# babybirdprd/dia-tts-prune

Hardware: AMD Instinct MI355X
Metric: audio-codec frames/sec (Dia-1.6B decode, whole job) (higher is better)
Workload: dtype bf16; 1 GPU; Dia-1.6B bf16 weights, bf16 K/V, batch 1, 1890 decode steps, text bytes [98], cfg 3.0 / T 1.3 / top-p 0.95 / top-k 35, hipGraph=True; batch_per_gpu=1, parallelism=single

## Files before the change

### dia-tts-prune_amd/csrc/engine.hip

```cpp
#include "common.hpp"
#include "../../include/dia_hip.h"
#include "errors.hpp"
#include "launch.hpp"
#include "tuning.hpp"
#include <cstdlib>
#include <vector>
#include <algorithm>
#include <utility>

struct dia_engine {
  dia_engine_desc d;
  std::vector<dia_dec_layer> layers;
  hipStream_t stream = nullptr;
  hipGraph_t graph = nullptr;
  hipGraphExec_t exec = nullptr;
  int launches = 0;
  bool seg = false;
  std::vector<const void*> seg_w;
  int mlp_fused = -1;
  std::vector<hipEvent_t> prof;
  int pf_lookahead = 0;
  bool pf_capturing = false;
  hipStream_t side = nullptr;
  std::vector<hipEvent_t> pf_ev;
  std::vector<std::pair<const void*, long>> pf_w;
};

int dia_prefetch_launch(const void* ptr, long nbytes, int nblocks, hipStream_t st);
static int ensure_sink();

static inline void mark(dia_engine* e, int i) {
  if (!e->prof.empty() && i + 1 < (int)e->prof.size()) (void)hipEventRecord(e->prof[i + 1], e->stream);
  if (e->pf_capturing) {
    const int j = i + e->pf_lookahead;
    if (j < (int)e->pf_w.size() && e->pf_w[j].first != nullptr) {
      (void)hipEventRecord(e->pf_ev[i], e->stream);
      (void)hipStreamWaitEvent(e->side, e->pf_ev[i], 0);
      const long bytes = e->pf_w[j].second;
      const int nb = (int)std::min<long>(512, std::max<long>(32, bytes / (256 * 16 * 8)));
      (void)dia_prefetch_launch(e->pf_w[j].first, bytes, nb, e->side);
    }
  }
}

constexpr int MXFP8_DEFAULT = (1 << DIA_MAT_WI | 1 << DIA_MAT_WO | 1 << DIA_MAT_LOGITS) | (1 << DIA_MAT_WI | 1 << DIA_MAT_LOGITS) << 8;
static_assert(MXFP8_DEFAULT == 0x5070 && DIA_MAT_COUNT <= 8, "the knob mxfp8 holds one byte of class bits per row range");
extern "C" int dia_mxfp8_classes(int rows) {
  if (rows <= 0 || rows > 16) return 0;
  const int knob = dia_tune(DIA_TUNE_MXFP8);
  const int mask = knob >= 0 ? knob : MXFP8_DEFAULT;
  return (rows <= 4 ? mask : mask >> 8) & ((1 << DIA_MAT_COUNT) - 1);
}

enum { PL_NONE = -1, PL_X, PL_A, PL_H };
enum { OUT_NONE, OUT_QKV, OUT_QC, OUT_LOGITS, OUT_X };
struct step_mat_row {
  int mat;
  const void* dia_dec_layer::*w; int32_t dia_dec_layer::*kt; int32_t dia_dec_layer::*ns;
  const void* dia_dec_layer::*w24; const void* dia_dec_layer::*wf8;
  int epi, in, out, emit;
  const int32_t* dia_dec_layer::*cmap;
  const float* dia_dec_layer::*gnext;
};
#define MAT(M, m) DIA_MAT_##M, &dia_dec_layer::w_##m, &dia_dec_layer::kt_##m, &dia_dec_layer::ns_##m, &dia_dec_layer::w_##m##_24, &dia_dec_layer::w_##m##_f8
constexpr step_mat_row STEP_MATS[DIA_MAT_COUNT] = {
  {MAT(QKV, qkv), DIA_EPI_SCALE_STORE, PL_X, OUT_QKV, PL_NONE, nullptr, nullptr},
  {MAT(O, o), DIA_EPI_RESID_EMIT, PL_A, OUT_X, PL_X, &dia_dec_layer::cmap_ca, &dia_dec_layer::g_ca},
  {MAT(CQ, cq), DIA_EPI_SCALE_STORE, PL_X, OUT_QC, PL_NONE, nullptr, nullptr},
  {MAT(CO, co), DIA_EPI_RESID_EMIT, PL_A, OUT_X, PL_X, &dia_dec_layer::cmap_mlp, &dia_dec_layer::g_mlp},
  {MAT(WI, wi), DIA_EPI_SWIGLU_EMIT, PL_X, OUT_NONE, PL_H, nullptr, nullptr},
  {MAT(WO, wo), DIA_EPI_RESID_EMIT, PL_H, OUT_X, PL_X, &dia_dec_layer::cmap_next, nullptr},
  {DIA_MAT_LOGITS, nullptr, nullptr, nullptr, nullptr, nullptr, DIA_EPI_SCALE_STORE, PL_X, OUT_LOGITS, PL_NONE, nullptr, nullptr},
};
#undef MAT
constexpr bool rows_in_order(int m = 0) { return m == DIA_MAT_COUNT || (STEP_MATS[m].mat == m && rows_in_order(m + 1)); }
static_assert(rows_in_order(), "row m of STEP_MATS describes matrix m of dia_step_mat");

struct mat_w { const void* w; int kt, ns; const void *w24, *wf8; };
static mat_w mat_weights(const dia_engine* e, int l, int m) {
  const dia_engine_desc& d = e->d;
  if (m == DIA_MAT_LOGITS) return {d.w_logits, d.kt_logits, d.ns_logits, d.w_logits_24, d.w_logits_f8};
  const dia_dec_layer& L = e->layers[l];
  const step_mat_row& r = STEP_MATS[m];
  return {L.*r.w, L.*r.kt, L.*r.ns, L.*r.w24, L.*r.wf8};
}

enum { ATTN_SELF = DIA_MAT_COUNT, ATTN_CROSS, SEG_MLP, SAMPLER };
template <class Launch>
static int step_sequence(const dia_engine* e, bool with_sampler, Launch&& launch) {
  int rc = DIA_OK;
  auto run = [&](int l, std::initializer_list<int> seq) { for (int what : seq) if (!rc) rc = launch(l, what); };
  for (int l = 0; l < e->d.n_layer; ++l) {
    if (!e->seg || l == 0) run(l, {DIA_MAT_QKV});
    run(l, {ATTN_SELF, DIA_MAT_O, DIA_MAT_CQ, ATTN_CROSS});
    if (e->seg) run(l, {SEG_MLP});
    else run(l, {DIA_MAT_CO, DIA_MAT_WI, DIA_MAT_WO});
  }
  run(e->d.n_layer, {DIA_MAT_LOGITS});
  if (with_sampler) run(e->d.n_layer, {SAMPLER});
  return rc;
}

static bool wo_split_k(const dia_engine_desc& d, const dia_dec_layer& L, int R, dia_gemm_args& g) {
  int wo_sk = (R <= 4 && L.kt_wo % 2 == 0) ? 2 : ((R <= 16 && L.kt_wo % 4 == 0) ? 4 : 1);
  int wo_spw = 0;
  if (R > 4 && R <= 16) {
    if (L.kt_wo % 64 == 0 && L.kt_wo / 64 >= 2 && L.kt_wo / 64 <= 8) wo_sk = L.kt_wo / 64;
    if (wo_sk > 1 && L.ns_wo * wo_sk >= 512 && L.ns_wo % 2 == 0) wo_spw = 2;
  }
  const int w2_sk = (d.w_planes == 2 && L.kt_wo % 128 == 0 && L.kt_wo / 128 <= 8) ? L.kt_wo / 128 : 1;
  if (d.w_planes == 2) { wo_sk = w2_sk; wo_spw = 0; }
  if (dia_tune(DIA_TUNE_WO_SK) >= 1 && dia_tune(DIA_TUNE_WO_SK) <= 8 && L.kt_wo % dia_tune(DIA_TUNE_WO_SK) == 0) wo_sk = dia_tune(DIA_TUNE_WO_SK);
  g.sk = wo_sk; g.sk_scratch = wo_sk > 1 ? d.sk_scratch : nullptr; g.sk_tickets = wo_sk > 1 ? d.sk_tickets : nullptr;
  bool wo_pair = false;
  if (R > 16 && R <= 128) {
    g.sk_scratch = d.sk_scratch; g.sk_tickets = d.sk_tickets;
    g.sk_scratch_floats = d.sk_scratch_floats > 0 ? d.sk_scratch_floats : (int64_t)(d.D / 16) * 4 * 512;
    wo_pair = L.kt_wo % 4 == 0 && g.sk_scratch_floats >= (int64_t)((R + 15) / 16) * L.ns_wo * 4 * 256 &&
              dia_tune(DIA_TUNE_WO_PAIR) != 0;
    g.sk = wo_pair ? 4 : 1;
    if (d.w_planes == 2) {
      wo_pair = w2_sk > 1 && g.sk_scratch_floats >= (int64_t)((R + 15) / 16) * L.ns_wo * w2_sk * 256;
      g.sk = wo_pair ? w2_sk : 1;
    }
  }
  if (dia_tune(DIA_TUNE_WO_NW) > 0) g.nw = dia_tune(DIA_TUNE_WO_NW);
  g.spw = wo_spw;
  if (dia_tune(DIA_TUNE_WO_SPW) > 0) g.spw = dia_tune(DIA_TUNE_WO_SPW);
  return wo_pair;
}

static int enqueue_step(dia_engine* e, bool with_sampler) {
  const dia_engine_desc& d = e->d;
  void* st = (void*)e->stream;
  const int R = 2 * d.B;
  const int xkt = d.D / 32;
  const int akt = (max(d.q_heads, d.cq_heads) * 128) / 32;
  const int hkt = d.F / 32;
  const long mt = d.rows_pad / 16;
  const struct { void* p; long stride; int kt; } planes[] = {
    {d.planes_x, mt * xkt * 512, xkt}, {d.planes_a, mt * akt * 512, akt}, {d.planes_h, mt * hkt * 512, hkt}};
  const int nqkv = (d.q_heads + 2 * d.kv_heads) * 128;
  const int F = d.act_f32 ? 1 : 0;
  const bool two_tiles = R > 16 && R <= 32 && d.sk_scratch && d.sk_tickets && d.sk_scratch_floats > 0;

  const bool seg = e->seg;
  bool diag = (R <= 2 || (R <= 4 && d.F <= 4096)) && d.act_f32 && d.w_planes <= 1 && dia_tune(DIA_TUNE_WO_DIAG) == 1 && !seg;
  for (int l = 0; l < d.n_layer && diag; ++l) diag = e->layers[l].w_wo_diag != nullptr && e->layers[l].cmap_next == nullptr;
  const int xn_wo = diag ? d.D / 8 : d.D / 16;
  auto sparse24 = [&](dia_gemm_args& g, const void* w24) {
    if (!w24 || !F || d.w_planes > 1 || R > 4) return;
    g.W = w24; g.KT /= 2; g.w_format = DIA_W_SPARSE24; g.nw = 0; g.spw = 0;
    int sk = g.sk > 1 ? g.sk : 1;
    while (sk > 1 && g.KT % (8 * sk) != 0) sk /= 2;
    g.sk = sk;
    if (sk == 1) { g.sk_scratch = nullptr; g.sk_tickets = nullptr; }
  };
  const int f8_mask = (F && d.w_planes <= 1 && !seg && !diag) ? dia_mxfp8_classes(R) : 0;
  auto mxfp8 = [&](dia_gemm_args& g, const void* wf8, int cls) {
    if (!wf8 || !(f8_mask >> cls & 1) || g.cmap || g.strip_map || g.KT % 16 != 0) return;
    int sk = g.sk > 1 ? g.sk : 1;
    while (sk > 1 && g.KT % (16 * sk) != 0) sk /= 2;
    while (g.KT / sk > 128 && g.KT % (32 * sk) == 0 && d.sk_scratch && d.sk_tickets && sk < 4) sk *= 2;
    if (g.KT / sk > 128) return;
    g.W = wf8; g.w_format = DIA_W_MXFP8; g.nw = 0; g.spw = 0;
    g.sk = sk;
    if (sk == 1) { g.sk_scratch = nullptr; g.sk_tickets = nullptr; }
    else { g.sk_scratch = d.sk_scratch; g.sk_tickets = d.sk_tickets; }
  };
  bool wo_pair = false;
  auto step_gemm = [&](int l, int m) {
    const step_mat_row& r = STEP_MATS[m];
    const dia_dec_layer* L = l < d.n_layer ? &e->layers[l] : nullptr;
    const mat_w w = mat_weights(e, l, m);
    dia_gemm_args g = {};
    g.A = planes[r.in].p; g.a_plane_stride = planes[r.in].stride; g.a_ktiles = planes[r.in].kt; g.M = R;
    g.W = w.w; g.KT = w.kt; g.nstrips = w.ns; g.epi = r.epi; g.ssq_ld = d.rows_pad;
    if (r.in == PL_X) {
      g.ssq_in = d.ssq; g.ssq_in_n = (m == DIA_MAT_LOGITS || (m == DIA_MAT_QKV && l > 0)) ? xn_wo : d.D / 16; g.inv_d = 1.0f / d.D; g.eps = d.eps;
    }
    if (r.emit != PL_NONE) { g.P = planes[r.emit].p; g.p_plane_stride = planes[r.emit].stride; g.p_ktiles = planes[r.emit].kt; }
    switch (r.out) {
      case OUT_QKV: g.out = d.qkv; g.ldo = nqkv; g.strip_map = L->smap_qkv; break;
      case OUT_QC: g.out = d.qc; g.ldo = d.cq_heads * 128; g.strip_map = L->smap_cq; break;
      case OUT_LOGITS: g.out = d.logits; g.ldo = d.ld_logits; break;
      case OUT_X:
        g.out = d.x; g.ldo = d.D; g.ssq_out = d.ssq; g.cmap = L->*r.cmap;
        g.gnext = r.gnext ? L->*r.gnext : ((l + 1 < d.n_layer) ? e->layers[l + 1].g_sa : d.g_final);
        break;
    }
    g.w_planes = d.w_planes; g.act_f32 = r.epi == DIA_EPI_SCALE_STORE ? F : 3 * F;
    if (two_tiles) { g.sk_scratch = d.sk_scratch; g.sk_tickets = d.sk_tickets; g.sk_scratch_floats = d.sk_scratch_floats; }
    if (m == DIA_MAT_WO) wo_pair = wo_split_k(d, *L, R, g);
    if (m == DIA_MAT_WO && diag) {
      g.W = L->w_wo_diag; g.w_layout = 1; g.nstrips = d.D / 8; g.sk = 1; g.sk_scratch = nullptr; g.sk_tickets = nullptr; g.nw = 0; g.spw = 0;
      return g;
    }
    sparse24(g, w.w24);
    mxfp8(g, w.wf8, m);
    return g;
  };

  int n = 0;
  bool fused = false;
  const int rc = step_sequence(e, with_sampler, [&](int l, int what) -> int {
    int rc = DIA_OK;
    if (what == ATTN_SELF || what == ATTN_CROSS) {
      const dia_dec_layer& L = e->layers[l];
      dia_attn_args a = {};
      a.kv_dtype = d.kv_dtype; a.cur = d.sample.cur; a.v_blocked = d.v_blocked; a.cos_t = d.cos_t; a.sin_t = d.sin_t;
      a.P = planes[PL_A].p; a.p_plane_stride = planes[PL_A].stride; a.p_ktiles = akt;
      a.scratch = d.attn_scratch; a.tickets = d.attn_tickets; a.act_f32 = F;
      if (what == ATTN_SELF) {
        a.mode = DIA_ATTN_SELF; a.n_kv_heads = d.kv_heads; a.group = d.q_heads / d.kv_heads; a.n_rows = R; a.kv_cap = d.T;
        a.q = d.qkv; a.ldq = nqkv; a.k_off = d.q_heads * 128; a.v_off = (d.q_heads + d.kv_heads) * 128; a.rope_rows = d.T + 1;
        a.kc = L.k_self; a.vc = L.v_self; a.head_map = L.hmap_self; a.kv_plane_stride = d.kv_plane_self;
      } else {
        a.mode = DIA_ATTN_CROSS; a.n_kv_heads = d.cq_heads; a.group = 1; a.n_rows = d.B; a.kv_cap = d.S;
        a.q = d.qc; a.ldq = d.cq_heads * 128; a.len = d.text_len;
        a.kc = L.k_cross; a.vc = L.v_cross; a.head_map = L.hmap_cross; a.kv_plane_stride = d.kv_plane_cross;
      }
      rc = dia_attn(&a, st);
    } else if (what == SEG_MLP) {
      dia_seg_args sa = {};
      sa.a_in = (const float*)d.planes_a; sa.a_ktiles = akt; sa.M = R; sa.W = e->seg_w[l];
      sa.has_qkv = l + 1 < d.n_layer; sa.nslots = dia_seg_slots(sa.has_qkv); sa.D = d.D; sa.F = d.F;
      sa.x = d.x; sa.ldx = d.D; sa.g_mlp = e->layers[l].g_mlp; sa.g_next = (l + 1 < d.n_layer) ? e->layers[l + 1].g_sa : d.g_final;
      sa.qkv_out = d.qkv; sa.ldq = nqkv; sa.planes_x = (float*)d.planes_x; sa.xkt = xkt; sa.ssq = d.ssq; sa.ssq_ld = d.rows_pad;
      sa.eps = d.eps; sa.ws = d.seg_ws;
      rc = dia_seg_mlp(&sa, st);
    } else if (what == SAMPLER) {
      rc = dia_sample(&d.sample, st);
    } else if (what == DIA_MAT_WO && fused) {
      fused = false;
    } else {
      dia_gemm_args g = step_gemm(l, what);
      if (what == DIA_MAT_WI && e->mlp_fused != 0 && R <= 2 && d.mlp_barrier && !e->layers[l].cmap_mlp && d.w_planes <= 1 && !d.act_f32) {
        dia_gemm_args go = step_gemm(l, DIA_MAT_WO);
        go.sk = 2; go.sk_scratch = d.sk_scratch; go.sk_tickets = d.sk_tickets; go.nw = 0; go.spw = 0;
        rc = dia_mlp_fused(&g, &go, d.mlp_barrier, st);
        if (rc != DIA_OK && rc != DIA_E_ARG) return rc;
        fused = rc == DIA_OK;
        e->mlp_fused = fused ? 1 : 0;
      }
      if (!fused) rc = dia_gemm(&g, st);
      if (what == DIA_MAT_WO && rc == DIA_E_ARG && g.sk > 1) {
        g.sk = 1;
        if (!wo_pair) { g.sk_scratch = nullptr; g.sk_tickets = nullptr; }
        rc = dia_gemm(&g, st);
      }
    }
    if (!rc) mark(e, n++);
    return rc;
  });
  if (!rc) e->launches = n;
  return rc;
}

extern "C" int dia_engine_create(const dia_engine_desc* d, void* stream, dia_engine** out) {
  if (!d || !out || !d->layers) return dia_fail(DIA_E_ARG, "dia_engine_create: null argument");
  if (d->n_layer <= 0 || d->B <= 0) return dia_fail(DIA_E_ARG, "dia_engine_create: empty model");
  if (d->D % 32 != 0 || d->F % 32 != 0) return dia_fail(DIA_E_ARG, "dia_engine_create: D and F must be multiples of 32");
  if (d->rows_pad < 2 * d->B || d->rows_pad % 16 != 0) return dia_fail(DIA_E_ARG, "dia_engine_create: rows_pad must be 16*ceil(2B/16)");
  if (d->q_heads % d->kv_heads != 0) return dia_fail(DIA_E_ARG, "dia_engine_create: q_heads % kv_heads != 0");
  if (d->act_f32 && !d->sample.embed.act_f32)
    return dia_fail(DIA_E_ARG, "dia_engine_create: act_f32 needs an embedding that writes fp32 tiles too");
  if (!d->act_f32 && d->sample.embed.act_f32) return dia_fail(DIA_E_ARG, "dia_engine_create: the embedding writes fp32 tiles but the engine reads planes");
  if (!d->x || !d->planes_x || !d->planes_a || !d->planes_h || !d->ssq || !d->qkv || !d->qc || !d->logits || !d->cos_t ||
      !d->sin_t || !d->text_len || !d->w_logits || !d->g_final || !d->attn_scratch || !d->attn_tickets)
    return dia_fail(DIA_E_ARG, "dia_engine_create: missing buffer");
  dia_engine* e = new dia_engine();
  e->d = *d;
  e->layers.assign(d->layers, d->layers + d->n_layer);
  e->d.layers = e->layers.data();
  e->stream = (hipStream_t)stream;
  if (d->seg_w && d->seg_ws) {
    const int nqkv = (d->q_heads + 2 * d->kv_heads) * 128;
    if (2 * d->B > 4 || !d->act_f32 || d->w_planes > 1 || !dia_seg_supported(d->D, d->F, max(d->q_heads, d->cq_heads) * 128, nqkv) ||
        d->cq_heads * 128 != 2048) {
      delete e;
      return dia_fail(DIA_E_ARG, "dia_engine_create: persistent segments need <= 4 rows, fp32 activation tiles, one weight plane, Dia-1.6B decoder shapes and 256 CUs");
    }
    for (int l = 0; l < d->n_layer; ++l) {
      const dia_dec_layer& L = d->layers[l];
      if (!d->seg_w[l] || L.cmap_mlp || L.cmap_next || L.smap_qkv) { delete e; return dia_fail(DIA_E_ARG, "dia_engine_create: persistent segments take dense (uncompacted) layers only"); }
    }
    e->seg_w.assign(d->seg_w, d->seg_w + d->n_layer);
    e->d.seg_w = e->seg_w.data();
    e->seg = true;
  }
  e->mlp_fused = dia_tune(DIA_TUNE_MLP_FUSE) > 0 ? -1 : 0;
  *out = e;
  return DIA_OK;
}

extern "C" int dia_engine_destroy(dia_engine* e) {
  if (!e) return DIA_OK;
  hipError_t he = hipSuccess;
  if (e->stream) he = hipStreamSynchronize(e->stream);
  if (e->side) { hipError_t h2 = hipStreamSynchronize(e->side); if (he == hipSuccess) he = h2; }
  if (e->exec) (void)hipGraphExecDestroy(e->exec);
  if (e->graph) (void)hipGraphDestroy(e->graph);
  for (auto& ev : e->pf_ev) if (ev) (void)hipEventDestroy(ev);
  for (auto& ev : e->prof) if (ev) (void)hipEventDestroy(ev);
  if (e->side) (void)hipStreamDestroy(e->side);
  delete e;
  return he == hipSuccess ? DIA_OK : dia_fail_hip(he, "dia_engine_destroy: hipStreamSynchronize");
}

extern "C" int dia_engine_decode(dia_engine* e, int n_steps, int use_graph) {
  if (!e || n_steps < 0) return dia_fail(DIA_E_ARG, "dia_engine_decode: bad argument");
  if (!use_graph) {
    for (int i = 0; i < n_steps; ++i) {
      int rc = enqueue_step(e, true);
      if (rc) return rc;
    }
    return DIA_OK;
  }
  if (!e->exec) {
    if (e->stream == nullptr) return dia_fail(DIA_E_STATE, "dia_engine_decode: graph capture needs a non-default stream");
    if (e->pf_lookahead > 0) {
      int rc0 = ensure_sink();
      if (rc0) return rc0;
      e->pf_w.clear();
      (void)step_sequence(e, true, [&](int l, int what) {
        const mat_w w = what < DIA_MAT_COUNT ? mat_weights(e, l, what) : mat_w{};
        e->pf_w.push_back({w.w, (long)w.kt * w.ns * 1024});
        return DIA_OK;
      });
      if (!e->side && hipStreamCreateWithFlags(&e->side, hipStreamNonBlocking) != hipSuccess) return dia_fail(DIA_E_HIP, "hipStreamCreate(side)");
      e->pf_ev.assign(e->pf_w.size() + 2, nullptr);
      for (auto& ev : e->pf_ev)
        if (hipEventCreateWithFlags(&ev, hipEventDisableTiming) != hipSuccess) return dia_fail(DIA_E_HIP, "hipEventCreate(prefetch)");
    }
    hipError_t he = hipStreamBeginCapture(e->stream, hipStreamCaptureModeThreadLocal);
    if (he != hipSuccess) return dia_fail_hip(he, "hipStreamBeginCapture");
    if (e->pf_lookahead > 0) {
      (void)hipEventRecord(e->pf_ev[e->pf_w.size()], e->stream);
      (void)hipStreamWaitEvent(e->side, e->pf_ev[e->pf_w.size()], 0);
      e->pf_capturing = true;
    }
    int rc = enqueue_step(e, true);
    if (e->pf_lookahead > 0) {
      e->pf_capturing = false;
      (void)hipEventRecord(e->pf_ev[e->pf_w.size() + 1], e->side);
      (void)hipStreamWaitEvent(e->stream, e->pf_ev[e->pf_w.size() + 1], 0);
    }
    he = hipStreamEndCapture(e->stream, &e->graph);
    if (rc) return rc;
    if (he != hipSuccess) return dia_fail_hip(he, "hipStreamEndCapture");
    he = hipGraphInstantiate(&e->exec, e->graph, nullptr, nullptr, 0);
    if (he != hipSuccess) return dia_fail_hip(he, "hipGraphInstantiate");
  }
  for (int i = 0; i < n_steps; ++i) {
    hipError_t he = hipGraphLaunch(e->exec, e->stream);
    if (he != hipSuccess) return dia_fail_hip(he, "hipGraphLaunch");
  }
  return DIA_OK;
}

extern "C" int dia_engine_step_logits_only(dia_engine* e) {
  if (!e) return dia_fail(DIA_E_ARG, "dia_engine_step_logits_only: null engine");
  return enqueue_step(e, false);
}

__global__ void k_delay(long long ticks) {
  const long long t0 = wall_clock64();
  while (wall_clock64() - t0 < ticks) __builtin_amdgcn_s_sleep(32);
}

extern "C" int dia_engine_profile_step(dia_engine* e, float* ms, int cap) {
  if (!e || !ms) return dia_fail(DIA_E_ARG, "dia_engine_profile_step: null argument");
  const int n = dia_engine_launches_per_step(e);
  if (cap < n) return dia_fail(DIA_E_ARG, "dia_engine_profile_step: output array too small");
  e->prof.resize(n + 1);
  for (auto& ev : e->prof) {
    hipError_t he = hipEventCreate(&ev);
    if (he != hipSuccess) return dia_fail_hip(he, "hipEventCreate");
  }
  int rc = DIA_OK;
  dia_launch<k_delay>(dim3(1), dim3(64), 0, e->stream, 300000LL );
  (void)hipEventRecord(e->prof[0], e->stream);
  rc = enqueue_step(e, true);
  {
    hipError_t he = hipStreamSynchronize(e->stream);
    if (rc == DIA_OK && he != hipSuccess) rc = dia_fail_hip(he, "hipStreamSynchronize");
  }
  if (rc == DIA_OK)
    for (int i = 0; i < n; ++i)
      if (hipEventElapsedTime(&ms[i], e->prof[i], e->prof[i + 1]) != hipSuccess) { ms[i] = -1.f; (void)hipGetLastError(); }
  for (auto& ev : e->prof) (void)hipEventDestroy(ev);
  e->prof.clear();
  return rc;
}

extern "C" int dia_engine_time_step(dia_engine* e, float* ms, float* interval_ms, int cap) {
  if (!e || !ms) return dia_fail(DIA_E_ARG, "dia_engine_time_step: null argument");
  const int n = dia_engine_launches_per_step(e);
  if (cap < n) return dia_fail(DIA_E_ARG, "dia_engine_time_step: output array too small");
  dia_launch<k_delay>(dim3(1), dim3(64), 0, e->stream, 300000LL );
  dia_recorder_arm();
  int rc = enqueue_step(e, true);
  const int got = dia_recorder_collect(ms, cap, interval_ms);
  hipError_t he = hipStreamSynchronize(e->stream);
  if (rc != DIA_OK) return rc;
  if (he != hipSuccess) return dia_fail_hip(he, "dia_engine_time_step: hipStreamSynchronize");
  return got;
}

extern "C" const char* dia_timed_kernel_name(int i) { return dia_recorder_label(i); }

extern "C" int dia_engine_mlp_fused(const dia_engine* e) { return e && e->mlp_fused == 1; }

extern "C" int dia_engine_launches_per_step(const dia_engine* e) {
  if (!e) return dia_fail(DIA_E_ARG, "null engine");
  int n = 0;
  (void)step_sequence(e, true, [&](int, int) { return ++n, DIA_OK; });
  return n;
}

__global__ __launch_bounds__(256) void k_prefetch(const uint4* __restrict__ p, long n16, unsigned* sink) {
  uint4 acc = {0, 0, 0, 0};
  const long stride = (long)gridDim.x * 256;
  long i = (long)blockIdx.x * 256 + threadIdx.x;
  for (; i + 3 * stride < n16; i += 4 * stride) {
    const uint4 a = p[i], b = p[i + stride], c = p[i + 2 * stride], d = p[i + 3 * stride];
    acc.x ^= a.x ^ b.x ^ c.x ^ d.x; acc.y ^= a.y ^ b.y ^ c.y ^ d.y;
    acc.z ^= a.z ^ b.z ^ c.z ^ d.z; acc.w ^= a.w ^ b.w ^ c.w ^ d.w;
  }
  for (; i < n16; i += stride) { const uint4 a = p[i]; acc.x ^= a.x; acc.y ^= a.y; acc.z ^= a.z; acc.w ^= a.w; }
  if ((acc.x ^ acc.y ^ acc.z ^ acc.w) == 0x9E3779B9u && sink) *sink = 1;
}

static unsigned* g_sink = nullptr;
static int ensure_sink() {
  if (!g_sink) {
    hipError_t e = hipMalloc(&g_sink, 4);
    if (e != hipSuccess) return dia_fail_hip(e, "hipMalloc(sink)");
  }
  return DIA_OK;
}

int dia_prefetch_launch(const void* ptr, long nbytes, int nblocks, hipStream_t st) {
  dia_launch<k_prefetch>(dim3(nblocks), dim3(256), 0, st, (const uint4*)ptr, (long)(nbytes / 16), g_sink);
  return dia_check_launch("k_prefetch");
}

extern "C" int dia_prefetch(const void* ptr, int64_t nbytes, int nblocks, void* stream) {
  if (!ptr || nbytes <= 0 || nblocks <= 0) return dia_fail(DIA_E_ARG, "dia_prefetch: bad argument");
  int rc = ensure_sink();
  if (rc) return rc;
  return dia_prefetch_launch(ptr, (long)nbytes, nblocks, (hipStream_t)stream);
}

extern "C" int dia_engine_set_prefetch(dia_engine* e, int lookahead) {
  if (!e || lookahead < 0) return dia_fail(DIA_E_ARG, "dia_engine_set_prefetch: bad argument");
  if (e->exec) return dia_fail(DIA_E_STATE, "dia_engine_set_prefetch: the step graph is already captured");
  e->pf_lookahead = lookahead;
  return DIA_OK;
}
```

### dia-tts-prune_amd/csrc/gemm.hip

```cpp
#include "gemm_common.hpp"
#include "gemm_experiments.hpp"

namespace {

template <int MT, int NW, int KPW>
__global__ __launch_bounds__(NW * 64) void k_gemm(GemmK p) {
  extern __shared__ __attribute__((aligned(16))) unsigned char smem_raw[];
  f32x4* red = reinterpret_cast<f32x4*>(smem_raw);
  float* tile = reinterpret_cast<float*>(smem_raw + sizeof(f32x4) * NW * MT * 64);
  float* inv_s = tile + MT * 16 * 17;

  const int tid = threadIdx.x, lane = tid & 63, w = tid >> 6;
  const int strip = blockIdx.x;
  const int mt0 = blockIdx.y * MT;
  const int kpw = (KPW > 0) ? KPW : (p.KT + NW - 1) / NW;
  const int kt0 = w * kpw;

  f32x4 acc[MT];
  long aoff[MT];
#pragma unroll
  for (int i = 0; i < MT; ++i) {
    acc[i] = f32x4{0.f, 0.f, 0.f, 0.f};
    const int mtile = min(mt0 + i, (p.M - 1) >> 4);
    const int rlast = min(15, p.M - 1 - mtile * 16);
    const int alane = (lane & 48) | min(lane & 15, rlast);
    aoff[i] = ((long)mtile * p.a_ktiles * 64 + alane) * 8;
  }

  const bf16x8* Wt = reinterpret_cast<const bf16x8*>(p.W) + ((long)strip * p.KT) * 64 + lane;
  const bf16x8 zero8 = {0, 0, 0, 0, 0, 0, 0, 0};

  const int e_mt = tid >> 5, e_r = (tid >> 1) & 15, half = tid & 1;
  const int m = (mt0 + e_mt) * 16 + e_r;
  const int n0 = strip * 16 + half * 8;
  const bool e_thread = tid < MT * 32;
  const bool live = e_thread && m < p.M;
  float xpre[8], gpre[8];

  if (p.w_planes > 1) {
    prefetch_epilogue<MT, NW * 64>(p, tid, mt0, m, n0, live, xpre, gpre, inv_s);
    const int kt1 = min(kt0 + kpw, p.KT);
    const int npw = p.w_planes == 2 ? 1 : p.w_planes, ash = p.w_planes == 2 ? 1 : 0;
    for (int pw = 0; pw < npw; ++pw) {
      const bf16x8* Wp = Wt + pw * (p.w_plane_stride / 8);
      for (int kt = kt0; kt < kt1; ++kt) {
        const bf16x8 bb = DIA_WLOAD(Wp + (long)kt * 64);
#pragma unroll
        for (int mt = 0; mt < MT; ++mt) {
          bf16x8 a3[DIA_NPLANES];
          load_afrag3(p, aoff[mt] + (long)(kt >> ash) * 512, a3[0], a3[1], a3[2]);
#pragma unroll
          for (int pl = 0; pl < DIA_NPLANES; ++pl)
            acc[mt] = __builtin_amdgcn_mfma_f32_16x16x32_bf16(a3[pl], bb, acc[mt], 0, 0, 0);
        }
      }
    }
  } else if constexpr (KPW > 0) {
    bf16x8 b[KPW];
#pragma unroll
    for (int i = 0; i < KPW; ++i) b[i] = DIA_WLOAD(Wt + (long)(kt0 + i) * 64);
    __builtin_amdgcn_sched_barrier(0);
    constexpr int AP = (KPW >= 8) ? 1 : ((KPW * MT <= 4) ? KPW : ((4 / MT) > 0 ? (4 / MT) : 1));
    bf16x8 a0[AP][MT][DIA_NPLANES];
#pragma unroll
    for (int i = 0; i < AP; ++i)
#pragma unroll
      for (int mt = 0; mt < MT; ++mt)
        load_afrag3(p, aoff[mt] + (long)(kt0 + i) * 512, a0[i][mt][0], a0[i][mt][1], a0[i][mt][2]);
    prefetch_epilogue<MT, NW * 64>(p, tid, mt0, m, n0, live, xpre, gpre, inv_s);
#pragma unroll
    for (int i = 0; i < KPW; ++i) {
#pragma unroll
      for (int mt = 0; mt < MT; ++mt) {
        bf16x8 a3[DIA_NPLANES];
        if (i < AP) { a3[0] = a0[i < AP ? i : 0][mt][0]; a3[1] = a0[i < AP ? i : 0][mt][1]; a3[2] = a0[i < AP ? i : 0][mt][2]; }
        else load_afrag3(p, aoff[mt] + (long)(kt0 + i) * 512, a3[0], a3[1], a3[2]);
#pragma unroll
        for (int pl = 0; pl < DIA_NPLANES; ++pl)
          acc[mt] = __builtin_amdgcn_mfma_f32_16x16x32_bf16(a3[pl], b[i], acc[mt], 0, 0, 0);
      }
    }
  } else {
    prefetch_epilogue<MT, NW * 64>(p, tid, mt0, m, n0, live, xpre, gpre, inv_s);
    const int kt1 = min(kt0 + kpw, p.KT);
    for (int kt = kt0; kt < kt1; kt += 4) {
      bf16x8 b[4];
#pragma unroll
      for (int i = 0; i < 4; ++i) b[i] = (kt + i < kt1) ? DIA_WLOAD(Wt + (long)(kt + i) * 64) : zero8;
#pragma unroll
      for (int i = 0; i < 4; ++i) {
        if (kt + i < kt1) {
#pragma unroll
          for (int mt = 0; mt < MT; ++mt) {
            bf16x8 a3[DIA_NPLANES];
            load_afrag3(p, aoff[mt] + (long)(kt + i) * 512, a3[0], a3[1], a3[2]);
#pragma unroll
            for (int pl = 0; pl < DIA_NPLANES; ++pl)
              acc[mt] = __builtin_amdgcn_mfma_f32_16x16x32_bf16(a3[pl], b[i], acc[mt], 0, 0, 0);
          }
        }
      }
    }
  }

  reduce_to_tile<MT, NW>(acc, red, tile, tid, lane, w);
  if (!e_thread) return;
  run_epilogue(p, tile + (e_mt * 16 + e_r) * 17, inv_s[e_mt * 16 + e_r], m, n0, half, strip, live, xpre, gpre);
}


template <int NW, int KPW, int RS, bool MULTI, bool AF32 = false, bool PF32 = false, bool W2 = false>
__global__ __launch_bounds__(NW * 64) void k_gemv_small(const bf16_raw* a_A, long a_aps, const bf16_raw* a_W, int a_KT, int a_M, int a_epi,
                                                        int a_nstrips, float* a_out, int a_ldo, const float* a_gnext, GemmK p) {
  p.A = a_A; p.a_plane_stride = a_aps; p.W = a_W; p.KT = a_KT; p.M = a_M; p.epi = a_epi; p.nstrips = a_nstrips;
  p.out = a_out; p.ldo = a_ldo; p.gnext = a_gnext;
  extern __shared__ __attribute__((aligned(16))) unsigned char smem_raw[];
  f32x4* red = reinterpret_cast<f32x4*>(smem_raw);
  float* tile = reinterpret_cast<float*>(smem_raw + sizeof(f32x4) * NW * 64);
  float* inv_s = tile + 16 * 17;
  bf16x8* As = reinterpret_cast<bf16x8*>(smem_raw + sizeof(f32x4) * NW * 64 + sizeof(float) * (16 * 17 + 16));

  const int tid = threadIdx.x, lane = tid & 63, w = tid >> 6;
  const int kt0 = w * KPW;
  const int ktg = blockIdx.y * (NW * KPW);
  constexpr int WS = W2 ? 1 : 0;
  const int ktga = ktg >> WS;
  const int G = gridDim.x;
  const bf16x8* Wl = reinterpret_cast<const bf16x8*>(p.W) + (long)(ktg + kt0) * 64 + lane;
  auto load_strip = [&](bf16x8* b, int strip) {
    const bf16x8* Wt = Wl + (long)strip * p.KT * 64;
#pragma unroll
    for (int i = 0; i < KPW; ++i) b[i] = DIA_WLOAD(Wt + (long)i * 64);
  };
  __shared__ int sk_flag;

  STAMP(0);
  bf16x8 b0[KPW], b1[MULTI ? KPW : 1];
  constexpr int KT = (NW * KPW) >> WS;
  constexpr int KPA = KPW >> WS;
  static_assert(!W2 || KPW % 2 == 0, "two-plane weights: whole activation k-tiles per wave");
  constexpr int NT = NW * 64;
#ifdef DIA_X_WFIRST
  load_strip(b0, blockIdx.x);
  __builtin_amdgcn_sched_barrier(0);
#endif

  constexpr int CH = (3 * KPA * RS + 15) / 16;
  constexpr int nchunks = DIA_NPLANES * KT * 4 * RS;
  constexpr int nentries = KT * 4 * RS;
  constexpr int CE = (KPA * RS + 15) / 16;
  bf16x8 v0[AF32 ? 1 : CH];
  float4 ex[AF32 ? CE : 1], ey[AF32 ? CE : 1];
  if constexpr (AF32) {
    const float* Af = reinterpret_cast<const float*>(p.A);
#pragma unroll
    for (int u = 0; u < CE; ++u) {
      const int c = min(tid + u * NT, nentries - 1);
      const int row = c % RS, kq = (c / RS) & 3, kt = c / (4 * RS);
      const float4* src = reinterpret_cast<const float4*>(Af + ((long)(ktga + kt) * 64 + row + 16 * kq) * 8);
      ex[u] = src[0]; ey[u] = src[1];
    }
  } else {
#pragma unroll
    for (int u = 0; u < CH; ++u) {
      const int c = min(tid + u * NT, nchunks - 1);
      const int row = c % RS, kq = (c / RS) & 3, kt = (c / (4 * RS)) % KT, pl = c / (4 * RS * KT);
      v0[u] = *reinterpret_cast<const bf16x8*>(p.A + pl * p.a_plane_stride + ((long)(ktga + kt) * 64 + row + 16 * kq) * 8);
    }
  }
  const bool has_norm = p.ssq_in != nullptr;
  const int s_row = tid >> 3, s_part = tid & 7;
  const bool s_thread = tid < 128 && has_norm;
  float sq[16];
#pragma unroll
  for (int i = 0; i < 16; ++i) sq[i] = 0.f;
  if (s_thread) {
    const float* sp = p.ssq_in + min(s_row, p.M - 1);
#pragma unroll
    for (int i = 0; i < 16; ++i) sq[i] = sp[(long)min(s_part + 8 * i, p.ssq_in_n - 1) * p.ssq_ld];
  }
  const bool resid = p.epi == DIA_EPI_RESID_EMIT;
  const bool r_thread = tid < 16 * RS;
  float xpre1 = 0.f, gpre1 = 1.f;
  auto load_resid = [&](int strip) {
    const int r_m = tid >> 4, n = strip * 16 + (tid & 15);
    xpre1 = p.out[(long)(r_m < p.M ? r_m : 0) * p.ldo + n];
    gpre1 = p.gnext[n];
  };
  if (resid && r_thread) load_resid(blockIdx.x);
  __builtin_amdgcn_sched_barrier(0);
#ifndef DIA_X_WFIRST
  load_strip(b0, blockIdx.x);
  __builtin_amdgcn_sched_barrier(0);
#endif
  STAMP(1);
  if constexpr (AF32) {
#pragma unroll
    for (int u = 0; u < CE; ++u)
      if (tid + u * NT < nentries) {
        const int c = tid + u * NT;
        bf16x8 h, mi, lo;
        split3x8(ex[u], ey[u], h, mi, lo);
        As[c] = h; As[nentries + c] = mi; As[2 * nentries + c] = lo;
      }
  } else {
#pragma unroll
    for (int u = 0; u < CH; ++u)
      if (tid + u * NT < nchunks) As[tid + u * NT] = v0[u];
  }
  {
    float s0 = 0.f;
#pragma unroll
    for (int i = 0; i < 16; ++i) s0 += (s_part + 8 * i < p.ssq_in_n && s_row < p.M) ? sq[i] : 0.f;
    if (s_thread && s_row < p.M)
      for (int idx = s_part + 128; idx < p.ssq_in_n; idx += 8) s0 += p.ssq_in[(long)idx * p.ssq_ld + s_row];
    s0 += __builtin_bit_cast(float, __builtin_amdgcn_update_dpp(0, __builtin_bit_cast(int, s0), 0xB1, 0xF, 0xF, true));
    s0 += __builtin_bit_cast(float, __builtin_amdgcn_update_dpp(0, __builtin_bit_cast(int, s0), 0x4E, 0xF, 0xF, true));
    s0 += __builtin_bit_cast(float, __builtin_amdgcn_update_dpp(0, __builtin_bit_cast(int, s0), 0x141, 0xF, 0xF, true));
    if (tid < 128 && s_part == 0) inv_s[s_row] = has_norm ? rsqrtf(s0 * p.inv_d + p.eps) : 1.0f;
  }
  lds_barrier();
  STAMP(2);

  const int arow = min(lane & 15, RS - 1), akq = lane >> 4;
  f32x4* red16 = red;
  int sbuf = 0;
  auto body = [&](bf16x8* bc, bf16x8* bn, int strip) {
    const int next = strip + G;
    if constexpr (MULTI) load_strip(bn, DIA_PREFETCH_CLAMP(next, p.nstrips));
#ifdef DIA_PIN_PREFETCH
    if constexpr (MULTI) __builtin_amdgcn_sched_barrier(0);
#endif
    f32x4 acc[1] = {f32x4{0.f, 0.f, 0.f, 0.f}};
#pragma unroll
    for (int i = 0; i < KPW; ++i) {
#pragma unroll
      for (int pl = 0; pl < DIA_NPLANES; ++pl) {
        const bf16x8 a = As[((pl * KT + ((kt0 + i) >> WS)) * 4 + akq) * RS + arow];
        acc[0] = __builtin_amdgcn_mfma_f32_16x16x32_bf16(a, bc[i], acc[0], 0, 0, 0);
      }
    }
    STAMP(3);
    float v = 0.f;
    if (MULTI || gridDim.y == 1) {
      f32x4* rb = red16 + sbuf * (NW * 16);
      sbuf ^= 1;
      if (lane < 16) rb[w * 16 + lane] = acc[0];
      lds_barrier();
      if (r_thread) {
        const float* rf = reinterpret_cast<const float*>(rb) + (tid & 15) * 4 + (tid >> 4);
        v = rf[0];
#pragma unroll
        for (int ww = 1; ww < NW; ++ww) v += rf[ww * 64];
      }
      STAMP(4);
    } else {
      reduce_to_tile<1, NW, true>(acc, red, tile, tid, lane, w);
      STAMP(4);
      if (!splitk_combine(p, tile, strip, tid, &sk_flag)) return;
      if (r_thread) v = tile[(tid >> 4) * 17 + (tid & 15)];
    }
    if (r_thread) {
      run_epilogue_rows<RS, PF32>(p, v, inv_s, tid, strip, xpre1, gpre1);
      if (MULTI && next < p.nstrips && resid) load_resid(next);
    }
  };
  if constexpr (MULTI) {
    int strip = blockIdx.x;
    for (; strip + G < p.nstrips; strip += 2 * G) {
      body(b0, b1, strip);
      body(b1, b0, strip + G);
    }
    if (strip < p.nstrips) body(b0, b1, strip);
  } else {
    body(b0, b1, blockIdx.x);
  }
  STAMP(5);
}


#ifndef DIA_Z_TEMPORAL
#define DIA_Z_TEMPORAL 1
#endif
constexpr bool ZTEMPORAL = DIA_Z_TEMPORAL != 0;
#ifndef DIA_ZR_RING3
#define DIA_ZR_RING3 0
#endif
constexpr size_t g16_smem(int nw) { return sizeof(f32x4) * 2 * nw * 64 + 1536 + sizeof(float) * (2 * 16 * 17 + 16); }
constexpr size_t g16_alds(int nw, int kpw) { return (size_t)2 * nw * kpw * 64 * 16; }
template <int NW, int KPW, bool MULTI, bool MZ = false, bool AF32 = false, bool PF32 = false, bool PAIR = false, bool ALDS = false, bool W2 = false>
__global__ __launch_bounds__(NW * 64) void k_gemm16(const bf16_raw* a_A, long a_aps, const bf16_raw* a_W, int a_KT, int a_M, int a_epi,
                                                    int a_nstrips, float* a_out, int a_ldo, const float* a_gnext, GemmK p) {
  p.A = a_A; p.a_plane_stride = a_aps; p.W = a_W; p.KT = a_KT; p.M = a_M; p.epi = a_epi; p.nstrips = a_nstrips;
  p.out = a_out; p.ldo = a_ldo; p.gnext = a_gnext;
  extern __shared__ __attribute__((aligned(16))) unsigned char smem_raw[];
  f32x4* red = reinterpret_cast<f32x4*>(smem_raw);
  bf16_raw* stg = reinterpret_cast<bf16_raw*>(smem_raw + sizeof(f32x4) * 2 * NW * 64);
  float* tile = reinterpret_cast<float*>(smem_raw + sizeof(f32x4) * 2 * NW * 64 + 1536);
  float* inv_s = tile + 16 * 17;
  constexpr int NT = NW * 64;

  int zrow0 = 0;
  if constexpr (MZ) {
    const int z = blockIdx.z;
    zrow0 = 16 * z;
    p.A += (long)z * p.a_ktiles * 512 * (AF32 ? 2 : 1);
    p.M = min(16, p.M - 16 * z);
    if (p.ssq_in) p.ssq_in += 16 * z;
    if (p.out) p.out += (long)16 * z * p.ldo;
    if (p.P) p.P += (long)z * p.p_ktiles * 512 * (PF32 ? 2 : 1);
    if (p.ssq_out) p.ssq_out += 16 * z;
    if (p.sk_scratch) { p.sk_scratch += (long)z * p.nstrips * gridDim.y * 256; p.sk_tickets += z * p.nstrips; }
  }
  const int tid = threadIdx.x, lane = tid & 63, w = tid >> 6;
  const int kt0 = blockIdx.y * (NW * KPW) + w * KPW;
  constexpr int WS = W2 ? 1 : 0;
  constexpr int KPA = KPW >> WS;
  static_assert(!W2 || KPW % 2 == 0, "two-plane weights: whole activation k-tiles per wave");
  const int kta0 = kt0 >> WS;
  const int G = gridDim.x;
  __shared__ int sk_flag;
  const bf16x8* Wl = reinterpret_cast<const bf16x8*>(p.W) + (long)kt0 * 64 + lane;
  auto load_strip = [&](bf16x8* b, int strip) {
    const bf16x8* Wt = Wl + (long)strip * p.KT * 64;
#pragma unroll
    for (int i = 0; i < KPW; ++i) b[i] = (MZ && ZTEMPORAL) ? *(Wt + (long)i * 64) : DIA_WLOAD(Wt + (long)i * 64);
  };
  bf16x8 b0[KPW], b1[MULTI ? KPW : 1];
  STAMP(0);

  const int r16 = tid >> 4, c16 = tid & 15;
  const bool r_thread = tid < 256;
  float xpre1 = 0.f, gpre1 = 1.f;

  const int alane = (lane & 48) | min(lane & 15, p.M - 1);
  bf16x8 a[KPA][DIA_NPLANES];
  constexpr bool ALDS_LATE = ALDS && !MZ;
  if constexpr (AF32) {
    const float4* Af = reinterpret_cast<const float4*>(reinterpret_cast<const float*>(p.A) + ((long)kta0 * 64 + alane) * 8);
#pragma unroll
    for (int i = 0; i < KPA; ++i) {
#ifdef DIA_X_NOA
      a[i][0] = __builtin_bit_cast(bf16x8, Af[0]);
      a[i][1] = __builtin_bit_cast(bf16x8, Af[1]);
#else
      a[i][0] = __builtin_bit_cast(bf16x8, Af[(long)i * 128]);
      a[i][1] = __builtin_bit_cast(bf16x8, Af[(long)i * 128 + 1]);
#endif
    }
    if constexpr (!ALDS_LATE) {
#pragma unroll
      for (int i = 0; i < KPA; ++i)
        split3x8(__builtin_bit_cast(float4, a[i][0]), __builtin_bit_cast(float4, a[i][1]), a[i][0], a[i][1], a[i][2]);
    }
  } else {
#pragma unroll
    for (int i = 0; i < KPA; ++i)
#pragma unroll
      for (int pl = 0; pl < DIA_NPLANES; ++pl)
        a[i][pl] = *reinterpret_cast<const bf16x8*>(p.A + pl * p.a_plane_stride + ((long)(kta0 + i) * 64 + alane) * 8);
  }
  bf16x8* my = reinterpret_cast<bf16x8*>(smem_raw + g16_smem(NW)) + (long)w * 2 * KPA * 64 + lane;
  if constexpr (ALDS && !ALDS_LATE) {
#pragma unroll
    for (int i = 0; i < KPA; ++i) { my[i * 64] = a[i][1]; my[(KPA + i) * 64] = a[i][2]; }
  }
  auto afrag = [&](int i, int pl) -> bf16x8 {
    if constexpr (ALDS) { if (pl > 0) return my[((pl - 1) * KPA + (i >> WS)) * 64]; }
    return a[i >> WS][pl];
  };
  const bool has_norm = p.ssq_in != nullptr;
  const int s_row = tid >> 3, s_part = tid & 7;
  const bool s_thread = tid < 128 && has_norm;
  float sq[16];
#pragma unroll
  for (int i = 0; i < 16; ++i) sq[i] = 0.f;
  if (s_thread) {
    const float* sp = p.ssq_in + min(s_row, p.M - 1);
#pragma unroll
    for (int i = 0; i < 16; ++i) sq[i] = sp[(long)min(s_part + 8 * i, p.ssq_in_n - 1) * p.ssq_ld];
  }
  const bool resid = p.epi == DIA_EPI_RESID_EMIT;
  auto load_resid = [&](int strip) {
    const int n = strip * 16 + c16;
    xpre1 = p.out[(long)(r16 < p.M ? r16 : 0) * p.ldo + n];
    gpre1 = p.gnext[n];
  };
  const int e_r = (tid >> 1) & 15, e_half = tid & 1;
  const bool e_thread = tid < 32, e_live = e_thread && e_r < p.M;
  float xpre8[8], gpre8[8];
  auto load_resid8 = [&](int strip) {
    const int n0 = strip * 16 + e_half * 8;
    const float* o = p.out + (long)(e_live ? e_r : 0) * p.ldo + n0;
    const float4 xa = *reinterpret_cast<const float4*>(o), xb = *reinterpret_cast<const float4*>(o + 4);
    xpre8[0] = xa.x; xpre8[1] = xa.y; xpre8[2] = xa.z; xpre8[3] = xa.w;
    xpre8[4] = xb.x; xpre8[5] = xb.y; xpre8[6] = xb.z; xpre8[7] = xb.w;
    const float4 ga = *reinterpret_cast<const float4*>(p.gnext + n0), gb = *reinterpret_cast<const float4*>(p.gnext + n0 + 4);
    gpre8[0] = ga.x; gpre8[1] = ga.y; gpre8[2] = ga.z; gpre8[3] = ga.w;
    gpre8[4] = gb.x; gpre8[5] = gb.y; gpre8[6] = gb.z; gpre8[7] = gb.w;
  };
  constexpr bool ZTAIL8 = MULTI && !MZ && !PAIR && KPW == 8 && AF32 && !ALDS;
  constexpr bool pair = PAIR;
  constexpr bool ZT = (MZ && !ALDS) || ZTAIL8;
  if constexpr (ZT) { if (resid && e_thread) load_resid8(blockIdx.x); }
  else { if (resid && r_thread) load_resid(blockIdx.x); }
  __builtin_amdgcn_sched_barrier(0);
  load_strip(b0, blockIdx.x);
  __builtin_amdgcn_sched_barrier(0);
  if constexpr (ALDS_LATE) {
#pragma unroll
    for (int i = 0; i < KPA; ++i) {
      if constexpr (AF32) split3x8(__builtin_bit_cast(float4, a[i][0]), __builtin_bit_cast(float4, a[i][1]), a[i][0], a[i][1], a[i][2]);
      my[i * 64] = a[i][1]; my[(KPA + i) * 64] = a[i][2];
// ... 1217 lines not shown
      if (kpw == 2) return launch_g16<8, 2, true, true>(k, st);
      if (kpw == 3) return launch_g16<8, 3, true, true>(k, st);
      if (kpw == 4) return launch_g16<8, 4, true, true>(k, st);
      if (kpw == 5) return launch_g16<8, 5, true, true>(k, st);
      if (kpw == 6) return launch_g16<8, 6, true, true>(k, st);
      if (kpw == 7) return launch_g16<8, 7, true, true>(k, st);
      if (kpw == 8) return launch_g16<8, 8, true, true>(k, st);
    }
    handled = false;
    return DIA_OK;
  }
  if (nw == 16) {
    if (kpw == 1) return launch_g16<16, 1>(k, st);
    if (kpw == 2) return launch_g16<16, 2>(k, st);
    if (kpw == 4) return launch_g16<16, 4>(k, st);
  } else if (nw == 8) {
    if (kpw == 1) return launch_g16<8, 1>(k, st);
    if (kpw == 2) return launch_g16<8, 2>(k, st);
    if (kpw == 3) return launch_g16<8, 3>(k, st);
    if (kpw == 4) return launch_g16<8, 4>(k, st);
    if (kpw == 5) return launch_g16<8, 5>(k, st);
    if (kpw == 6) return launch_g16<8, 6>(k, st);
    if (kpw == 7) return launch_g16<8, 7>(k, st);
    if (kpw == 8) return launch_g16<8, 8>(k, st);
  } else if (nw == 4) {
    if (kpw == 4) return launch_g16<4, 4>(k, st);
    if (kpw == 8) return launch_g16<4, 8>(k, st);
  }
  handled = false;
  return DIA_OK;
}

template <int MT, int NW, int KPW>
int launch(const GemmK& k, int mgroups, hipStream_t st) {
  size_t smem = sizeof(f32x4) * NW * MT * 64 + sizeof(float) * (MT * 16 * 17 + MT * 16);
  launch_kernel<k_gemm<MT, NW, KPW>>(dim3(k.nstrips, mgroups), dim3(NW * 64), smem, st, k);
  return dia_check_launch("k_gemm");
}

template <int MT, int NW>
int launch_kpw(const GemmK& k, int mgroups, hipStream_t st) {
  if (k.KT % NW == 0) {
    switch (k.KT / NW) {
      case 1: return launch<MT, NW, 1>(k, mgroups, st);
      case 2: return launch<MT, NW, 2>(k, mgroups, st);
      case 4: return launch<MT, NW, 4>(k, mgroups, st);
      case 8: return launch<MT, NW, 8>(k, mgroups, st);
      case 16: if constexpr (NW <= 8) return launch<MT, NW, 16>(k, mgroups, st); else break;
      case 32: if constexpr (NW <= 8) return launch<MT, NW, 32>(k, mgroups, st); else break;
      default: break;
    }
  }
  return launch<MT, NW, 0>(k, mgroups, st);
}

template <int MT>
int launch_nw(const GemmK& k, int nw, int mgroups, hipStream_t st) {
  switch (nw) {
    case 4: return launch_kpw<MT, 4>(k, mgroups, st);
    case 8: return launch_kpw<MT, 8>(k, mgroups, st);
    case 16: return launch_kpw<MT, 16>(k, mgroups, st);
    default: return dia_fail(DIA_E_ARG, "dia_gemm: nw must be 4, 8 or 16");
  }
}

int launch_generic(const GemmK& k, int nw, hipStream_t st) {
  const int mtiles = (k.M + 15) / 16;
  if (mtiles == 1) return launch_nw<1>(k, nw, 1, st);
  if (mtiles == 2) return launch_nw<2>(k, nw, 1, st);
  return launch_nw<4>(k, nw, (mtiles + 3) / 4, st);
}

size_t small_smem(int nw, int KT, int rs) {
  return sizeof(f32x4) * nw * 64 + sizeof(float) * (16 * 17 + 16) + (size_t)DIA_NPLANES * KT * 4 * rs * 16;
}

template <int NW, int KPW, int RS, bool F32 = false>
int launch_small(const GemmK& k, hipStream_t st) {
  size_t smem = small_smem(NW, NW * KPW, RS);
  const int sk = k.KT / (NW * KPW);
  const int spw = pick_spw(k, 512, 1, sk);
  const int grid = (k.nstrips + spw - 1) / spw;
  if (sk > 1) {
    launch_small_kernel<k_gemv_small<NW, KPW, RS, false, F32, F32>>(dim3(k.nstrips, sk), dim3(NW * 64), smem, st, k);
    return dia_check_launch("k_gemv_small");
  }
  if (spw > 1) {
    if constexpr (KPW <= 16 && !(NW == 16 && KPW > 4))
      launch_small_kernel<k_gemv_small<NW, KPW, RS, true, F32, F32>>(dim3(grid), dim3(NW * 64), smem, st, k);
    else
      launch_small_kernel<k_gemv_small<NW, KPW, RS, false, F32, F32>>(dim3(k.nstrips), dim3(NW * 64), smem, st, k);
  } else {
    launch_small_kernel<k_gemv_small<NW, KPW, RS, false, F32, F32>>(dim3(k.nstrips), dim3(NW * 64), smem, st, k);
  }
  return dia_check_launch("k_gemv_small");
}

template <int RS, bool F32 = false>
int launch_small_rs(const GemmK& k, int nw, int sk, hipStream_t st, bool& handled) {
  handled = true;
  const int kpw = (k.KT % (nw * sk) == 0) ? k.KT / (nw * sk) : 0;
  if (nw == 4) {
    if (kpw == 4) return launch_small<4, 4, RS, F32>(k, st);
    if (kpw == 8) return launch_small<4, 8, RS, F32>(k, st);
    if (kpw == 16) return launch_small<4, 16, RS, F32>(k, st);
  } else if (nw == 8) {
    if (kpw == 2) return launch_small<8, 2, RS, F32>(k, st);
    if (kpw == 3) return launch_small<8, 3, RS, F32>(k, st);
    if (kpw == 4) return launch_small<8, 4, RS, F32>(k, st);
    if (kpw == 5) return launch_small<8, 5, RS, F32>(k, st);
    if (kpw == 6) return launch_small<8, 6, RS, F32>(k, st);
    if (kpw == 7) return launch_small<8, 7, RS, F32>(k, st);
    if (kpw == 8) return launch_small<8, 8, RS, F32>(k, st);
    if (kpw == 10) return launch_small<8, 10, RS, F32>(k, st);
    if (kpw == 12) return launch_small<8, 12, RS, F32>(k, st);
    if (kpw == 14) return launch_small<8, 14, RS, F32>(k, st);
    if (kpw == 16) return launch_small<8, 16, RS, F32>(k, st);
    if (kpw == 32) return launch_small<8, 32, RS, F32>(k, st);
  } else if (nw == 16) {
    if (kpw == 1) return launch_small<16, 1, RS, F32>(k, st);
    if (kpw == 2) return launch_small<16, 2, RS, F32>(k, st);
    if (kpw == 4) return launch_small<16, 4, RS, F32>(k, st);
    if (kpw == 8) return launch_small<16, 8, RS, F32>(k, st);
  }
  handled = false;
  return DIA_OK;
}

constexpr int W2_KTW = 128;

template <int RS>
int launch_small_w2(const GemmK& k, int sk, hipStream_t st) {
  const size_t smem = small_smem(8, W2_KTW / 2, RS);
  if (sk > 1) {
    launch_small_kernel<k_gemv_small<8, 16, RS, false, true, true, true>>(dim3(k.nstrips, sk), dim3(512), smem, st, k);
    return dia_check_launch("k_gemv_small");
  }
  const int spw = pick_spw(k, 512, 1, 1);
  if (spw > 1) launch_small_kernel<k_gemv_small<8, 16, RS, true, true, true, true>>(dim3((k.nstrips + spw - 1) / spw), dim3(512), smem, st, k);
  else launch_small_kernel<k_gemv_small<8, 16, RS, false, true, true, true>>(dim3(k.nstrips), dim3(512), smem, st, k);
  return dia_check_launch("k_gemv_small");
}

int launch_g16_w2(const GemmK& k, int mz, int sk, hipStream_t st) {
  const size_t smem = g16_smem(8) + g16_alds(8, W2_KTW / 16);
  const int spw = pick_spw(k, 256, mz, sk);
  int gx = (k.nstrips + spw - 1) / spw;
  if (mz >= 2) gx = xcd_round(gx, sk, k.nstrips);
  if (mz >= 2) launch_small_kernel<k_gemm16<8, 16, true, true, true, true, false, true, true>>(dim3(gx, sk, mz), dim3(512), smem, st, k);
  else launch_small_kernel<k_gemm16<8, 16, true, false, true, true, false, true, true>>(dim3(gx, sk), dim3(512), smem, st, k);
  return dia_check_launch("k_gemm16");
}

}

#ifdef DIA_DBG_STAMPS
extern "C" int dia_dbg_stamps(long long* host, int n) {
  return hipMemcpyFromSymbol(host, HIP_SYMBOL(g_stamps), sizeof(long long) * n) == hipSuccess ? 0 : -2;
}
#endif

extern "C" int dia_has_experiments(void) {
#ifdef DIA_EXPERIMENTS
  return 1;
#else
  return 0;
#endif
}

namespace {
int split_k(const dia_gemm_args* a) {
  const int sk = a->sk > 1 ? a->sk : 1;
  if (sk > 1 && (!a->sk_scratch || !a->sk_tickets || a->KT % sk != 0)) return dia_fail(DIA_E_ARG, "dia_gemm: split-K needs sk_scratch, sk_tickets and KT % sk == 0");
  return sk;
}

int gemm_mz_max() { return dia_tune(DIA_TUNE_GEMM_MZ_MAX) >= 0 ? dia_tune(DIA_TUNE_GEMM_MZ_MAX) : 8; }

int gemm_w2(const dia_gemm_args* a, GemmK& k, hipStream_t st) {
  const int sk = split_k(a);
  if (sk < 0) return sk;
  const int mtiles = (a->M + 15) / 16;
  const bool fast_epi = a->epi != DIA_EPI_CROSSKV && !(a->epi == DIA_EPI_RESID_EMIT && !a->gnext);
  const bool emits = a->epi == DIA_EPI_RESID_EMIT || a->epi == DIA_EPI_SWIGLU_EMIT;
  const bool uni_f32 = k.a_f32 && (!emits || k.p_f32);
  if (uni_f32 && fast_epi && a->KT % sk == 0 && a->KT / sk == W2_KTW && (a->nw == 0 || a->nw == 8)) {
    if (a->M <= 4) return a->M <= 2 ? launch_small_w2<2>(k, sk, st) : launch_small_w2<4>(k, sk, st);
    if (mtiles == 1) return launch_g16_w2(k, 1, sk, st);
    if (mtiles <= gemm_mz_max() && (sk == 1 || a->sk_scratch_floats >= (int64_t)mtiles * a->nstrips * sk * 256)) return launch_g16_w2(k, mtiles, sk, st);
  }
  if (sk > 1) return dia_fail(DIA_E_ARG, "dia_gemm: two-plane weights: no split-K kernel for this shape");
  return launch_generic(k, (a->KT % 8 == 0) ? 8 : 4, st);
}
}

extern "C" int dia_gemm(const dia_gemm_args* a, void* stream) {
  if (!a || !a->A || (!a->W && !a->sp_blocks)) return dia_fail(DIA_E_ARG, "dia_gemm: null argument");
  if (a->M <= 0 || a->KT <= 0 || a->nstrips <= 0) return dia_fail(DIA_E_ARG, "dia_gemm: empty problem");
  if (a->w_format != DIA_W_DENSE && a->w_format != DIA_W_SPARSE24 && a->w_format != DIA_W_MXFP8) return dia_fail(DIA_E_ARG, "dia_gemm: unknown w_format");
  if (a->w_format == DIA_W_SPARSE24) {
    const int rc = dia_gemm_sparse24_check(a);
    if (rc != DIA_OK) return rc;
  }
  if (a->w_format == DIA_W_MXFP8) {
    const int rc = dia_gemm_mxfp8_check(a);
    if (rc != DIA_OK) return rc;
  }
  if (a->w_planes == 2) {
    if (a->w_layout == 1)
      return dia_fail(DIA_E_ARG, "dia_gemm: w_planes = 2 interleaves hi / lo tiles inside the strip layout; the diagonal layout (w_layout = 1) has no two-plane form");
    if (a->sp_blocks || a->sp_toff)
      return dia_fail(DIA_E_ARG, "dia_gemm: w_planes = 2 streams dense hi / lo tiles; the zero-skipping sparse stream has no two-plane form");
    if (!a->W || a->KT % 2 != 0) return dia_fail(DIA_E_ARG, "dia_gemm: w_planes = 2 needs W and an even KT (two tiles per activation k-tile)");
    if (a->KT / 2 > a->a_ktiles) return dia_fail(DIA_E_ARG, "dia_gemm: weight K exceeds the plane layout's K");
  }
  if (a->w_layout == 1) {
    const int groups = a->nstrips;
    if (!a->out || !a->P || !a->ssq_out || a->ssq_ld < a->M || a->a_ktiles < a->KT) return dia_fail(DIA_E_ARG, "dia_gemm: diagonal layout: missing buffer");
    GemmK k;
    fill_gemmk(a, k);
    if (a->M > 4 || a->epi != DIA_EPI_RESID_EMIT || !a->gnext || a->cmap || (a->act_f32 & 3) != 3 || a->w_planes > 1 || a->sk > 1 ||
        a->KT % 32 != 0 || a->KT / 32 > 8 || a->p_ktiles * 32 < groups * 8 || a->ldo < groups * 8)
      return dia_fail(DIA_E_ARG, "dia_gemm: the diagonal weight layout serves M <= 4, RESID_EMIT, fp32 tiles, K a multiple of 1024 up to 8192");
    const int rs = a->M <= 2 ? 2 : 4;
    const size_t smem = sizeof(f32x4) * 16 * 16 + (size_t)3 * a->KT * 4 * rs * 16;
    if (smem > 152 * 1024) return dia_fail(DIA_E_ARG, "dia_gemm: diagonal layout: the activation image of these rows does not fit LDS (3-4 rows: K <= 4096)");
    if (rs == 2) launch_kernel<k_gemv_diag<2>>(dim3(groups), dim3(1024), smem, (hipStream_t)stream, k);
    else launch_kernel<k_gemv_diag<4>>(dim3(groups), dim3(1024), smem, (hipStream_t)stream, k);
    return dia_check_launch("k_gemv_diag");
  }
  if (a->w_planes != 2 && a->KT > a->a_ktiles) return dia_fail(DIA_E_ARG, "dia_gemm: weight K exceeds the plane layout's K");
  if (a->a_plane_stride % 8 != 0 || a->p_plane_stride % 8 != 0) return dia_fail(DIA_E_ARG, "dia_gemm: plane stride must be a multiple of 8");
  if ((a->epi == DIA_EPI_SCALE_STORE || a->epi == DIA_EPI_RESID_EMIT) && (!a->out || (!a->strip_map && a->ldo < a->nstrips * 16) || a->ldo % 4 != 0))
    return dia_fail(DIA_E_ARG, "dia_gemm: output leading dimension too small");
  if ((a->epi == DIA_EPI_RESID_EMIT) && (!a->P || !a->ssq_out || a->p_ktiles * 32 < a->nstrips * 16))
    return dia_fail(DIA_E_ARG, "dia_gemm: RESID_EMIT needs planes and ssq_out covering N");
  if ((a->epi == DIA_EPI_SWIGLU_EMIT) && (!a->P || a->p_ktiles * 32 < a->nstrips * 8))
    return dia_fail(DIA_E_ARG, "dia_gemm: SWIGLU_EMIT needs planes covering N/2");
  if (a->epi == DIA_EPI_CROSSKV && (!a->kc || !a->vc || !a->cos_t || !a->sin_t || (!a->strip_map && a->nstrips != a->kv_heads * 16 && !(a->kv_layer_strips == a->kv_heads * 16 && a->nstrips % (a->kv_heads * 16) == 0)) ||
                                     a->kv_layer_strips < 0 || (a->kv_layer_strips > 0 && (a->kv_layer_strips != a->kv_heads * 16 || a->kv_layer_stride <= 0)) || (!a->row_b && a->M > a->kv_cap) || (!a->row_b != !a->seg_off) || (a->kv_vblocked && a->kv_cap % 32 != 0)))
    return dia_fail(DIA_E_ARG, "dia_gemm: CROSSKV shape mismatch");
  if (a->epi < 0 || a->epi > DIA_EPI_CROSSKV) return dia_fail(DIA_E_ARG, "dia_gemm: unknown epilogue");
  if (a->ssq_in && a->ssq_ld < ((a->M + 15) / 16) * 16) return dia_fail(DIA_E_ARG, "dia_gemm: ssq_ld smaller than padded rows");

  if (a->w_format == DIA_W_SPARSE24) return dia_gemm_sparse24(a, stream);
  if (a->w_format == DIA_W_MXFP8) return dia_gemm_mxfp8(a, stream);
  if (a->sp_blocks || a->sp_toff) {
#ifdef DIA_EXPERIMENTS
    return dia_exp_gemm_sparse(a, stream);
#else
    return dia_fail(DIA_E_ARG, "dia_gemm: the sparse weight stream needs a build with EXPERIMENTS=1");
#endif
  }
  GemmK k;
  fill_gemmk(a, k);
  if (a->w_planes == 2) return gemm_w2(a, k, (hipStream_t)stream);
  if (a->w_planes > 1) {
    if (a->w_planes != 3) return dia_fail(DIA_E_ARG, "dia_gemm: w_planes must be 0, 1, 2 or 3");
    return launch_generic(k, (a->KT % 8 == 0) ? 8 : 4, (hipStream_t)stream);
  }
  const bool fast_epi = a->epi != DIA_EPI_CROSSKV && !(a->epi == DIA_EPI_RESID_EMIT && !a->gnext);
  int nw = a->nw;
  if (nw == 0) {
    if (a->M <= 4 && a->nstrips >= 1024 && a->KT % 16 == 0 && a->KT / 16 <= 4) nw = 16;
    else if (a->M <= 4 && a->KT % 8 == 0 && a->KT / 8 <= 8) nw = 8;
    else if (a->nstrips >= 512 && a->KT % 4 == 0 && a->KT / 4 <= 32) nw = 4;
    else if (a->KT % 16 == 0 && a->KT / 16 <= 8) nw = 16;
    else if (a->KT % 8 == 0) nw = 8;
    else nw = 4;
  }
  const int mtiles = (a->M + 15) / 16;
  hipStream_t st = (hipStream_t)stream;
  const int sk = split_k(a);
  if (sk < 0) return sk;
  if (sk > 1 && !a->nw) { const int ktl = a->KT / sk; nw = (ktl % 16 == 0 && ktl / 16 <= (a->M <= 4 ? 8 : 4)) ? 16 : ((ktl % 8 == 0) ? 8 : 4); }
  const bool emits_ = a->epi == DIA_EPI_RESID_EMIT || a->epi == DIA_EPI_SWIGLU_EMIT;
  const bool uni_f32 = k.a_f32 && (!emits_ || k.p_f32);
  if (a->M <= 4 && fast_epi && (!a->act_f32 || uni_f32)) {
    const int rs = a->M <= 2 ? 2 : 4;
    if (small_smem(nw, a->KT / sk, rs) <= 150 * 1024) {
      bool handled = false;
      int rc;
      if (uni_f32) rc = (rs == 2) ? launch_small_rs<2, true>(k, nw, sk, st, handled) : launch_small_rs<4, true>(k, nw, sk, st, handled);
      else rc = (rs == 2) ? launch_small_rs<2>(k, nw, sk, st, handled) : launch_small_rs<4>(k, nw, sk, st, handled);
      if (handled) return rc;
    }
  }
  const int ktl16 = a->KT / sk;
  int nw16 = a->nw ? a->nw : ((ktl16 % 8 == 0 && ktl16 / 8 <= 8) ? 8 : ((ktl16 % 16 == 0 && ktl16 / 16 <= 4) ? 16 : 0));
  if (mtiles == 1 && fast_epi && nw16) {
    bool handled = false;
    int rc = launch_g16_any(k, nw16, sk, st, handled);
    if (handled) return rc;
  }
  const int mz_max = gemm_mz_max();
  {
    const bool f32io = k.a_f32 && (!emits_ || k.p_f32);
    const bool planes = !k.a_f32 && !k.p_f32;
    const int ktw = a->KT / sk;
    const bool shape = (ktw == 64 || (planes && ktw == 32)) && a->KT % sk == 0 && a->w_planes <= 1 && mtiles >= 2 && mtiles <= mz_max &&
                       (sk == 1 || a->sk_scratch_floats >= (int64_t)((mtiles + 1) / 2) * a->nstrips * sk * 512);
    const bool decode_ok = f32io && fast_epi && !a->cmap && !a->strip_map &&
                           (a->nstrips >= 1024 || (a->nstrips >= 512 && mtiles >= 2) || mtiles >= 7 || sk > 1 || dia_tune(DIA_TUNE_GEMM_2T) == 2);
    const bool prefill_ok = planes && mtiles >= 3 && (fast_epi || (a->epi == DIA_EPI_CROSSKV && ktw == 32)) && !(ktw == 32 && sk > 1);
    if (shape && (decode_ok || prefill_ok) && dia_tune(DIA_TUNE_GEMM_2T) != 0) {
      const int zp = (mtiles + 1) / 2;
      const bool half = !f32io && ktw == 32 && dia_tune(DIA_TUNE_GEMM_2T) != 3;
      int budget = half ? 512 : 256;
      if (!f32io && dia_tune(DIA_TUNE_G2T_WGS) > 0) budget = dia_tune(DIA_TUNE_G2T_WGS);
      const int spw_ = z_spw(a->nstrips, budget, zp, sk);
      const int gx = xcd_round((a->nstrips + spw_ - 1) / spw_, 1, a->nstrips);
      const dim3 grid(gx, sk, zp), blk(half ? 256 : 512);
      const bool puni = !f32io && !a->cmap && !a->strip_map && (a->epi != DIA_EPI_RESID_EMIT || a->gnext) && dia_tune(DIA_TUNE_GEMM_2T) != 5;
      if (f32io) {
        const bool uni = dia_tune(DIA_TUNE_GEMM_2T) != 5;
        if (sk > 1 && sk <= 4 && a->epi == DIA_EPI_RESID_EMIT && a->gnext && dia_tune(DIA_TUNE_GEMM_2T) != 6)
          launch_small_kernel<k_gemm2t<8, true, true, 8, false, -1, true>>(grid, blk, g2t_smem(8, 8, true), st, k);
        else if (sk > 1) launch_small_kernel<k_gemm2t<8, true, true>>(grid, blk, g2t_smem(8), st, k);
        else if (uni && a->epi == DIA_EPI_SCALE_STORE) launch_small_kernel<k_gemm2t<8, true, false, 8, false, DIA_EPI_SCALE_STORE>>(grid, blk, g2t_smem(8), st, k);
        else if (uni && a->epi == DIA_EPI_RESID_EMIT) launch_small_kernel<k_gemm2t<8, true, false, 8, false, DIA_EPI_RESID_EMIT>>(grid, blk, g2t_smem(8), st, k);
        else if (uni && a->epi == DIA_EPI_SWIGLU_EMIT) launch_small_kernel<k_gemm2t<8, true, false, 8, false, DIA_EPI_SWIGLU_EMIT>>(grid, blk, g2t_smem(8), st, k);
        else launch_small_kernel<k_gemm2t<8, true, false>>(grid, blk, g2t_smem(8), st, k);
      } else if (ktw == 64) {
        if (sk > 1 && sk <= 4 && a->epi == DIA_EPI_RESID_EMIT && a->gnext && !a->cmap && dia_tune(DIA_TUNE_GEMM_2T) != 6)
          launch_small_kernel<k_gemm2t<8, false, true, 8, false, -1, true>>(grid, blk, g2t_smem(8, 8, true), st, k);
        else if (sk > 1) launch_small_kernel<k_gemm2t<8, false, true>>(grid, blk, g2t_smem(8), st, k);
        else if (puni && a->epi == DIA_EPI_RESID_EMIT) launch_small_kernel<k_gemm2t<8, false, false, 8, false, DIA_EPI_RESID_EMIT>>(grid, blk, g2t_smem(8), st, k);
        else launch_small_kernel<k_gemm2t<8, false, false>>(grid, blk, g2t_smem(8), st, k);
      } else if (half && a->epi == DIA_EPI_CROSSKV && a->kv_dtype == DIA_KV_BF16 && a->kv_vblocked && !a->strip_map && dia_tune(DIA_TUNE_GEMM_2T) != 4) {
        launch_small_kernel<k_gemm2t<8, false, false, 4, true>>(grid, blk, g2t_smem(8, 4), st, k);
      } else if (half && puni && a->epi == DIA_EPI_SCALE_STORE) {
        launch_small_kernel<k_gemm2t<8, false, false, 4, false, DIA_EPI_SCALE_STORE>>(grid, blk, g2t_smem(8, 4), st, k);
      } else if (half && puni && a->epi == DIA_EPI_SWIGLU_EMIT) {
        launch_small_kernel<k_gemm2t<8, false, false, 4, false, DIA_EPI_SWIGLU_EMIT>>(grid, blk, g2t_smem(8, 4), st, k);
      } else if (half) {
        launch_small_kernel<k_gemm2t<8, false, false, 4>>(grid, blk, g2t_smem(8, 4), st, k);
      } else {
        launch_small_kernel<k_gemm2t<4, false, false>>(grid, blk, g2t_smem(4), st, k);
      }
      return dia_check_launch("k_gemm2t");
    }
  }
  const bool z_epi = fast_epi || a->epi == DIA_EPI_CROSSKV;
  if (mtiles >= 2 && mtiles <= mz_max && z_epi && nw16 && (sk == 1 || a->sk_scratch_floats >= (int64_t)mtiles * a->nstrips * sk * 256)) {
    bool handled = false;
    k.mz = mtiles;
    int rc = launch_g16_any(k, nw16, sk, st, handled);
    k.mz = 0;
    if (handled) return rc;
  }
#ifdef DIA_EXPERIMENTS
  if (mtiles == 2 && !a->act_f32) {
    bool handled = false;
    int rc = dia_exp_gemm_two_mtiles(a, stream, handled);
    if (handled) return rc;
  }
#endif
  if (sk > 1) return dia_fail(DIA_E_ARG, "dia_gemm: no split-K kernel for this shape");
  {
    const int blocks = ((mtiles + GT_MT - 1) / GT_MT) * ((a->nstrips + 15) / 16);
    const int min_blocks = dia_tune(DIA_TUNE_TILE_MIN_BLOCKS) >= 0 ? dia_tune(DIA_TUNE_TILE_MIN_BLOCKS) : 48;
    if (mtiles >= 3 && a->KT % 8 == 0 && blocks >= min_blocks && !a->act_f32) {
#ifdef DIA_EXPERIMENTS
      const int v = dia_tune(DIA_TUNE_TILE_V);
      if (v >= 0 && v <= 2) return dia_exp_tile_variant(a, stream, v);
#endif
      return launch_tile(k, st);
    }
  }
  return launch_generic(k, nw, st);
}

extern "C" int dia_gemm_timed(const dia_gemm_args* a, void* stream, float* ms_out) {
  if (!ms_out) return dia_fail(DIA_E_ARG, "dia_gemm_timed: null output");
  dia_recorder_arm();
  int rc = dia_gemm(a, stream);
  float ms[4] = {0.f, 0.f, 0.f, 0.f};
  const int n = dia_recorder_collect(ms, 4);
  if (rc != DIA_OK) return rc;
  if (n < 1) return n < 0 ? n : dia_fail(DIA_E_STATE, "dia_gemm_timed: nothing was launched");
  *ms_out = ms[0];
  return DIA_OK;
}

#ifndef DIA_EXPERIMENTS
extern "C" int dia_mlp_fused(const dia_gemm_args*, const dia_gemm_args*, int32_t*, void*) {
  return dia_fail(DIA_E_ARG, "dia_mlp_fused: experiment, needs a build with EXPERIMENTS=1");
}
extern "C" int dia_mlp_fused_timed(const dia_gemm_args*, const dia_gemm_args*, int32_t*, void*, float*) {
  return dia_fail(DIA_E_ARG, "dia_mlp_fused_timed: experiment, needs a build with EXPERIMENTS=1");
}
#endif
```

### dia-tts-prune_amd/csrc/gemm_common.hpp

```cpp
#pragma once
#include "common.hpp"
#include <type_traits>
#include "../../include/dia_hip.h"
#include "errors.hpp"
#include <hip/hip_ext.h>
#include <cstdlib>
#include <cstring>
#include "tuning.hpp"
#include "launch.hpp"

namespace {


#ifdef DIA_DBG_PLAIN_LOAD
#define DIA_WLOAD(ptr) (*(ptr))
#else
#define DIA_WLOAD(ptr) __builtin_nontemporal_load(ptr)
#endif

#ifdef DIA_DBG_COND_PREFETCH
#define DIA_PREFETCH_CLAMP(next, n) (next)
#else
#define DIA_PREFETCH_CLAMP(next, n) min((next), (n) - 1)
#endif

template <auto Kern, typename Arg>
void launch_kernel(dim3 grid, dim3 block, size_t smem, hipStream_t st, const Arg& arg) {
  dia_launch<Kern>(grid, block, smem, st, arg);
}

struct GemmK;
template <auto Kern>
void launch_small_kernel(dim3 grid, dim3 block, size_t smem, hipStream_t st, const GemmK& k);

typedef unsigned int u32x4 __attribute__((ext_vector_type(4)));

struct GemmK {
  const bf16_raw* A; long a_plane_stride; int a_ktiles; int M;
  const bf16_raw* W; int KT; int nstrips; int epi;
  const float* ssq_in; int ssq_in_n; int ssq_ld; float inv_d; float eps;
  float* out; int ldo;
  const float* gnext;
  bf16_raw* P; long p_plane_stride; int p_ktiles;
  float* ssq_out;
  void* kc; void* vc; int kv_dtype; int kv_heads; int kv_cap; int kv_batch_index;
  const float* cos_t; const float* sin_t;
  int spw;
  const int* cmap; const int* strip_map;
  float* sk_scratch; int* sk_tickets;
  int kv_vblocked;
  const int* row_b; const int* seg_off;
  const unsigned char* sp_blocks; const unsigned int* sp_toff;
  int mz;
  int a_f32, p_f32;
  long kv_plane_stride;
  long kv_layer_stride; int kv_layer_strips;
  int sk2_quads;
  int w_planes; long w_plane_stride;
};

__device__ __forceinline__ void load_afrag3(const GemmK& p, long off, bf16x8& a0, bf16x8& a1, bf16x8& a2) {
  if (p.a_f32) {
    const float4* s = reinterpret_cast<const float4*>(reinterpret_cast<const float*>(p.A) + off);
    split3x8(s[0], s[1], a0, a1, a2);
  } else {
    a0 = *reinterpret_cast<const bf16x8*>(p.A + off);
    a1 = *reinterpret_cast<const bf16x8*>(p.A + p.a_plane_stride + off);
    a2 = *reinterpret_cast<const bf16x8*>(p.A + 2 * p.a_plane_stride + off);
  }
}
__device__ __forceinline__ void emit_act8(const GemmK& p, int m, int n0, const float* v, const int* cmap) {
  if (p.p_f32) {
    float* Pf = reinterpret_cast<float*>(p.P);
    if (cmap) emit_f32x8_mapped(Pf, p.p_ktiles, m, n0, v, cmap);
    else emit_f32x8(Pf, p.p_ktiles, m, n0, v);
  } else {
    if (cmap) emit_planes8_mapped(p.P, p.p_plane_stride, p.p_ktiles, m, n0, v, cmap);
    else emit_planes8(p.P, p.p_plane_stride, p.p_ktiles, m, n0, v);
  }
}

template <auto Kern>
void launch_small_kernel(dim3 grid, dim3 block, size_t smem, hipStream_t st, const GemmK& k) {
  dia_launch<Kern>(grid, block, smem, st, k.A, k.a_plane_stride, k.W, k.KT, k.M, k.epi, k.nstrips, k.out, k.ldo, k.gnext, k);
}

__device__ __forceinline__ void kv_store(void* base, int dtype, long idx, float v, long plane_stride = 0) {
  if (dtype == DIA_KV_F32) reinterpret_cast<float*>(base)[idx] = v;
  else if (dtype == DIA_KV_BF16X2) {
    const __bf16 hi = (__bf16)v, lo = (__bf16)(v - (float)hi);
    reinterpret_cast<bf16_raw*>(base)[idx] = *reinterpret_cast<const bf16_raw*>(&hi);
    reinterpret_cast<bf16_raw*>(base)[idx + plane_stride] = *reinterpret_cast<const bf16_raw*>(&lo);
  } else KVElem<bf16_raw>::store(reinterpret_cast<bf16_raw*>(base) + idx, v);
}

template <int MT, int NT>
__device__ __forceinline__ void prefetch_epilogue(const GemmK& p, int tid, int mt0, int m, int n0, bool live,
                                                  float* xpre, float* gpre, float* inv_s) {
  if (p.epi == DIA_EPI_RESID_EMIT && live) {
    const float* o = p.out + (long)m * p.ldo + n0;
    const float4 xa = *reinterpret_cast<const float4*>(o), xb = *reinterpret_cast<const float4*>(o + 4);
    xpre[0] = xa.x; xpre[1] = xa.y; xpre[2] = xa.z; xpre[3] = xa.w;
    xpre[4] = xb.x; xpre[5] = xb.y; xpre[6] = xb.z; xpre[7] = xb.w;
#pragma unroll
    for (int j = 0; j < 8; ++j) gpre[j] = p.gnext ? p.gnext[n0 + j] : 1.0f;
  }
  for (int t = tid; t < MT * 128; t += NT) {
    const int r = t >> 3, part = t & 7;
    const int row = mt0 * 16 + r;
    float sA = 0.f, sB = 0.f;
    if (p.ssq_in != nullptr && row < p.M) {
      int i = part;
      for (; i + 8 < p.ssq_in_n; i += 16) {
        sA += p.ssq_in[(long)i * p.ssq_ld + row];
        sB += p.ssq_in[(long)(i + 8) * p.ssq_ld + row];
      }
      if (i < p.ssq_in_n) sA += p.ssq_in[(long)i * p.ssq_ld + row];
    }
    float sq = sA + sB;
    sq += __shfl_xor(sq, 1, 64);
    sq += __shfl_xor(sq, 2, 64);
    sq += __shfl_xor(sq, 4, 64);
    if (part == 0) inv_s[r] = (p.ssq_in != nullptr) ? rsqrtf(sq * p.inv_d + p.eps) : 1.0f;
  }
}

__device__ __forceinline__ void run_epilogue(const GemmK& p, const float* trow, float inv, int m, int n0, int half,
                                             int strip, bool live, const float* xpre, const float* gpre, bool pre_cs = false) {
  if (p.epi == DIA_EPI_SCALE_STORE) {
    if (!live) return;
    if (p.strip_map) n0 = p.strip_map[strip] * 16 + half * 8;
    float4 a = {trow[half * 8 + 0] * inv, trow[half * 8 + 1] * inv, trow[half * 8 + 2] * inv, trow[half * 8 + 3] * inv};
    float4 b = {trow[half * 8 + 4] * inv, trow[half * 8 + 5] * inv, trow[half * 8 + 6] * inv, trow[half * 8 + 7] * inv};
    float* o = p.out + (long)m * p.ldo + n0;
    *reinterpret_cast<float4*>(o) = a;
    *reinterpret_cast<float4*>(o + 4) = b;
  } else if (p.epi == DIA_EPI_RESID_EMIT) {
    float v[8];
    float ss = 0.f;
    if (live) {
      float* o = p.out + (long)m * p.ldo + n0;
#pragma unroll
      for (int j = 0; j < 8; ++j) v[j] = xpre[j] + trow[half * 8 + j];
      *reinterpret_cast<float4*>(o) = float4{v[0], v[1], v[2], v[3]};
      *reinterpret_cast<float4*>(o + 4) = float4{v[4], v[5], v[6], v[7]};
#pragma unroll
      for (int j = 0; j < 8; ++j) ss += v[j] * v[j];
#pragma unroll
      for (int j = 0; j < 8; ++j) v[j] = mul_rn(v[j], gpre[j]);
      emit_act8(p, m, n0, v, p.cmap);
    }
    float other = __shfl_xor(ss, 1, 64);
    if (half == 0 && live) p.ssq_out[(long)strip * p.ssq_ld + m] = ss + other;
  } else if (p.epi == DIA_EPI_SWIGLU_EMIT) {
    if (!live || half != 0) return;
    float v[8];
#pragma unroll
    for (int j = 0; j < 8; ++j) {
      float g = trow[j] * inv, u = trow[8 + j] * inv;
      v[j] = (g / (1.0f + expf(-g))) * u;
    }
    emit_act8(p, m, strip * 8, v, nullptr);
  } else {
    if (!live) return;
    if (p.strip_map) strip = p.strip_map[strip];
    long lofs = 0;
    if (p.kv_layer_strips > 0) {
      const int layer = strip / p.kv_layer_strips;
      strip -= layer * p.kv_layer_strips;
      lofs = (long)layer * p.kv_layer_stride;
    }
    int kvb = p.kv_batch_index;
    if (p.row_b) {
      kvb = p.row_b[m];
      if (kvb < 0) return;
      m -= p.seg_off[kvb];
    }
    const int nk = p.kv_heads * 8;
    if (strip < nk) {
      const int head = strip >> 3, i0 = (strip & 7) * 8 + half * 4;
      const long base = lofs + (((long)kvb * p.kv_heads + head) * p.kv_cap + m) * 128;
#pragma unroll
      for (int t = 0; t < 4; ++t) {
        const int i = i0 + t;
        const float x1 = trow[half * 8 + 2 * t] * inv, x2 = trow[half * 8 + 2 * t + 1] * inv;
        const float c = pre_cs ? xpre[t] : p.cos_t[(long)m * 64 + i], s = pre_cs ? gpre[t] : p.sin_t[(long)m * 64 + i];
        kv_store(p.kc, p.kv_dtype, base + i, x1 * c - x2 * s, p.kv_plane_stride);
        kv_store(p.kc, p.kv_dtype, base + i + 64, x1 * s + x2 * c, p.kv_plane_stride);
      }
    } else {
      const int sv = strip - nk, head = sv >> 3, d0 = (sv & 7) * 16 + half * 8;
      if (p.kv_vblocked) {
        const long hb = lofs + ((long)kvb * p.kv_heads + head) * p.kv_cap * 128;
        const long blk = hb + (long)(m >> 5) * 128 * 32 + (m & 31);
#pragma unroll
        for (int j = 0; j < 8; ++j) kv_store(p.vc, p.kv_dtype, blk + (long)(d0 + j) * 32, trow[half * 8 + j] * inv, p.kv_plane_stride);
      } else {
        const long base = lofs + (((long)kvb * p.kv_heads + head) * p.kv_cap + m) * 128 + d0;
#pragma unroll
        for (int j = 0; j < 8; ++j) kv_store(p.vc, p.kv_dtype, base + j, trow[half * 8 + j] * inv, p.kv_plane_stride);
      }
    }
  }
}

#define DIA_ROW_SHR(v, n) __builtin_bit_cast(float, __builtin_amdgcn_update_dpp(0, __builtin_bit_cast(int, (v)), 0x110 + (n), 0xF, 0xF, true))
#define DIA_ROW_SHL(v, n) __builtin_bit_cast(float, __builtin_amdgcn_update_dpp(0, __builtin_bit_cast(int, (v)), 0x100 + (n), 0xF, 0xF, true))

template <int RS, bool PF32 = false>
__device__ __forceinline__ void run_epilogue_rows(const GemmK& p, float v_tile, const float* inv_s, int tid, int strip,
                                                  float xpre1, float gpre1) {
  const int m = tid >> 4, c = tid & 15;
  const bool live = m < p.M;
  if (p.epi == DIA_EPI_RESID_EMIT) {
    const int n = strip * 16 + c;
    const float v = xpre1 + v_tile;
    if (live) p.out[(long)m * p.ldo + n] = v;
    const float sq = mul_rn(v, v);
    float acc = sq;
#pragma unroll
    for (int j = 1; j < 8; ++j) {
      const float t = DIA_ROW_SHR(acc, 1);
      if ((c & 7) == j) acc = add_rn(t, sq);
    }
    const float h0 = DIA_ROW_SHR(acc, 8);
    if (live && c == 15) p.ssq_out[(long)strip * p.ssq_ld + m] = h0 + acc;
    const float vg = mul_rn(v, gpre1);
    int cc = n;
    if (p.cmap) cc = p.cmap[n];
    if (live && cc >= 0) {
      const long off = plane_frag_off(m, cc & ~7, p.p_ktiles) + (cc & 7);
      if constexpr (PF32) {
        reinterpret_cast<float*>(p.P)[off] = vg;
      } else {
        __bf16 a, b, d;
        split3(vg, a, b, d);
        p.P[off] = *reinterpret_cast<bf16_raw*>(&a);
        p.P[p.p_plane_stride + off] = *reinterpret_cast<bf16_raw*>(&b);
        p.P[2 * p.p_plane_stride + off] = *reinterpret_cast<bf16_raw*>(&d);
      }
    }
  } else if (p.epi == DIA_EPI_SWIGLU_EMIT) {
    const float up_raw = DIA_ROW_SHL(v_tile, 8);
    if (!live || c >= 8) return;
    const float inv = inv_s[m];
    const float g = v_tile * inv, u = up_raw * inv;
    const float v = (g / (1.0f + expf(-g))) * u;
    const long off = plane_frag_off(m, strip * 8, p.p_ktiles) + c;
    if constexpr (PF32) {
      reinterpret_cast<float*>(p.P)[off] = v;
    } else {
      __bf16 a, b, d;
      split3(v, a, b, d);
      p.P[off] = *reinterpret_cast<bf16_raw*>(&a);
      p.P[p.p_plane_stride + off] = *reinterpret_cast<bf16_raw*>(&b);
      p.P[2 * p.p_plane_stride + off] = *reinterpret_cast<bf16_raw*>(&d);
    }
  } else {
    if (!live) return;
    const int s_out = p.strip_map ? p.strip_map[strip] : strip;
    p.out[(long)m * p.ldo + s_out * 16 + c] = v_tile * inv_s[m];
  }
}

template <int MT, int NW, bool RAW = false>
__device__ __forceinline__ void reduce_to_tile(const f32x4* acc, f32x4* red, float* tile, int tid, int lane, int w) {
#pragma unroll
  for (int mt = 0; mt < MT; ++mt) red[(w * MT + mt) * 64 + lane] = acc[mt];
  if constexpr (RAW) lds_barrier(); else __syncthreads();
  if (tid < MT * 64) {
    const int mt = tid >> 6;
    f32x4 s = red[(0 * MT + mt) * 64 + lane];
#pragma unroll
    for (int ww = 1; ww < NW; ++ww) {
      f32x4 t = red[(ww * MT + mt) * 64 + lane];
      s[0] += t[0]; s[1] += t[1]; s[2] += t[2]; s[3] += t[3];
    }
    const int col = lane & 15, r0 = (lane >> 4) * 4;
#pragma unroll
    for (int r = 0; r < 4; ++r) tile[(mt * 16 + r0 + r) * 17 + col] = s[r];
  }
  if constexpr (RAW) lds_barrier(); else __syncthreads();
}

__device__ __forceinline__ bool splitk_combine(const GemmK& p, float* tile, int strip, int tid, int* flag_s) {
  const int SK = gridDim.y;
  if (SK == 1) return true;
  const int ks = blockIdx.y;
#ifdef DIA_X_NOHANDOFF
  return ks == SK - 1;
#endif
  const __amdgpu_buffer_rsrc_t sr = agent_rsrc(p.sk_scratch);
  const int row = tid >> 2, c4 = (tid & 3) * 4;
  if (tid < 64) {
    const float* t = tile + row * 17 + c4;
    st4_agent(sr, (int)((((long)strip * SK + ks) * 256 + row * 16 + c4) * 4), f32x4{t[0], t[1], t[2], t[3]});
  }
  asm volatile("s_waitcnt vmcnt(0)" ::: "memory");
  __syncthreads();
  if (tid == 0) {
    const int ticket = __hip_atomic_fetch_add(p.sk_tickets + strip, 1, __ATOMIC_RELAXED, __HIP_MEMORY_SCOPE_AGENT);
    const int last = ticket == SK - 1;
    if (last) __hip_atomic_store(p.sk_tickets + strip, 0, __ATOMIC_RELAXED, __HIP_MEMORY_SCOPE_AGENT);
    *flag_s = last;
  }
  __syncthreads();
  if (!*flag_s) return false;
  if (tid < 64) {
    f32x4 v[4];
#pragma unroll
    for (int k = 0; k < 4; ++k)
      if (k < SK) v[k] = ld4_agent(sr, (int)((((long)strip * SK + k) * 256 + row * 16 + c4) * 4));
    f32x4 a = {0.f, 0.f, 0.f, 0.f};
#pragma unroll
    for (int k = 0; k < 4; ++k)
      if (k < SK) { a[0] += v[k][0]; a[1] += v[k][1]; a[2] += v[k][2]; a[3] += v[k][3]; }
    for (int k = 4; k < SK; ++k) {
      const f32x4 t = ld4_agent(sr, (int)((((long)strip * SK + k) * 256 + row * 16 + c4) * 4));
      a[0] += t[0]; a[1] += t[1]; a[2] += t[2]; a[3] += t[3];
    }
    float* t = tile + row * 17 + c4;
    t[0] = a[0]; t[1] = a[1]; t[2] = a[2]; t[3] = a[3];
  }
  __syncthreads();
  return true;
}

#ifdef DIA_DBG_STAMPS
__device__ long long g_stamps[4096 * 8];
#define STAMP(i) do { if (tid == 0) g_stamps[((blockIdx.y * gridDim.x + blockIdx.x) & 4095) * 8 + (i)] = wall_clock64(); } while (0)
#else
#define STAMP(i) do {} while (0)
#endif

constexpr int GT_MT = 4, GT_WM = 2, GT_WS = 4;
constexpr size_t gt_abuf(int kc) { return (size_t)kc * DIA_NPLANES * GT_MT * 64 * 16; }
constexpr size_t gt_smem(int kc, int nw) { return 2 * gt_abuf(kc) + sizeof(float) * (nw * 2 * 16 * 17 + 64); }

inline int fill_gemmk(const dia_gemm_args* a, GemmK& k) {
  k.A = (const bf16_raw*)a->A; k.a_plane_stride = a->a_plane_stride; k.a_ktiles = a->a_ktiles; k.M = a->M;
  k.W = (const bf16_raw*)a->W; k.KT = a->KT; k.nstrips = a->nstrips; k.epi = a->epi;
  k.ssq_in = a->ssq_in; k.ssq_in_n = a->ssq_in_n; k.ssq_ld = a->ssq_ld; k.inv_d = a->inv_d; k.eps = a->eps;
  k.out = a->out; k.ldo = a->ldo; k.gnext = a->gnext;
  k.P = (bf16_raw*)a->P; k.p_plane_stride = a->p_plane_stride; k.p_ktiles = a->p_ktiles; k.ssq_out = a->ssq_out;
  k.kc = a->kc; k.vc = a->vc; k.kv_dtype = a->kv_dtype; k.kv_heads = a->kv_heads; k.kv_cap = a->kv_cap;
  k.kv_batch_index = a->kv_batch_index; k.cos_t = a->cos_t; k.sin_t = a->sin_t; k.spw = a->spw;
  k.cmap = a->cmap; k.strip_map = a->strip_map;
  k.sk_scratch = a->sk_scratch; k.sk_tickets = a->sk_tickets; k.kv_vblocked = a->kv_vblocked;
  k.row_b = a->row_b; k.seg_off = a->seg_off;
  k.sp_blocks = (const unsigned char*)a->sp_blocks; k.sp_toff = (const unsigned int*)a->sp_toff;
  k.mz = 0;
  k.a_f32 = a->act_f32 & 1; k.p_f32 = (a->act_f32 >> 1) & 1;
  k.kv_plane_stride = a->kv_plane_stride;
  k.kv_layer_strips = a->kv_layer_strips; k.kv_layer_stride = a->kv_layer_stride;
  k.sk2_quads = dia_tune(DIA_TUNE_GEMM_2T) != 7;
  k.w_planes = a->w_planes > 1 ? a->w_planes : 1; k.w_plane_stride = (long)a->KT * a->nstrips * 512;
  return DIA_OK;
}

}

int dia_gemm_sparse24_check(const dia_gemm_args* a);
int dia_gemm_sparse24(const dia_gemm_args* a, void* stream);
int dia_gemm_mxfp8_check(const dia_gemm_args* a);
int dia_gemm_mxfp8(const dia_gemm_args* a, void* stream);
```

### dia-tts-prune_amd/csrc/tuning.cpp

```cpp
#include "tuning.hpp"
#include "errors.hpp"
#include "../../include/dia_hip.h"
#include <cstdio>
#include <cstdlib>
#include <cstring>
#include <string>

static const char* const k_names[DIA_TUNE_COUNT] = {
    "attn_nz", "attn_gpw", "attn_gpw_cross", "gemm_spw", "gemm_mz_max", "tile_min_blocks", "wo_sk", "wo_pair", "wo_nw", "wo_spw", "act_f32", "wo_diag", "gemm_2t", "gemm_zr", "seg", "seg_nb", "seg_dbg", "seg_sleep", "g2t_wgs", "ckv_merge", "mxfp8",
    "mlp_fuse", "tile_v", "blk32_kr", "blk32_ws", "no_g32", "g32_all", "g32m"};
static int g_tune[DIA_TUNE_COUNT] = {-1, -1, -1, -1, -1, -1, -1, -1, -1, -1, -1, -1, -1, -1, -1, -1, -1, -1, -1, -1, -1, -1, -1, -1, -1, -1, -1};

int dia_tune(int id) {
  dia_tuning_init_from_env();
  return (id >= 0 && id < DIA_TUNE_COUNT) ? g_tune[id] : -1;
}

extern "C" int dia_set_tuning(const char* name, int value) {
  if (!name) return dia_fail(DIA_E_ARG, "dia_set_tuning: null name");
  dia_tuning_init_from_env();
  for (int i = 0; i < DIA_TUNE_COUNT; ++i)
    if (strcmp(name, k_names[i]) == 0) { g_tune[i] = value < 0 ? -1 : value; return DIA_OK; }
  return dia_fail(DIA_E_ARG, "dia_set_tuning: unknown knob");
}

extern "C" int dia_get_tuning(const char* name) {
  if (!name) return -1;
  dia_tuning_init_from_env();
  for (int i = 0; i < DIA_TUNE_COUNT; ++i)
    if (strcmp(name, k_names[i]) == 0) return g_tune[i];
  return -1;
}

void dia_tuning_init_from_env() {
  static bool done = false;
  if (done) return;
  done = true;
  const char* e = getenv("DIA_TUNE");
  if (!e) return;
  std::string s(e);
  size_t pos = 0;
  while (pos < s.size()) {
    size_t end = s.find(',', pos);
    if (end == std::string::npos) end = s.size();
    const std::string item = s.substr(pos, end - pos);
    const size_t eq = item.find('=');
    if (eq == std::string::npos) {
      if (!item.empty()) fprintf(stderr, "dia_hip: DIA_TUNE item '%s' ignored (expected name=value)\n", item.c_str());
    } else if (dia_set_tuning(item.substr(0, eq).c_str(), atoi(item.c_str() + eq + 1)) != DIA_OK) {
      fprintf(stderr, "dia_hip: DIA_TUNE knob '%s' unknown, ignored\n", item.substr(0, eq).c_str());
    }
    pos = end + 1;
  }
}
```

### dia-tts-prune_amd/csrc/tuning.hpp

```cpp
#pragma once

enum dia_tune_id {
  DIA_TUNE_ATTN_NZ = 0,
  DIA_TUNE_ATTN_GPW,
  DIA_TUNE_ATTN_GPW_CROSS,
  DIA_TUNE_GEMM_SPW,
  DIA_TUNE_GEMM_MZ_MAX,
  DIA_TUNE_TILE_MIN_BLOCKS,
  DIA_TUNE_WO_SK,
  DIA_TUNE_WO_PAIR,
  DIA_TUNE_WO_NW,
  DIA_TUNE_WO_SPW,
  DIA_TUNE_ACT_F32,
  DIA_TUNE_WO_DIAG,
  DIA_TUNE_GEMM_2T,
  DIA_TUNE_GEMM_ZR,
  DIA_TUNE_SEG,
  DIA_TUNE_SEG_NB,
  DIA_TUNE_SEG_DBG,
  DIA_TUNE_SEG_SLEEP,
  DIA_TUNE_G2T_WGS,
  DIA_TUNE_CKV_MERGE,
  DIA_TUNE_MXFP8,
  DIA_TUNE_MLP_FUSE,
  DIA_TUNE_TILE_V,
  DIA_TUNE_BLK32_KR,
  DIA_TUNE_BLK32_WS,
  DIA_TUNE_NO_G32,
  DIA_TUNE_G32_ALL,
  DIA_TUNE_G32M,
  DIA_TUNE_COUNT
};

int dia_tune(int id);
void dia_tuning_init_from_env();
```

### dia-tts-prune_amd/dia_hip/binding.py

```python

from __future__ import annotations

import ctypes as C
import os
from typing import Optional

_HERE = os.path.dirname(os.path.abspath(__file__))
LIB_PATH = os.environ.get("DIA_HIP_LIB") or os.path.join(_HERE, "libdia_hip.so")

ABI_VERSION = 8
KV_F32, KV_BF16, KV_BF16X2 = 0, 1, 2
EPI_SCALE_STORE, EPI_RESID_EMIT, EPI_SWIGLU_EMIT, EPI_CROSSKV = 0, 1, 2, 3
W_DENSE, W_SPARSE24, W_MXFP8 = 0, 1, 2
ATTN_SELF, ATTN_CROSS, ATTN_ENC = 0, 1, 2

EXPORTS = (
    "dia_last_error", "dia_abi_version", "dia_device_count", "dia_set_tuning", "dia_get_tuning", "dia_has_experiments", "dia_gemm", "dia_gemm_timed", "dia_mlp_fused", "dia_mlp_fused_timed", "dia_engine_mlp_fused", "dia_attn", "dia_attn_scratch_floats", "dia_enc_kv_prep", "dia_enc_attn", "dia_dec_prefill_embed", "dia_dec_prefill_kv", "dia_dec_prefill_attn",
    "dia_embed_text", "dia_embed_tokens", "dia_sample", "dia_slot_admit", "dia_slot_retire", "dia_prefetch", "dia_engine_create", "dia_engine_destroy",
    "dia_engine_decode", "dia_engine_set_prefetch", "dia_engine_step_logits_only", "dia_engine_profile_step", "dia_engine_time_step", "dia_timed_kernel_name", "dia_engine_launches_per_step", "dia_mxfp8_classes",
    "dia_seg_mlp", "dia_seg_workspace_bytes", "dia_seg_workspace_control_bytes", "dia_seg_slots", "dia_seg_supported", "dia_seg_error",
)


class DiaHipError(RuntimeError):
    pass


class GemmArgs(C.Structure):
    _fields_ = [
        ("A", C.c_void_p), ("a_plane_stride", C.c_int64), ("a_ktiles", C.c_int32), ("M", C.c_int32),
        ("W", C.c_void_p), ("KT", C.c_int32), ("nstrips", C.c_int32), ("epi", C.c_int32), ("nw", C.c_int32),
        ("ssq_in", C.c_void_p), ("ssq_in_n", C.c_int32), ("ssq_ld", C.c_int32), ("inv_d", C.c_float), ("eps", C.c_float),
        ("out", C.c_void_p), ("ldo", C.c_int32), ("spw", C.c_int32),
        ("gnext", C.c_void_p), ("P", C.c_void_p), ("p_plane_stride", C.c_int64), ("p_ktiles", C.c_int32), ("_pad1", C.c_int32),
        ("ssq_out", C.c_void_p),
        ("kc", C.c_void_p), ("vc", C.c_void_p), ("kv_dtype", C.c_int32), ("kv_heads", C.c_int32), ("kv_cap", C.c_int32),
        ("kv_batch_index", C.c_int32), ("cos_t", C.c_void_p), ("sin_t", C.c_void_p),
        ("cmap", C.c_void_p), ("strip_map", C.c_void_p),
        ("sk_scratch", C.c_void_p), ("sk_tickets", C.c_void_p), ("sk", C.c_int32), ("kv_vblocked", C.c_int32),
        ("row_b", C.c_void_p), ("seg_off", C.c_void_p), ("sk_scratch_floats", C.c_int64),
        ("sp_blocks", C.c_void_p), ("sp_toff", C.c_void_p),
        ("act_f32", C.c_int32), ("w_planes", C.c_int32), ("kv_plane_stride", C.c_int64),
        ("w_layout", C.c_int32), ("kv_layer_strips", C.c_int32), ("kv_layer_stride", C.c_int64),
        ("w_format", C.c_int32), ("_pad2", C.c_int32),
    ]


class AttnArgs(C.Structure):
    _fields_ = [
        ("mode", C.c_int32), ("kv_dtype", C.c_int32), ("n_kv_heads", C.c_int32), ("group", C.c_int32),
        ("n_rows", C.c_int32), ("kv_cap", C.c_int32),
        ("q", C.c_void_p), ("ldq", C.c_int32), ("q_off", C.c_int32), ("k_off", C.c_int32), ("v_off", C.c_int32),
        ("kc", C.c_void_p), ("vc", C.c_void_p), ("cur", C.c_void_p), ("len", C.c_void_p),
        ("enc_len", C.c_int32), ("rope_rows", C.c_int32), ("cos_t", C.c_void_p), ("sin_t", C.c_void_p),
        ("P", C.c_void_p), ("p_plane_stride", C.c_int64), ("p_ktiles", C.c_int32), ("_pad1", C.c_int32),
        ("scratch", C.c_void_p), ("tickets", C.c_void_p), ("head_map", C.c_void_p),
        ("v_blocked", C.c_int32), ("act_f32", C.c_int32), ("kv_plane_stride", C.c_int64),
    ]


class EncAttnArgs(C.Structure):
    _fields_ = [
        ("qkv", C.c_void_p), ("ldq", C.c_int32), ("q_off", C.c_int32), ("k_off", C.c_int32), ("v_off", C.c_int32),
        ("heads", C.c_int32), ("rows", C.c_int32),
        ("row_b", C.c_void_p), ("seg_off", C.c_void_p), ("seg_len", C.c_void_p), ("cos_t", C.c_void_p), ("sin_t", C.c_void_p),
        ("kp", C.c_void_p), ("vp", C.c_void_p), ("P", C.c_void_p), ("p_plane_stride", C.c_int64), ("p_ktiles", C.c_int32),
        ("_pad0", C.c_int32),
    ]


class DecPrefillArgs(C.Structure):
    _fields_ = [
        ("row_seg", C.c_void_p), ("seg_off", C.c_void_p), ("seg_len", C.c_void_p), ("seg_row", C.c_void_p),
        ("rows", C.c_int32), ("_pad0", C.c_int32),
        ("tokens", C.c_void_p), ("T", C.c_int32), ("C", C.c_int32), ("V", C.c_int32), ("D", C.c_int32),
        ("emb", C.c_void_p), ("g", C.c_void_p), ("x", C.c_void_p),
        ("P", C.c_void_p), ("p_plane_stride", C.c_int64), ("p_ktiles", C.c_int32), ("ssq_ld", C.c_int32),
        ("ssq", C.c_void_p),
        ("q", C.c_void_p), ("ldq", C.c_int32), ("q_off", C.c_int32), ("k_off", C.c_int32), ("v_off", C.c_int32),
        ("q_heads", C.c_int32), ("kv_heads", C.c_int32), ("kv_cap", C.c_int32), ("causal", C.c_int32),
        ("kc", C.c_void_p), ("vc", C.c_void_p), ("cos_t", C.c_void_p), ("sin_t", C.c_void_p), ("text_len", C.c_void_p),
    ]


class EmbedArgs(C.Structure):
    _fields_ = [
        ("tokens", C.c_void_p), ("cur", C.c_void_p),
        ("B", C.c_int32), ("T", C.c_int32), ("C", C.c_int32), ("V", C.c_int32), ("D", C.c_int32), ("act_f32", C.c_int32),
        ("emb", C.c_void_p), ("g", C.c_void_p), ("x", C.c_void_p), ("P", C.c_void_p),
        ("p_plane_stride", C.c_int64), ("p_ktiles", C.c_int32), ("ssq_ld", C.c_int32), ("ssq", C.c_void_p),
        ("cmap", C.c_void_p),
        ("slots", C.c_void_p), ("n_slots", C.c_int32), ("_pad0", C.c_int32),
    ]


class SampleArgs(C.Structure):
    _fields_ = [
        ("logits", C.c_void_p), ("ld_logits", C.c_int32), ("B", C.c_int32), ("T", C.c_int32), ("C", C.c_int32),
        ("V", C.c_int32), ("max_tokens", C.c_int32),
        ("cfg_scale", C.c_float), ("temperature", C.c_float), ("top_p", C.c_float), ("top_k", C.c_int32),
        ("eos", C.c_int32), ("pad", C.c_int32), ("bos", C.c_int32), ("max_delay", C.c_int32),
        ("ignore_eos", C.c_int32), ("teacher", C.c_int32),
        ("delay", C.c_void_p), ("noise", C.c_void_p), ("noise_steps", C.c_int32), ("_pad0", C.c_int32),
        ("tokens", C.c_void_p), ("pred", C.c_void_p), ("cur", C.c_void_p), ("fsm", C.c_void_p),
        ("first_step", C.c_void_p), ("embed", EmbedArgs),
        ("slot_cfg_scale", C.c_void_p), ("slot_temperature", C.c_void_p), ("slot_top_p", C.c_void_p),
        ("slot_top_k", C.c_void_p), ("slot_max_tokens", C.c_void_p),
    ]


SLOTS_PER_CALL = 64


class SlotAdmitArgs(C.Structure):
    _fields_ = [
        ("B", C.c_int32), ("T", C.c_int32), ("C", C.c_int32), ("S", C.c_int32), ("max_delay", C.c_int32), ("n", C.c_int32),
        ("slot", C.POINTER(C.c_int32)), ("text_len", C.POINTER(C.c_int32)), ("first_step", C.POINTER(C.c_int32)),
        ("prefix_rows", C.POINTER(C.c_int32)), ("max_tokens", C.POINTER(C.c_int32)),
        ("cfg_scale", C.POINTER(C.c_float)), ("temperature", C.POINTER(C.c_float)), ("top_p", C.POINTER(C.c_float)),
        ("top_k", C.POINTER(C.c_int32)),
        ("prefix", C.c_void_p), ("prefix_ld", C.c_int32), ("_pad0", C.c_int32),
        ("tokens", C.c_void_p), ("pred", C.c_void_p), ("cur", C.c_void_p), ("fsm", C.c_void_p),
        ("d_first_step", C.c_void_p), ("d_text_len", C.c_void_p),
        ("slot_cfg_scale", C.c_void_p), ("slot_temperature", C.c_void_p), ("slot_top_p", C.c_void_p),
        ("slot_top_k", C.c_void_p), ("slot_max_tokens", C.c_void_p),
    ]


class DecLayer(C.Structure):
    _fields_ = [
        ("w_qkv", C.c_void_p), ("w_o", C.c_void_p), ("w_cq", C.c_void_p), ("w_co", C.c_void_p),
        ("w_wi", C.c_void_p), ("w_wo", C.c_void_p), ("w_wo_diag", C.c_void_p),
        ("g_sa", C.c_void_p), ("g_ca", C.c_void_p), ("g_mlp", C.c_void_p),
        ("k_self", C.c_void_p), ("v_self", C.c_void_p), ("k_cross", C.c_void_p), ("v_cross", C.c_void_p),
        ("kt_qkv", C.c_int32), ("ns_qkv", C.c_int32), ("kt_o", C.c_int32), ("ns_o", C.c_int32),
        ("kt_cq", C.c_int32), ("ns_cq", C.c_int32), ("kt_co", C.c_int32), ("ns_co", C.c_int32),
        ("kt_wi", C.c_int32), ("ns_wi", C.c_int32), ("kt_wo", C.c_int32), ("ns_wo", C.c_int32),
        ("cmap_ca", C.c_void_p), ("cmap_mlp", C.c_void_p), ("cmap_next", C.c_void_p),
        ("smap_qkv", C.c_void_p), ("smap_cq", C.c_void_p), ("hmap_self", C.c_void_p), ("hmap_cross", C.c_void_p),
        ("w_qkv_24", C.c_void_p), ("w_o_24", C.c_void_p), ("w_cq_24", C.c_void_p), ("w_co_24", C.c_void_p),
        ("w_wi_24", C.c_void_p), ("w_wo_24", C.c_void_p),
        ("w_qkv_f8", C.c_void_p), ("w_o_f8", C.c_void_p), ("w_cq_f8", C.c_void_p), ("w_co_f8", C.c_void_p),
        ("w_wi_f8", C.c_void_p), ("w_wo_f8", C.c_void_p),
    ]


class EngineDesc(C.Structure):
    _fields_ = [
        ("n_layer", C.c_int32), ("D", C.c_int32), ("F", C.c_int32), ("q_heads", C.c_int32), ("kv_heads", C.c_int32),
        ("cq_heads", C.c_int32), ("C", C.c_int32), ("V", C.c_int32),
        ("B", C.c_int32), ("T", C.c_int32), ("S", C.c_int32), ("kv_dtype", C.c_int32),
        ("rows_pad", C.c_int32), ("ld_logits", C.c_int32), ("eps", C.c_float), ("v_blocked", C.c_int32),
        ("layers", C.POINTER(DecLayer)), ("w_logits", C.c_void_p), ("kt_logits", C.c_int32), ("ns_logits", C.c_int32),
        ("g_final", C.c_void_p),
        ("x", C.c_void_p), ("planes_x", C.c_void_p), ("planes_a", C.c_void_p), ("planes_h", C.c_void_p),
        ("ssq", C.c_void_p), ("qkv", C.c_void_p), ("qc", C.c_void_p), ("logits", C.c_void_p),
        ("cos_t", C.c_void_p), ("sin_t", C.c_void_p), ("text_len", C.c_void_p),
        ("sk_scratch", C.c_void_p), ("sk_tickets", C.c_void_p),
        ("attn_scratch", C.c_void_p), ("attn_tickets", C.c_void_p), ("sk_scratch_floats", C.c_int64), ("mlp_barrier", C.c_void_p),
        ("act_f32", C.c_int32), ("w_planes", C.c_int32),
        ("sample", SampleArgs),
        ("seg_w", C.POINTER(C.c_void_p)), ("seg_ws", C.c_void_p),
        ("kv_plane_self", C.c_int64), ("kv_plane_cross", C.c_int64),
        ("w_logits_24", C.c_void_p), ("w_logits_f8", C.c_void_p),
    ]


class SegArgs(C.Structure):
    _fields_ = [
        ("a_in", C.c_void_p), ("a_ktiles", C.c_int32), ("M", C.c_int32),
        ("W", C.c_void_p), ("nslots", C.c_int32), ("has_qkv", C.c_int32), ("D", C.c_int32), ("F", C.c_int32),
        ("x", C.c_void_p), ("ldx", C.c_int32), ("_pad0", C.c_int32),
        ("g_mlp", C.c_void_p), ("g_next", C.c_void_p), ("qkv_out", C.c_void_p), ("ldq", C.c_int32), ("_pad1", C.c_int32),
        ("planes_x", C.c_void_p), ("xkt", C.c_int32), ("_pad2", C.c_int32), ("ssq", C.c_void_p), ("ssq_ld", C.c_int32), ("eps", C.c_float),
        ("ws", C.c_void_p), ("timeout_us", C.c_int32), ("_pad3", C.c_int32), ("stamps", C.c_void_p),
    ]


_lib: Optional[C.CDLL] = None


def lib() -> C.CDLL:
    global _lib
    if _lib is not None:
        return _lib
    if not os.path.isfile(LIB_PATH):
        raise DiaHipError(
            f"{LIB_PATH} is missing: build it with `python __graft_entry__.py` or "
            f"`make -C dia-tts-prune_amd/csrc` (hipcc --offload-arch=gfx950). There is no CPU fallback."
        )
    import torch

    try:
        L = C.CDLL(LIB_PATH)
    except OSError as e:
        raise DiaHipError(f"cannot load {LIB_PATH}: {e}") from e
    for name in EXPORTS:
        if not hasattr(L, name):
            raise DiaHipError(f"{LIB_PATH} does not export {name}; rebuild it")
    L.dia_last_error.restype = C.c_char_p
    L.dia_abi_version.restype = C.c_int
    if L.dia_abi_version() != ABI_VERSION:
        raise DiaHipError(f"ABI mismatch: library {L.dia_abi_version()} vs binding {ABI_VERSION}")
    L.dia_set_tuning.argtypes = [C.c_char_p, C.c_int]
    L.dia_get_tuning.argtypes = [C.c_char_p]
    L.dia_has_experiments.restype = C.c_int
    L.dia_gemm.argtypes = [C.POINTER(GemmArgs), C.c_void_p]
    L.dia_gemm_timed.argtypes = [C.POINTER(GemmArgs), C.c_void_p, C.POINTER(C.c_float)]
    L.dia_mlp_fused.argtypes = [C.POINTER(GemmArgs), C.POINTER(GemmArgs), C.c_void_p, C.c_void_p]
    L.dia_mlp_fused_timed.argtypes = [C.POINTER(GemmArgs), C.POINTER(GemmArgs), C.c_void_p, C.c_void_p, C.POINTER(C.c_float)]
    L.dia_engine_mlp_fused.argtypes = [C.c_void_p]
    L.dia_attn.argtypes = [C.POINTER(AttnArgs), C.c_void_p]
    L.dia_attn_scratch_floats.argtypes = [C.c_int, C.c_int, C.c_int]
    L.dia_enc_attn.argtypes = [C.POINTER(EncAttnArgs), C.c_void_p]
    for fn in (L.dia_dec_prefill_embed, L.dia_dec_prefill_kv, L.dia_dec_prefill_attn):
        fn.argtypes = [C.POINTER(DecPrefillArgs), C.c_void_p]
    L.dia_enc_kv_prep.argtypes = [C.c_void_p, C.c_int, C.c_int, C.c_int, C.c_int, C.c_int, C.c_int,
                                  C.c_void_p, C.c_void_p, C.c_void_p, C.c_void_p, C.c_void_p]
    L.dia_embed_text.argtypes = [C.c_void_p, C.c_int, C.c_void_p, C.c_int, C.c_void_p, C.c_void_p, C.c_void_p,
                                 C.c_int64, C.c_int, C.c_void_p, C.c_int, C.c_void_p, C.c_void_p]
    L.dia_embed_tokens.argtypes = [C.POINTER(EmbedArgs), C.c_void_p]
    L.dia_sample.argtypes = [C.POINTER(SampleArgs), C.c_void_p]
    L.dia_slot_admit.argtypes = [C.POINTER(SlotAdmitArgs), C.c_void_p]
    L.dia_slot_retire.argtypes = [C.POINTER(SlotAdmitArgs), C.c_void_p]
    L.dia_prefetch.argtypes = [C.c_void_p, C.c_int64, C.c_int, C.c_void_p]
    L.dia_engine_create.argtypes = [C.POINTER(EngineDesc), C.c_void_p, C.POINTER(C.c_void_p)]
    L.dia_engine_destroy.argtypes = [C.c_void_p]
    L.dia_engine_decode.argtypes = [C.c_void_p, C.c_int, C.c_int]
    L.dia_engine_step_logits_only.argtypes = [C.c_void_p]
    L.dia_engine_set_prefetch.argtypes = [C.c_void_p, C.c_int]
    L.dia_engine_launches_per_step.argtypes = [C.c_void_p]
    L.dia_engine_profile_step.argtypes = [C.c_void_p, C.POINTER(C.c_float), C.c_int]
    L.dia_engine_time_step.argtypes = [C.c_void_p, C.POINTER(C.c_float), C.POINTER(C.c_float), C.c_int]
    L.dia_timed_kernel_name.argtypes = [C.c_int]
    L.dia_timed_kernel_name.restype = C.c_char_p
    L.dia_mxfp8_classes.argtypes = [C.c_int]
    L.dia_seg_mlp.argtypes = [C.POINTER(SegArgs), C.c_void_p]
    L.dia_seg_workspace_bytes.restype = C.c_int64
    L.dia_seg_workspace_control_bytes.restype = C.c_int64
    L.dia_seg_slots.argtypes = [C.c_int]
    L.dia_seg_supported.argtypes = [C.c_int, C.c_int, C.c_int, C.c_int]
    L.dia_seg_error.argtypes = [C.c_void_p, C.c_void_p]
    _lib = L
    return L


def set_tuning(name: str, value: int) -> None:
    check(lib().dia_set_tuning(name.encode(), int(value)), f"dia_set_tuning({name})")


def get_tuning(name: str) -> int:
    return int(lib().dia_get_tuning(name.encode()))


def mxfp8_mask(rows: int) -> int:
    return int(lib().dia_mxfp8_classes(int(rows)))


def has_experiments() -> bool:
    return bool(lib().dia_has_experiments())


def check(rc: int, what: str = "") -> None:
    if rc != 0:
        msg = lib().dia_last_error()
        raise DiaHipError(f"{what} failed ({rc}): {msg.decode() if msg else ''}")


def ptr(t) -> int:
    return 0 if t is None else t.data_ptr()
```

### dia-tts-prune_amd/dia_hip/engine.py

```python

from __future__ import annotations

import ctypes as C
from dataclasses import dataclass
from functools import partial
from typing import Dict, List, Optional, Sequence

import numpy as np
import torch

from . import binding as hb
from . import compact as cpt
from . import layout as lay
from .config import DiaConfig
from .pruning import is_2of4
from .quant import is_mxfp8

HEAD_DIM = 128
_TILERS = {1: lay.tile_weight, 2: lay.tile_weight_bf16x2, 3: lay.tile_weight_planes}


def _ceil(v: int, m: int) -> int:
    return (v + m - 1) // m * m

# ... 273 lines not shown
            wi3 = self._dev(sd, p + "mlp.wi_fused.weight")
            qn = None
            if i + 1 < d.n_layer:
                pn = f"decoder.layers.{i + 1}."
                qn = torch.cat([self._dev(sd, pn + f"self_attention.{n_}_proj.weight").reshape(D, -1) for n_ in "qkv"], dim=1)
            self.seg_layers.append(lay.seg_ring(self._dev(sd, p + "cross_attention.o_proj.weight").reshape(-1, D), wi3[:, 0, :], wi3[:, 1, :],
                                                self._dev(sd, p + "mlp.wo.weight"), qn))
            del wi3, qn

    def ckv_all(self) -> Optional[TiledW]:
        ts = [L["ckv"] for L in self.dec_layers]
        if self.weight_planes != 1 or not ts or any(t.kt != ts[0].kt for t in ts):
            return None
        p0 = ts[0].t.data_ptr()
        for t in ts:
            if t.t.data_ptr() != p0:
                return None
            p0 += t.nbytes
        n = sum(t.t.numel() for t in ts)
        base = ts[0].t
        whole = torch.empty(0, dtype=base.dtype, device=base.device).set_(base.untyped_storage(), base.storage_offset(), (n,))
        return TiledW(whole, ts[0].kt, sum(t.ns for t in ts))

    def tensors(self) -> List[torch.Tensor]:
        out: List[torch.Tensor] = [self.enc_emb]
        for L in self.enc_layers:
            out += [L["g_sa"], L["g_mlp"], L["qkv"].t, L["o"].t, L["wi"].t, L["wo"].t]
            out += [L[k] for k in ("cmap_mlp", "cmap_next") if L[k] is not None]
        out += [self.enc_norm, self.dec_emb]
        for L in self.dec_layers:
            out += [L["g_sa"], L["g_ca"], L["g_mlp"]] + [L[k].t for k in DEC_MATS]
            out += [L[k] for k in ("cmap_ca", "cmap_mlp", "cmap_next", "smap_qkv", "smap_cq", "smap_ckv", "hmap_self", "hmap_cross", "wo_diag")
                    if L[k] is not None]
        out += [L["ckv"].t for L in self.dec_layers]
        if self.smap_ckv_all is not None:
            out.append(self.smap_ckv_all)
        out += [self.dec_norm, self.logits.t, self.cos_t, self.sin_t]
        out += [t for t in (self.cmap_first, self.enc_cmap_first) if t is not None]
        out += self.seg_layers
        if self.sparse == "2:4":
            for L in self.dec_layers:
                out += [L[k + "24"].t for k in DEC_MATS]
            out.append(self.logits24.t)
        if self.quant == "mxfp8":
            for L in self.dec_layers:
                out += [L[k + "f8"].t for k in DEC_MATS]
            out.append(self.logits_f8.t)
        return out

    def pack_flat(self):
        ts = self.tensors()
        offs, tot = [], 0
        for t in ts:
            offs.append(tot)
            tot += (t.numel() * t.element_size() + 255) // 256 * 256
        flat = torch.zeros(tot, dtype=torch.uint8, device=self.device)
        for t, o in zip(ts, offs):
            nb = t.numel() * t.element_size()
            v = flat[o: o + nb].view(t.dtype).view(t.shape)
            v.copy_(t)
            t.data = v
        self.flat = flat

    @classmethod
    def empty_like_config(cls, cfg: DiaConfig, device: torch.device, weight_planes: int = 1, seg: str = "off",
                          sparse: str = "off", quant: str = "off") -> "DeviceWeights":
        from .weights import param_shapes
        sd = {k: torch.zeros(shp, dtype=torch.float32, device=device) for k, shp in param_shapes(cfg).items()}
        return cls(cfg, sd, device, compact="off", weight_planes=weight_planes, seg=seg, sparse=sparse, quant=quant)

    def prefill_weight_bytes(self) -> int:
        n = sum(L[k].nbytes for L in self.enc_layers for k in ("qkv", "o", "wi", "wo"))
        return n + sum(L["ckv"].nbytes for L in self.dec_layers)

    def decode_weight_bytes(self, rows: int = 2) -> int:
        every = self.sparse == "2:4" and rows <= 4
        f8 = hb.mxfp8_mask(rows) if self.quant == "mxfp8" else 0

        def w(L, k):
            if f8 >> STEP_MATS.index(k) & 1:
                return L[k + "f8"].nbytes
            return L[k + "24"].nbytes if every else L[k].nbytes
        n = self.logits_f8.nbytes if f8 >> STEP_MATS.index("logits") & 1 else (self.logits24.nbytes if every else self.logits.nbytes)
        for L in self.dec_layers:
            n += sum(w(L, k) for k in DEC_MATS)
        return n


@dataclass
class Request:
    text_ids: np.ndarray
    seed: Optional[int] = None
    max_tokens: Optional[int] = None
    cfg_scale: float = 3.0
    temperature: float = 1.3
    top_p: float = 0.95
    top_k: int = 35
    audio_prompt: Optional[np.ndarray] = None


@dataclass
class UtteranceResult:
    tokens: np.ndarray
    codes: np.ndarray
    last_step: int
    preds: np.ndarray
    text_len: int


class DecodeSession:

    def __init__(self, w: DeviceWeights, text_ids: Sequence[np.ndarray], *, kv_dtype: str = "bf16",
                 max_tokens: Optional[int] = None, cfg_scale: float = 3.0, temperature: float = 1.3,
                 top_p: float = 0.95, top_k: int = 35, seeds: Optional[Sequence[Optional[int]]] = None,
                 noise: Optional[torch.Tensor] = None, ignore_eos: bool = False,
                 teacher_tokens: Optional[Sequence[np.ndarray]] = None, stream: Optional[torch.cuda.Stream] = None,
                 s_cap: Optional[int] = None, audio_prompts: Optional[Sequence[Optional[np.ndarray]]] = None,
                 prompt_prefill: str = "auto", attention: str = "auto", _slotted: bool = False):
        if prompt_prefill not in ("auto", "replay") or attention not in ("auto", "valu"):
            raise ValueError("prompt_prefill must be 'auto' or 'replay', attention 'auto' or 'valu'")
        self.prompt_prefill = prompt_prefill
        cfg, dev = w.cfg, w.device
        self.w, self.cfg, self.dev = w, cfg, dev
        d, da = cfg.model.decoder, cfg.data
        self.B = B = len(text_ids)
        self.R = 2 * B
        self.rows_pad = _ceil(self.R, 16)
        self.T = da.audio_length
        self.C, self.V, self.D, self.F = da.channels, cfg.model.tgt_vocab_size, d.n_embd, d.n_hidden
        self.max_tokens = self.T if max_tokens is None else int(max_tokens)
        if not (2 <= self.max_tokens <= self.T):
            raise ValueError(f"max_tokens must be in [2, {self.T}]")
        self.kv_code = {"f32": hb.KV_F32, "float32": hb.KV_F32, "bf16": hb.KV_BF16, "bfloat16": hb.KV_BF16, "bf16x2": hb.KV_BF16X2}[kv_dtype]
        if self.kv_code == hb.KV_BF16X2 and attention == "valu":
            raise ValueError("kv_dtype 'bf16x2' is served by the MFMA attention kernel only")
        self.v_blocked = int(self.kv_code in (hb.KV_BF16, hb.KV_BF16X2) and attention != "valu")
        kvt = torch.float32 if self.kv_code == hb.KV_F32 else torch.bfloat16
        self.kv_planes = 2 if self.kv_code == hb.KV_BF16X2 else 1
        self.stream = stream if stream is not None else torch.cuda.Stream(device=dev)
        self.lens = [int(len(t)) for t in text_ids]
        self.S = s_cap if s_cap is not None else max(32, _ceil(max(self.lens + [1]), 32))
        if self.S > da.text_length and s_cap is None:
            self.S = da.text_length
        self.text_ids = [np.asarray(t, dtype=np.int32) for t in text_ids]
        self.teacher = teacher_tokens is not None
        self.ignore_eos = ignore_eos
        md = max(da.delay_pattern)
        self.max_delay = md

        z = lambda *s, dt=torch.float32: torch.zeros(*s, dtype=dt, device=dev)
        mt = self.rows_pad // 16
        self.xkt, self.akt, self.hkt = self.D // 32, max(d.gqa_query_heads, d.cross_query_heads) * HEAD_DIM // 32, self.F // 32
        self.x = z(self.rows_pad, self.D)
        t_ = hb.get_tuning("act_f32")
        self.act_f32 = int(t_ != 0)
        self.seg = bool(self.R <= 4 and w.seg_layers and self.act_f32 and hb.get_tuning("seg") == 1)
        self.seg_ws = None
        if self.seg:
            self.seg_ws = torch.zeros(int(hb.lib().dia_seg_workspace_bytes()), dtype=torch.uint8, device=dev)
        self.planes_x = z(3, mt, self.xkt, 64, 8, dt=torch.bfloat16)
        self.planes_a = z(3, mt, self.akt, 64, 8, dt=torch.bfloat16)
        self.planes_h = z(3, mt, self.hkt, 64, 8, dt=torch.bfloat16)
        self.ssq = z(self.D // 8, self.rows_pad)
        self.nqkv = (d.gqa_query_heads + 2 * d.kv_heads) * HEAD_DIM
        self.qkv = z(self.rows_pad, self.nqkv)
        self.qc = z(self.rows_pad, d.cross_query_heads * HEAD_DIM)
        self.ld_logits = w.logits.ns * 16
        self.logits = z(self.rows_pad, self.ld_logits)
        pl = (self.kv_planes,) if self.kv_planes > 1 else ()
        self.k_self = [z(*pl, self.R, d.kv_heads, self.T, HEAD_DIM, dt=kvt) for _ in range(d.n_layer)]
        self.v_self = [z(*pl, self.R, d.kv_heads, self.T, HEAD_DIM, dt=kvt) for _ in range(d.n_layer)]
        self.k_cross_all = z(d.n_layer, *pl, B, d.cross_query_heads, self.S, HEAD_DIM, dt=kvt)
        self.v_cross_all = z(d.n_layer, *pl, B, d.cross_query_heads, self.S, HEAD_DIM, dt=kvt)
        self.k_cross = [self.k_cross_all[i] for i in range(d.n_layer)]
        self.v_cross = [self.v_cross_all[i] for i in range(d.n_layer)]
        self.kv_plane_self = self.R * d.kv_heads * self.T * HEAD_DIM if self.kv_planes > 1 else 0
        self.kv_plane_cross = B * d.cross_query_heads * self.S * HEAD_DIM if self.kv_planes > 1 else 0
        self.text_len = torch.tensor(self.lens, dtype=torch.int32, device=dev)
        nsc = max(hb.lib().dia_attn_scratch_floats(self.R, d.kv_heads, self.T),
                  hb.lib().dia_attn_scratch_floats(B, d.cross_query_heads, self.S))
        self.attn_scratch = z(max(nsc, 1))
        self.attn_tickets = z(max(self.R * d.kv_heads, B * d.cross_query_heads), dt=torch.int32)
        ns_max = max([self.D // 16, w.logits.ns] + [DL[k].ns for DL in w.dec_layers for k in DEC_MATS])
        n_scr = max((self.D // 16) * 4 * 512, ns_max * 2 * 512 if 16 < self.R <= 32 else 0)
        if 16 < self.R <= 128:
            n_scr = max(n_scr, 2 * -(-self.R // 32) * (self.D // 16) * 4 * 256)
        if 16 < self.R <= 32:
            n_scr = max([n_scr, w.logits.ns * -(-w.logits.kt // 8) * 512] +
                        [DL[k].ns * -(-DL[k].kt // 8) * 512 for DL in w.dec_layers for k in DEC_MATS])
        self.sk_scratch = z(n_scr)
        self.sk_tickets = z(max(ns_max, 8 * (self.D // 16)), dt=torch.int32)
        self.mlp_barrier = z(2, dt=torch.int32)

        from .tokens import delayed_prefill
        tok = np.full((B, self.T, self.C), -1, dtype=np.int32)
        self.first_steps = []
        for b in range(B):
            pr = None if audio_prompts is None else audio_prompts[b]
            if pr is not None:
                pr = np.asarray(pr)
                if pr.ndim == 3 and pr.shape[0] == 1:
                    pr = pr[0]
                if pr.ndim != 2 or pr.shape[1] != self.C:
                    raise ValueError(f"Unexpected audio_prompt shape: {pr.shape}. Expected [T, C] or [1, T, C].")
            prefill, pstep = delayed_prefill(cfg, pr)
            if prefill.shape[0] > self.T:
                raise ValueError(f"audio prompt of {pstep - 1} frames does not fit audio_length {self.T}")
            tok[b, : prefill.shape[0]] = prefill
            self.first_steps.append(int(pstep))
        if self.teacher:
            for b in range(B):
                tt = np.asarray(teacher_tokens[b], dtype=np.int32)
                tok[b, : tt.shape[0]] = tt
        self.prefill_step = 1
        self.first_step = torch.tensor(self.first_steps, dtype=torch.int32, device=dev)
        self.tokens = torch.from_numpy(tok).to(dev)
        self.pred = torch.full((B, self.T, self.C), -1, dtype=torch.int32, device=dev)
        self.cur = torch.full((B,), 1, dtype=torch.int32, device=dev)
        fsm = np.zeros((B, 8), dtype=np.int32)
        fsm[:, 1] = -1
        fsm[:, 2] = md
        self.fsm = torch.from_numpy(fsm).to(dev)
        self.delay = torch.tensor(list(da.delay_pattern), dtype=torch.int32, device=dev)

        self.noise_steps = self.max_tokens - 1
        self._noise_rows = 0
        self._issued = 0
        self._gens = None
        if temperature != 0.0:
            if noise is not None:
                nz = noise.to(torch.float32)
                if tuple(nz.shape) != (B, self.noise_steps, self.C, self.V):
                    raise ValueError(f"noise must be [B,{self.noise_steps},{self.C},{self.V}]")
                self.noise = nz.to(dev)
                self._noise_rows = self.noise_steps
            else:
                self.noise = torch.empty(B, self.noise_steps, self.C, self.V, dtype=torch.float32, device=dev)
                self._gens = []
                for b in range(B):
                    g = torch.Generator()
                    sd = None if seeds is None else seeds[b]
                    if sd is None:
                        g.seed()
                    else:
                        g.manual_seed(int(sd))
                    self._gens.append(g)
        else:
            self.noise = None
            self._noise_rows = self.noise_steps

        self.sample_params = dict(cfg_scale=float(cfg_scale), temperature=float(temperature), top_p=float(top_p),
                                  top_k=int(top_k or 0))
        self._pinned: List[torch.Tensor] = []
        self.slotted = bool(_slotted)
        if self.slotted:
            self._init_slots()
        self._engine = C.c_void_p()
        self._build_engine()
        self.prefilled = self.slotted

    def _embed_args(self) -> hb.EmbedArgs:
        e = hb.EmbedArgs()
        e.tokens, e.cur = hb.ptr(self.tokens), hb.ptr(self.cur)
        e.B, e.T, e.C, e.V, e.D = self.B, self.T, self.C, self.V, self.D
        e.emb, e.g, e.x = hb.ptr(self.w.dec_emb), hb.ptr(self.w.dec_layers[0]["g_sa"]), hb.ptr(self.x)
        e.P, e.p_plane_stride, e.p_ktiles = _plane_set(self.planes_x, self.xkt)
        e.ssq_ld, e.ssq = self.rows_pad, hb.ptr(self.ssq)
        e.cmap = hb.ptr(self.w.cmap_first)
        e.act_f32 = self.act_f32
        return e

    def _sample_args(self) -> hb.SampleArgs:
        da = self.cfg.data
        s = hb.SampleArgs()
        s.logits, s.ld_logits, s.B, s.T, s.C, s.V = hb.ptr(self.logits), self.ld_logits, self.B, self.T, self.C, self.V
        s.max_tokens = self.max_tokens
        s.cfg_scale, s.temperature, s.top_p = (self.sample_params[k] for k in ("cfg_scale", "temperature", "top_p"))
        s.top_k = self.sample_params["top_k"]
        s.eos, s.pad, s.bos, s.max_delay = da.audio_eos_value, da.audio_pad_value, da.audio_bos_value, self.max_delay
        s.ignore_eos, s.teacher = int(self.ignore_eos), int(self.teacher)
        s.delay, s.noise, s.noise_steps = hb.ptr(self.delay), hb.ptr(self.noise), self.noise_steps
        s.tokens, s.pred, s.cur, s.fsm = hb.ptr(self.tokens), hb.ptr(self.pred), hb.ptr(self.cur), hb.ptr(self.fsm)
        s.first_step = hb.ptr(self.first_step) if self.slotted or any(f != 1 for f in self.first_steps) else None
        s.embed = self._embed_args()
        if self.slotted:
            s.slot_cfg_scale, s.slot_temperature, s.slot_top_p = (hb.ptr(self.slot_f32[i]) for i in range(3))
            s.slot_top_k, s.slot_max_tokens = hb.ptr(self.slot_i32[0]), hb.ptr(self.slot_i32[1])
        return s

    def _build_engine(self):
        d = self.cfg.model.decoder
        w = self.w
        n = d.n_layer
        self._layers = (hb.DecLayer * n)()
        for i, L in enumerate(w.dec_layers):
            dl = self._layers[i]
            for f in DEC_MATS:
                setattr(dl, "w_" + f, hb.ptr(L[f].t))
                setattr(dl, "kt_" + f, L[f].kt)
                setattr(dl, "ns_" + f, L[f].ns)
                sp = L[f + "24"]
                setattr(dl, "w_" + f + "_24", hb.ptr(sp.t) if sp is not None else None)
                f8 = L[f + "f8"]
                setattr(dl, "w_" + f + "_f8", hb.ptr(f8.t) if f8 is not None else None)
            dl.g_sa, dl.g_ca, dl.g_mlp = hb.ptr(L["g_sa"]), hb.ptr(L["g_ca"]), hb.ptr(L["g_mlp"])
            dl.k_self, dl.v_self = hb.ptr(self.k_self[i]), hb.ptr(self.v_self[i])
            dl.k_cross, dl.v_cross = hb.ptr(self.k_cross[i]), hb.ptr(self.v_cross[i])
            for f in ("cmap_ca", "cmap_mlp", "cmap_next", "smap_qkv", "smap_cq", "hmap_self", "hmap_cross"):
                setattr(dl, f, hb.ptr(L[f]))
            dl.w_wo_diag = hb.ptr(L["wo_diag"])
        ed = hb.EngineDesc()
        ed.n_layer, ed.D, ed.F = n, self.D, self.F
        ed.q_heads, ed.kv_heads, ed.cq_heads = d.gqa_query_heads, d.kv_heads, d.cross_query_heads
        ed.C, ed.V, ed.B, ed.T, ed.S = self.C, self.V, self.B, self.T, self.S
        ed.kv_dtype, ed.rows_pad, ed.ld_logits = self.kv_code, self.rows_pad, self.ld_logits
        ed.v_blocked = self.v_blocked
        ed.kv_plane_self, ed.kv_plane_cross = self.kv_plane_self, self.kv_plane_cross
        ed.eps = float(self.cfg.model.normalization_layer_epsilon)
        ed.layers = C.cast(self._layers, C.POINTER(hb.DecLayer))
        ed.w_logits, ed.kt_logits, ed.ns_logits = hb.ptr(w.logits.t), w.logits.kt, w.logits.ns
        ed.w_logits_24 = hb.ptr(w.logits24.t) if w.logits24 is not None else None
        ed.w_logits_f8 = hb.ptr(w.logits_f8.t) if w.logits_f8 is not None else None
        ed.g_final = hb.ptr(w.dec_norm)
        ed.x, ed.planes_x, ed.planes_a, ed.planes_h = hb.ptr(self.x), hb.ptr(self.planes_x), hb.ptr(self.planes_a), hb.ptr(self.planes_h)
        ed.ssq, ed.qkv, ed.qc, ed.logits = hb.ptr(self.ssq), hb.ptr(self.qkv), hb.ptr(self.qc), hb.ptr(self.logits)
        ed.cos_t, ed.sin_t, ed.text_len = hb.ptr(w.cos_t), hb.ptr(w.sin_t), hb.ptr(self.text_len)
        ed.attn_scratch, ed.attn_tickets = hb.ptr(self.attn_scratch), hb.ptr(self.attn_tickets)
        ed.sk_scratch, ed.sk_tickets = hb.ptr(self.sk_scratch), hb.ptr(self.sk_tickets)
        ed.sk_scratch_floats = self.sk_scratch.numel()
        ed.mlp_barrier = hb.ptr(self.mlp_barrier)
        ed.act_f32 = self.act_f32
        ed.w_planes = w.weight_planes
        ed.sample = self._sample_args()
        if self.seg:
            self._seg_w = (C.c_void_p * n)(*[hb.ptr(t) for t in w.seg_layers])
            ed.seg_w = C.cast(self._seg_w, C.POINTER(C.c_void_p))
            ed.seg_ws = hb.ptr(self.seg_ws)
        self._desc = ed
        hb.check(hb.lib().dia_engine_create(C.byref(ed), C.c_void_p(self.stream.cuda_stream), C.byref(self._engine)),
                 "dia_engine_create")

    def close(self):
        if self._engine:
            eng, self._engine = self._engine, C.c_void_p()
            self.stream.synchronize()
            hb.check(hb.lib().dia_engine_destroy(eng), "dia_engine_destroy")

    def __del__(self):
        try:
            self.close()
        except Exception:
            pass

    def prefill(self, keep_encoder_out: bool = False):
        L = hb.lib()
        st = C.c_void_p(self.stream.cuda_stream)
        self.enc_out = [None] * self.B
        self._encode(list(enumerate(self.text_ids)), keep_encoder_out)
        with torch.cuda.stream(self.stream):
            if self._prompt_prefill_batched():
                self._prompt_prefill(st)
            ea = self._embed_args()
            hb.check(L.dia_embed_tokens(C.byref(ea), st), "dia_embed_tokens")
        self.prefilled = True

    def _encode(self, pairs, keep_encoder_out: bool = False):
        L = hb.lib()
        cfg, w, dev = self.cfg, self.w, self.dev
        e, d = cfg.model.encoder, cfg.model.decoder
        st = C.c_void_p(self.stream.cuda_stream)
        E, Fe = e.n_embd, e.n_hidden
        eps = float(cfg.model.normalization_layer_epsilon)
        utt = [int(b) for b, _ in pairs]
        lens = [int(len(t)) for _, t in pairs]
        offs, tot, row_seg = pack_segments(lens)
        with torch.cuda.stream(self.stream):
            if tot > 0:
                Mp, mt = tot, tot // 16
                Hmax = max(EL["heads"] for EL in w.enc_layers)
                ekt = E // 32
                akt = max(max(1, Hmax * HEAD_DIM // 32), max(EL["o"].a_kt for EL in w.enc_layers))
                hkt = max(EL["wo"].a_kt for EL in w.enc_layers)
                nq_max = 3 * Hmax * HEAD_DIM
                shapes = [((Mp, E), torch.float32), ((3, mt, ekt, 64, 8), torch.bfloat16), ((3, mt, akt, 64, 8), torch.bfloat16),
                          ((3, mt, hkt, 64, 8), torch.bfloat16), ((E // 16, Mp), torch.float32), ((Mp, nq_max), torch.float32),
                          ((3, Hmax, Mp, HEAD_DIM), torch.bfloat16), ((3, Hmax, Mp, HEAD_DIM), torch.bfloat16)]
                sizes = [_ceil(int(np.prod(sh)) * (4 if dt == torch.float32 else 2), 256) for sh, dt in shapes]
                ws = torch.zeros(sum(sizes), dtype=torch.uint8, device=dev)
                views, o_ = [], 0
                for (sh, dt), nb in zip(shapes, sizes):
                    n_el = int(np.prod(sh))
                    views.append(ws[o_: o_ + n_el * (4 if dt == torch.float32 else 2)].view(dt).view(*sh))
                    o_ += nb
                x, px, pa, ph, ssq, qkv, kp, vp = views
                live = [i for i in range(len(pairs)) if lens[i] > 0]
                id_off, n_ids = {}, 0
                for i in live:
                    id_off[i] = n_ids
                    n_ids += _ceil(lens[i], 4)
                tab = np.zeros((Mp + 2 * _ceil(self.B, 4) + n_ids,), dtype=np.int32)
                tab[:Mp] = np.where(row_seg >= 0, np.asarray(utt, dtype=np.int32)[np.maximum(row_seg, 0)], -1)
                o_so, o_sl = Mp, Mp + _ceil(self.B, 4)
                tab[o_so + np.asarray(utt)] = offs
                tab[o_sl + np.asarray(utt)] = lens
                o_id = Mp + 2 * _ceil(self.B, 4)
                for i in live:
                    tab[o_id + id_off[i]: o_id + id_off[i] + lens[i]] = pairs[i][1]
                self._pf_tab_host = torch.from_numpy(tab).pin_memory()
                self._pinned.append(self._pf_tab_host)
                tab_d = self._pf_tab_host.to(dev, non_blocking=True)
                row_b, seg_off, seg_len = tab_d[:Mp], tab_d[o_so: o_so + self.B], tab_d[o_sl: o_sl + self.B]

                def rows(t, i, width):
                    return t.data_ptr() + offs[i] * width * 4

                def planes_at(P, i, kt_):
                    return P.data_ptr() + (offs[i] // 16) * kt_ * 512 * 2

                for i in live:
                    ids = tab_d[o_id + id_off[i]: o_id + id_off[i] + lens[i]]
                    hb.check(L.dia_embed_text(hb.ptr(ids), lens[i], hb.ptr(w.enc_emb), E, hb.ptr(w.enc_layers[0]["g_sa"]),
                                              rows(x, i, E), planes_at(px, i, ekt), px[0].numel(), ekt,
                                              ssq.data_ptr() + offs[i] * 4, Mp, hb.ptr(w.enc_cmap_first), st), "dia_embed_text")

                gemm = partial(_launch_gemm, st, M=Mp, ssq=ssq, ssq_ld=Mp, width=E, eps=eps, w_planes=w.weight_planes)

                def cross_kv(kc, vc):
                    return (hb.ptr(kc), hb.ptr(vc), self.kv_code, d.cross_query_heads, self.S, 0, self.v_blocked, self.kv_plane_cross,
                            hb.ptr(w.cos_t), hb.ptr(w.sin_t))

                for i, EL in enumerate(w.enc_layers):
                    Hl = EL["heads"]
                    nq = 3 * Hl * HEAD_DIM
                    if Hl > 0:
                        gemm(px, ekt, EL["qkv"], hb.EPI_SCALE_STORE, ssq_in=True, out=qkv, ldo=nq)
                        ea_ = hb.EncAttnArgs()
                        ea_.qkv, ea_.ldq, ea_.q_off, ea_.k_off, ea_.v_off = hb.ptr(qkv), nq, 0, Hl * HEAD_DIM, 2 * Hl * HEAD_DIM
                        ea_.heads, ea_.rows = Hl, Mp
                        ea_.row_b, ea_.seg_off, ea_.seg_len = hb.ptr(row_b), hb.ptr(seg_off), hb.ptr(seg_len)
                        ea_.cos_t, ea_.sin_t, ea_.kp, ea_.vp = hb.ptr(w.cos_t), hb.ptr(w.sin_t), hb.ptr(kp), hb.ptr(vp)
                        ea_.P, ea_.p_plane_stride, ea_.p_ktiles = _plane_set(pa, akt)
                        hb.check(L.dia_enc_attn(C.byref(ea_), st), "dia_enc_attn")
                        gemm(pa, akt, EL["o"], hb.EPI_RESID_EMIT, out=x, ldo=E, gnext=EL["g_mlp"], P=px, p_kt=ekt, ssq_out=True,
                             cmap=EL["cmap_mlp"])
                    else:
                        raise hb.DiaHipError("encoder layer with every attention head pruned is not supported")
                    gemm(px, ekt, EL["wi"], hb.EPI_SWIGLU_EMIT, ssq_in=True, P=ph, p_kt=hkt)
                    gnext = w.enc_layers[i + 1]["g_sa"] if i + 1 < len(w.enc_layers) else w.enc_norm
                    wo_sk = None
                    kt_wo, ns_wo = EL["wo"].kt, EL["wo"].ns
                    if (16 < Mp <= 128 and kt_wo % 16 == 0 and kt_wo // 2 <= 64 and w.weight_planes == 1 and EL["cmap_next"] is None
                            and self.sk_scratch.numel() >= mt * ns_wo * 2 * 256 and self.sk_tickets.numel() >= mt * ns_wo):
                        wo_sk = (2, self.sk_scratch, self.sk_tickets)
                    gemm(ph, hkt, EL["wo"], hb.EPI_RESID_EMIT, out=x, ldo=E, gnext=gnext, P=px, p_kt=ekt, ssq_out=True,
                         cmap=EL["cmap_next"], sk=wo_sk)
                ckv_all = w.ckv_all() if hb.get_tuning("ckv_merge") != 0 else None
                if ckv_all is not None:
                    gemm(px, ekt, ckv_all, hb.EPI_CROSSKV, ssq_in=True, kv=cross_kv(self.k_cross_all, self.v_cross_all),
                         strip_map=w.smap_ckv_all, row_map=(row_b, seg_off), kv_layers=(d.cross_query_heads * 16, self.k_cross[0].numel()))
                else:
                    for i, DL in enumerate(w.dec_layers):
                        gemm(px, ekt, DL["ckv"], hb.EPI_CROSSKV, ssq_in=True, kv=cross_kv(self.k_cross[i], self.v_cross[i]),
                             strip_map=DL["smap_ckv"], row_map=(row_b, seg_off))
                if keep_encoder_out:
                    for i in live:
                        Lb, o = lens[i], offs[i]
                        inv = torch.rsqrt(ssq[:, o: o + Lb].sum(dim=0) / E + eps)
                        self.enc_out[utt[i]] = (x[o: o + Lb] * inv[:, None] * w.enc_norm[None, :]).clone()

    def _prompt_prefill_batched(self) -> bool:
        return (any(f > 2 for f in self.first_steps) and self.v_blocked == 1 and self.kv_code == hb.KV_BF16 and not self.w.compacted and not self.teacher
                and self.prompt_prefill != "replay" and self.w.weight_planes == 1)

    def _prompt_prefill(self, st):
        L = hb.lib()
        cfg, w, dev = self.cfg, self.w, self.dev
        d = cfg.model.decoder
        D, F = self.D, self.F
        QH, KVH, CH = d.gqa_query_heads, d.kv_heads, d.cross_query_heads
        eps = float(cfg.model.normalization_layer_epsilon)
        segs = []
        for b, fs in enumerate(self.first_steps):
            if fs > 2:
                segs += [(2 * b, fs - 1), (2 * b + 1, fs - 1)]
        offs, Mp, rs = pack_segments([n for _, n in segs])
        mt = Mp // 16
        i32 = lambda a: torch.tensor(a, dtype=torch.int32, device=dev)
        row_seg = torch.from_numpy(rs).to(dev)
        seg_off, seg_len, seg_row = i32(offs), i32([n for _, n in segs]), i32([r for r, _ in segs])
        z = lambda *sh, dt=torch.float32: torch.zeros(*sh, dtype=dt, device=dev)
        xkt, akt, hkt = D // 32, max(QH, CH) * HEAD_DIM // 32, F // 32
        x = z(Mp, D)
        px, pa, ph = (z(3, mt, kt_, 64, 8, dt=torch.bfloat16) for kt_ in (xkt, akt, hkt))
# ... 389 lines not shown
```

### include/dia_hip.h

```cpp
#ifndef DIA_HIP_H
#define DIA_HIP_H

#include <stdint.h>

#ifdef __cplusplus
extern "C" {
#endif

#define DIA_ABI_VERSION 8

#define DIA_OK 0
#define DIA_E_ARG (-1)
#define DIA_E_HIP (-2)
#define DIA_E_STATE (-3)

#define DIA_KV_F32 0
#define DIA_KV_BF16 1
#define DIA_KV_BF16X2 2

#define DIA_EPI_SCALE_STORE 0
#define DIA_EPI_RESID_EMIT 1
#define DIA_EPI_SWIGLU_EMIT 2
#define DIA_EPI_CROSSKV 3

#define DIA_W_DENSE 0
#define DIA_W_SPARSE24 1
#define DIA_W_MXFP8 2

#define DIA_ATTN_SELF 0
#define DIA_ATTN_CROSS 1
#define DIA_ATTN_ENC 2

const char* dia_last_error(void);
int dia_abi_version(void);
int dia_device_count(void);
int dia_set_tuning(const char* name, int value);
int dia_get_tuning(const char* name);
int dia_has_experiments(void);


typedef struct {
  const void* A;
  int64_t a_plane_stride;
  int32_t a_ktiles;
  int32_t M;
  const void* W;
  int32_t KT;
  int32_t nstrips;
  int32_t epi;
  int32_t nw;
  const float* ssq_in;
  int32_t ssq_in_n;
  int32_t ssq_ld;
  float inv_d;
  float eps;
  float* out;
  int32_t ldo;
  int32_t spw;
  const float* gnext;
  void* P;
  int64_t p_plane_stride;
  int32_t p_ktiles;
  int32_t _pad1;
  float* ssq_out;
  void* kc;
  void* vc;
  int32_t kv_dtype;
  int32_t kv_heads;
  int32_t kv_cap;
  int32_t kv_batch_index;
  const float* cos_t;
  const float* sin_t;
  const int32_t* cmap;
  const int32_t* strip_map;
  float* sk_scratch;
  int32_t* sk_tickets;
  int32_t sk;
  int32_t kv_vblocked;
  const int32_t* row_b;
  const int32_t* seg_off;
  int64_t sk_scratch_floats;
  const void* sp_blocks;
  const uint32_t* sp_toff;
  int32_t act_f32;
  int32_t w_planes;
  int64_t kv_plane_stride;
  int32_t w_layout;
  int32_t kv_layer_strips;
  int64_t kv_layer_stride;
  int32_t w_format;
  int32_t _pad2;
} dia_gemm_args;
int dia_gemm(const dia_gemm_args* a, void* stream);
int dia_mlp_fused(const dia_gemm_args* wi, const dia_gemm_args* wo, int32_t* barrier, void* stream);
int dia_mlp_fused_timed(const dia_gemm_args* wi, const dia_gemm_args* wo, int32_t* barrier, void* stream, float* ms_out);


int dia_gemm_timed(const dia_gemm_args* a, void* stream, float* ms_out);

typedef struct {
  int32_t mode;
  int32_t kv_dtype;
  int32_t n_kv_heads;
  int32_t group;
  int32_t n_rows;
  int32_t kv_cap;
  const float* q;
  int32_t ldq;
  int32_t q_off;
  int32_t k_off;
  int32_t v_off;
  void* kc;
  void* vc;
  const int32_t* cur;
  const int32_t* len;
  int32_t enc_len;
  int32_t rope_rows;
  const float* cos_t;
  const float* sin_t;
  void* P;
  int64_t p_plane_stride;
  int32_t p_ktiles;
  int32_t _pad1;
  float* scratch;
  int32_t* tickets;
  const int32_t* head_map;
  int32_t v_blocked;
  int32_t act_f32;
  int64_t kv_plane_stride;
} dia_attn_args;
int dia_attn(const dia_attn_args* a, void* stream);
int dia_attn_scratch_floats(int n_rows, int n_kv_heads, int kv_cap);

typedef struct {
  const float* qkv;
  int32_t ldq, q_off, k_off, v_off;
  int32_t heads;
  int32_t rows;
  const int32_t* row_b;
  const int32_t* seg_off;
  const int32_t* seg_len;
  const float* cos_t;
  const float* sin_t;
  void* kp;
  void* vp;
  void* P;
  int64_t p_plane_stride;
  int32_t p_ktiles;
  int32_t _pad0;
} dia_enc_attn_args;
int dia_enc_attn(const dia_enc_attn_args* a, void* stream);

typedef struct {
  const int32_t* row_seg; const int32_t* seg_off; const int32_t* seg_len; const int32_t* seg_row;
  int32_t rows;
  int32_t _pad0;
  const int32_t* tokens;
  int32_t T, C, V, D;
  const float* emb;
  const float* g;
  float* x;
  void* P; int64_t p_plane_stride; int32_t p_ktiles; int32_t ssq_ld;
  float* ssq;
  const float* q;
  int32_t ldq, q_off, k_off, v_off;
  int32_t q_heads, kv_heads, kv_cap;
  int32_t causal;
  void* kc; void* vc;
  const float* cos_t; const float* sin_t;
  const int32_t* text_len;
} dia_dec_prefill_args;
int dia_dec_prefill_embed(const dia_dec_prefill_args* a, void* stream);
int dia_dec_prefill_kv(const dia_dec_prefill_args* a, void* stream);
int dia_dec_prefill_attn(const dia_dec_prefill_args* a, void* stream);

int dia_enc_kv_prep(const float* qkv, int ldq, int k_off, int v_off, int heads, int L, int cap,
                    const float* cos_t, const float* sin_t, float* kc, float* vc, void* stream);

int dia_embed_text(const int32_t* ids, int L, const float* table, int D, const float* g, float* x,
                   void* P, int64_t p_plane_stride, int p_ktiles, float* ssq, int ssq_ld, const int32_t* cmap, void* stream);

typedef struct {
  const int32_t* tokens;
  const int32_t* cur;
  int32_t B, T, C, V, D;
  int32_t act_f32;
  const float* emb;
  const float* g;
  float* x;
  void* P;
  int64_t p_plane_stride;
  int32_t p_ktiles;
  int32_t ssq_ld;
  float* ssq;
  const int32_t* cmap;
  const int32_t* slots;
  int32_t n_slots;
  int32_t _pad0;
} dia_embed_args;
int dia_embed_tokens(const dia_embed_args* a, void* stream);

typedef struct {
  const float* logits;
  int32_t ld_logits;
  int32_t B;
  int32_t T;
  int32_t C;
  int32_t V;
  int32_t max_tokens;
  float cfg_scale, temperature, top_p;
  int32_t top_k;
  int32_t eos, pad, bos;
  int32_t max_delay;
  int32_t ignore_eos;
  int32_t teacher;
  const int32_t* delay;
  const float* noise;
  int32_t noise_steps;
  int32_t _pad0;
  int32_t* tokens;
  int32_t* pred;
  int32_t* cur;
  int32_t* fsm;
  const int32_t* first_step;
  dia_embed_args embed;
  const float* slot_cfg_scale;
  const float* slot_temperature;
  const float* slot_top_p;
  const int32_t* slot_top_k;
  const int32_t* slot_max_tokens;
} dia_sample_args;
int dia_sample(const dia_sample_args* a, void* stream);

#define DIA_SLOTS_PER_CALL 64
typedef struct {
  int32_t B, T, C, S;
  int32_t max_delay;
  int32_t n;
  const int32_t* slot;
  const int32_t* text_len;
  const int32_t* first_step;
  const int32_t* prefix_rows;
  const int32_t* max_tokens;
  const float* cfg_scale;
  const float* temperature;
  const float* top_p;
  const int32_t* top_k;
  const int32_t* prefix;
  int32_t prefix_ld;
  int32_t _pad0;
  int32_t* tokens;
  int32_t* pred;
  int32_t* cur;
  int32_t* fsm;
  int32_t* d_first_step;
  int32_t* d_text_len;
  float* slot_cfg_scale;
  float* slot_temperature;
  float* slot_top_p;
  int32_t* slot_top_k;
  int32_t* slot_max_tokens;
} dia_slot_admit_args;
int dia_slot_admit(const dia_slot_admit_args* a, void* stream);
int dia_slot_retire(const dia_slot_admit_args* a, void* stream);

int dia_prefetch(const void* ptr, int64_t nbytes, int nblocks, void* stream);


typedef struct {
  const float* a_in;
  int32_t a_ktiles;
  int32_t M;
  const void* W;
  int32_t nslots;
  int32_t has_qkv;
  int32_t D, F;
  float* x;
  int32_t ldx;
  const float* g_mlp;
  const float* g_next;
  float* qkv_out;
  int32_t ldq;
  float* planes_x;
  int32_t xkt;
  float* ssq;
  int32_t ssq_ld;
  float eps;
  void* ws;
  int32_t timeout_us;
  void* stamps;
} dia_seg_args;
int dia_seg_mlp(const dia_seg_args* a, void* stream);
int64_t dia_seg_workspace_bytes(void);
int64_t dia_seg_workspace_control_bytes(void);
int32_t dia_seg_slots(int with_qkv);
int dia_seg_supported(int D, int F, int attn_width, int nqkv);
int dia_seg_error(const void* ws, void* stream);

typedef struct {
  const void *w_qkv, *w_o, *w_cq, *w_co, *w_wi, *w_wo;
  const void* w_wo_diag;
  const float *g_sa, *g_ca, *g_mlp;
  void *k_self, *v_self;
  void *k_cross, *v_cross;
  int32_t kt_qkv, ns_qkv, kt_o, ns_o, kt_cq, ns_cq, kt_co, ns_co, kt_wi, ns_wi, kt_wo, ns_wo;
  const int32_t* cmap_ca;
  const int32_t* cmap_mlp;
  const int32_t* cmap_next;
  const int32_t* smap_qkv;
  const int32_t* smap_cq;
  const int32_t* hmap_self;
  const int32_t* hmap_cross;
  const void *w_qkv_24, *w_o_24, *w_cq_24, *w_co_24, *w_wi_24, *w_wo_24;
  const void *w_qkv_f8, *w_o_f8, *w_cq_f8, *w_co_f8, *w_wi_f8, *w_wo_f8;
} dia_dec_layer;

typedef struct {
  int32_t n_layer, D, F, q_heads, kv_heads, cq_heads, C, V;
  int32_t B;
  int32_t T;
  int32_t S;
  int32_t kv_dtype;
  int32_t rows_pad;
  int32_t ld_logits;
  float eps;
  int32_t v_blocked;
  const dia_dec_layer* layers;
  const void* w_logits;
  int32_t kt_logits, ns_logits;
  const float* g_final;
  float* x;
  void* planes_x;
  void* planes_a;
  void* planes_h;
  float* ssq;
  float* qkv;
  float* qc;
  float* logits;
  const float* cos_t;
  const float* sin_t;
  const int32_t* text_len;
  float* sk_scratch;
  int32_t* sk_tickets;
  float* attn_scratch;
  int32_t* attn_tickets;
  int64_t sk_scratch_floats;
  int32_t* mlp_barrier;
  int32_t act_f32;
  int32_t w_planes;
  dia_sample_args sample;
  const void* const* seg_w;
  void* seg_ws;
  int64_t kv_plane_self, kv_plane_cross;
  const void* w_logits_24;
  const void* w_logits_f8;
} dia_engine_desc;

enum dia_step_mat { DIA_MAT_QKV, DIA_MAT_O, DIA_MAT_CQ, DIA_MAT_CO, DIA_MAT_WI, DIA_MAT_WO, DIA_MAT_LOGITS, DIA_MAT_COUNT };

typedef struct dia_engine dia_engine;
int dia_engine_create(const dia_engine_desc* d, void* stream, dia_engine** out);
int dia_engine_destroy(dia_engine* e);
int dia_engine_mlp_fused(const dia_engine* e);
int dia_engine_decode(dia_engine* e, int n_steps, int use_graph);
int dia_engine_set_prefetch(dia_engine* e, int lookahead);
int dia_engine_step_logits_only(dia_engine* e);
int dia_engine_profile_step(dia_engine* e, float* ms_per_launch, int cap);
int dia_engine_time_step(dia_engine* e, float* ms_per_kernel, float* interval_ms, int cap);
const char* dia_timed_kernel_name(int i);
int dia_mxfp8_classes(int rows);
int dia_engine_launches_per_step(const dia_engine* e);

#ifdef __cplusplus
}
#endif
#endif
```

Baseline: 1028 frames/s.

## Defer MLP down-projection residual merge into the next layer's QKV GEMV

The wo (down-projection) GEMV now writes its two split-K partial slices to scratch and skips the split-K combine and residual epilogue. The following QKV (or logits) GEMV reads both slices plus the old residual and rebuilds x, the RMSNorm sum of squares and the normalized input inside its own prologue. x ping-pongs between two buffers so writeback does not race with readers. This removes the split-K ticket combine and one residual round trip per layer, in exchange for redundant merge work in every consumer workgroup and many added eligibility conditions.

```diff
diff --git a/dia-tts-prune_amd/csrc/engine.hip b/dia-tts-prune_amd/csrc/engine.hip
--- a/dia-tts-prune_amd/csrc/engine.hip
+++ b/dia-tts-prune_amd/csrc/engine.hip
@@ -18,6 +18,8 @@
   bool seg = false;
   std::vector<const void*> seg_w;
   int mlp_fused = -1;
+  int wo_defer = -1;
+  float* x_alt = nullptr;
   std::vector<hipEvent_t> prof;
   int pf_lookahead = 0;
   bool pf_capturing = false;
@@ -169,6 +171,9 @@
     else { g.sk_scratch = d.sk_scratch; g.sk_tickets = d.sk_tickets; }
   };
   bool wo_pair = false;
+  bool defer = false;
+  const int64_t slice_floats = (int64_t)d.rows_pad * d.D;
+  auto xbuf = [&](int l) { return (defer && (l & 1)) ? e->x_alt : d.x; };
   auto step_gemm = [&](int l, int m) {
     const step_mat_row& r = STEP_MATS[m];
     const dia_dec_layer* L = l < d.n_layer ? &e->layers[l] : nullptr;
@@ -185,7 +190,7 @@
       case OUT_QC: g.out = d.qc; g.ldo = d.cq_heads * 128; g.strip_map = L->smap_cq; break;
       case OUT_LOGITS: g.out = d.logits; g.ldo = d.ld_logits; break;
       case OUT_X:
-        g.out = d.x; g.ldo = d.D; g.ssq_out = d.ssq; g.cmap = L->*r.cmap;
+        g.out = xbuf(l); g.ldo = d.D; g.ssq_out = d.ssq; g.cmap = L->*r.cmap;
         g.gnext = r.gnext ? L->*r.gnext : ((l + 1 < d.n_layer) ? e->layers[l + 1].g_sa : d.g_final);
         break;
     }
@@ -198,8 +203,34 @@
     }
     sparse24(g, w.w24);
     mxfp8(g, w.wf8, m);
+    if (defer && (m == DIA_MAT_LOGITS || (m == DIA_MAT_QKV && l > 0))) g.gnext = L ? L->g_sa : d.g_final;
     return g;
   };
+  auto step_defer = [&](int l, int m) {
+    dia_wo_defer_args w = {};
+    if (!defer || !(m == DIA_MAT_WO || m == DIA_MAT_LOGITS || (m == DIA_MAT_QKV && l > 0))) return w;
+    w.nslices = 2; w.slices = d.sk_scratch; w.slice_stride = slice_floats;
+    if (m == DIA_MAT_WO) { w.defer = 1; return w; }
+    w.xold = xbuf(l - 1); w.ldx = d.D;
+    w.xnew = l < d.n_layer ? xbuf(l) : nullptr;
+    return w;
+  };
+  if (R <= 4 && F && d.w_planes <= 1 && !seg && !diag && e->wo_defer != 0 && dia_tune(DIA_TUNE_WO_DEFER) != 0 && dia_tune(DIA_TUNE_MLP_FUSE) <= 0 &&
+      e->x_alt && d.sk_scratch && d.D == 2048 && (d.sk_scratch_floats > 0 ? d.sk_scratch_floats : (int64_t)(d.D / 16) * 4 * 512) >= 2 * slice_floats) {
+    const auto al16 = [](const void* q) { return (reinterpret_cast<uintptr_t>(q) & 15) == 0; };
+    bool ok = al16(d.x) && al16(e->x_alt) && al16(d.sk_scratch) && slice_floats % 4 == 0 && slice_floats >= (int64_t)xkt * 512 && d.D % 4 == 0 &&
+              dia_tune(DIA_TUNE_GEMM_SPW) <= 0;
+    for (int l = 0; l < d.n_layer && ok; ++l) {
+      const dia_gemm_args go = step_gemm(l, DIA_MAT_WO), gc = step_gemm(l + 1, l + 1 < d.n_layer ? DIA_MAT_QKV : DIA_MAT_LOGITS);
+      const float* gcons = l + 1 < d.n_layer ? e->layers[l + 1].g_sa : d.g_final;
+      const int spw = gc.spw > 0 ? gc.spw : (gc.nstrips >= 1024 ? 4 : (gc.nstrips > 512 ? (gc.nstrips + 255) / 256 : 1));
+      ok = go.w_format == DIA_W_DENSE && go.w_layout == 0 && go.sk == 2 && go.KT == 256 && !go.cmap && go.nw == 0 && go.nstrips == d.D / 16 &&
+           (go.act_f32 & 3) == 3 && go.gnext && go.nstrips * 16 <= go.p_ktiles * 32 &&
+           gc.w_format == DIA_W_DENSE && gc.w_layout == 0 && gc.KT == 64 && gc.nw == 0 && gc.sk <= 1 && !gc.cmap && (gc.act_f32 & 1) && gcons && al16(gcons) &&
+           (l + 1 == d.n_layer || (gc.nstrips + spw - 1) / spw >= d.D / 16);
+    }
+    defer = ok;
+  }
 
   int n = 0;
   bool fused = false;
@@ -243,7 +274,17 @@
         fused = rc == DIA_OK;
         e->mlp_fused = fused ? 1 : 0;
       }
-      if (!fused) rc = dia_gemm(&g, st);
+      const dia_wo_defer_args wd = step_defer(l, what);
+      if (!fused) rc = wd.nslices ? dia_gemm_wo_deferred(&g, &wd, st, nullptr) : dia_gemm(&g, st);
+      if (rc == DIA_OK && wd.defer) e->wo_defer = 1;
+      if (rc == DIA_E_ARG && wd.nslices) {
+        const bool first = what == DIA_MAT_WO && l == 0 && e->wo_defer < 0;
+        e->wo_defer = 0;
+        if (!first) return rc;
+        defer = false;
+        g = step_gemm(l, what);
+        rc = dia_gemm(&g, st);
+      }
       if (what == DIA_MAT_WO && rc == DIA_E_ARG && g.sk > 1) {
         g.sk = 1;
         if (!wo_pair) { g.sk_scratch = nullptr; g.sk_tickets = nullptr; }
@@ -453,6 +494,13 @@
   return dia_prefetch_launch(ptr, (long)nbytes, nblocks, (hipStream_t)stream);
 }
 
+extern "C" int dia_engine_set_x_alt(dia_engine* e, float* x_alt) {
+  if (!e) return dia_fail(DIA_E_ARG, "dia_engine_set_x_alt: null engine");
+  if (e->exec || e->wo_defer == 1) return dia_fail(DIA_E_STATE, "dia_engine_set_x_alt: a step has already been issued or captured");
+  e->x_alt = x_alt;
+  return DIA_OK;
+}
+
 extern "C" int dia_engine_set_prefetch(dia_engine* e, int lookahead) {
   if (!e || lookahead < 0) return dia_fail(DIA_E_ARG, "dia_engine_set_prefetch: bad argument");
   if (e->exec) return dia_fail(DIA_E_STATE, "dia_engine_set_prefetch: the step graph is already captured");
diff --git a/dia-tts-prune_amd/csrc/gemm.hip b/dia-tts-prune_amd/csrc/gemm.hip
--- a/dia-tts-prune_amd/csrc/gemm.hip
+++ b/dia-tts-prune_amd/csrc/gemm.hip
@@ -109,7 +109,7 @@
 }
 
 
-template <int NW, int KPW, int RS, bool MULTI, bool AF32 = false, bool PF32 = false, bool W2 = false>
+template <int NW, int KPW, int RS, bool MULTI, bool AF32 = false, bool PF32 = false, bool W2 = false, int DF = 0>
 __global__ __launch_bounds__(NW * 64) void k_gemv_small(const bf16_raw* a_A, long a_aps, const bf16_raw* a_W, int a_KT, int a_M, int a_epi,
                                                         int a_nstrips, float* a_out, int a_ldo, const float* a_gnext, GemmK p) {
   p.A = a_A; p.a_plane_stride = a_aps; p.W = a_W; p.KT = a_KT; p.M = a_M; p.epi = a_epi; p.nstrips = a_nstrips;
@@ -119,6 +119,9 @@
   float* tile = reinterpret_cast<float*>(smem_raw + sizeof(f32x4) * NW * 64);
   float* inv_s = tile + 16 * 17;
   bf16x8* As = reinterpret_cast<bf16x8*>(smem_raw + sizeof(f32x4) * NW * 64 + sizeof(float) * (16 * 17 + 16));
+  static_assert(DF == 0 || (AF32 && PF32 && !W2), "the deferred wo merge: fp32 activation tiles, one weight plane");
+  static_assert(DF != 2 || (NW * KPW == 64 && (RS == 2 || RS == 4)), "the deferred consumer holds a whole row of D = 2048: 128 strips");
+  static_assert(DF != 1 || !MULTI, "the deferred producer: one strip per workgroup");
 
   const int tid = threadIdx.x, lane = tid & 63, w = tid >> 6;
   const int kt0 = w * KPW;
@@ -151,7 +154,22 @@
   constexpr int CE = (KPA * RS + 15) / 16;
   bf16x8 v0[AF32 ? 1 : CH];
   float4 ex[AF32 ? CE : 1], ey[AF32 ? CE : 1];
-  if constexpr (AF32) {
+  constexpr int CD = DF == 2 ? CE : 1;
+  float4 d0x[CD], d0y[CD], d1x[CD], d1y[CD], dxx[CD], dxy[CD], dgx[CD], dgy[CD];
+  float* hs = reinterpret_cast<float*>(As + nchunks);
+  if constexpr (DF == 2) {
+#pragma unroll
+    for (int u = 0; u < CE; ++u) {
+      const int c = min(tid + u * NT, nentries - 1);
+      const int row = min(c % RS, p.M - 1), kq = (c / RS) & 3, kt = c / (4 * RS);
+      const float4* s0 = reinterpret_cast<const float4*>(p.wo_slices + ((long)kt * 64 + row + 16 * kq) * 8);
+      const float4* s1 = reinterpret_cast<const float4*>(p.wo_slices + p.wo_slice_stride + ((long)kt * 64 + row + 16 * kq) * 8);
+      const float4* xo = reinterpret_cast<const float4*>(p.wo_xold + (long)row * p.wo_ldx + kt * 32 + kq * 8);
+      const float4* gn = reinterpret_cast<const float4*>(p.gnext + kt * 32 + kq * 8);
+      d0x[u] = s0[0]; d0y[u] = s0[1]; d1x[u] = s1[0]; d1y[u] = s1[1];
+      dxx[u] = xo[0]; dxy[u] = xo[1]; dgx[u] = gn[0]; dgy[u] = gn[1];
+    }
+  } else if constexpr (AF32) {
     const float* Af = reinterpret_cast<const float*>(p.A);
 #pragma unroll
     for (int u = 0; u < CE; ++u) {
@@ -168,18 +186,18 @@
       v0[u] = *reinterpret_cast<const bf16x8*>(p.A + pl * p.a_plane_stride + ((long)(ktga + kt) * 64 + row + 16 * kq) * 8);
     }
   }
-  const bool has_norm = p.ssq_in != nullptr;
+  const bool has_norm = DF == 2 || p.ssq_in != nullptr;
   const int s_row = tid >> 3, s_part = tid & 7;
   const bool s_thread = tid < 128 && has_norm;
   float sq[16];
 #pragma unroll
   for (int i = 0; i < 16; ++i) sq[i] = 0.f;
-  if (s_thread) {
+  if (DF != 2 && s_thread) {
     const float* sp = p.ssq_in + min(s_row, p.M - 1);
 #pragma unroll
     for (int i = 0; i < 16; ++i) sq[i] = sp[(long)min(s_part + 8 * i, p.ssq_in_n - 1) * p.ssq_ld];
   }
-  const bool resid = p.epi == DIA_EPI_RESID_EMIT;
+  const bool resid = DF != 1 && p.epi == DIA_EPI_RESID_EMIT;
   const bool r_thread = tid < 16 * RS;
   float xpre1 = 0.f, gpre1 = 1.f;
   auto load_resid = [&](int strip) {
@@ -194,7 +212,41 @@
   __builtin_amdgcn_sched_barrier(0);
 #endif
   STAMP(1);
-  if constexpr (AF32) {
+  if constexpr (DF == 2) {
+#pragma unroll
+    for (int u = 0; u < CE; ++u)
+      if (tid + u * NT < nentries) {
+        const int c = tid + u * NT;
+        const int row = c % RS, kq = (c / RS) & 3, kt = c / (4 * RS);
+        const float s0[8] = {d0x[u].x, d0x[u].y, d0x[u].z, d0x[u].w, d0y[u].x, d0y[u].y, d0y[u].z, d0y[u].w};
+        const float s1[8] = {d1x[u].x, d1x[u].y, d1x[u].z, d1x[u].w, d1y[u].x, d1y[u].y, d1y[u].z, d1y[u].w};
+        const float xo[8] = {dxx[u].x, dxx[u].y, dxx[u].z, dxx[u].w, dxy[u].x, dxy[u].y, dxy[u].z, dxy[u].w};
+        const float gn[8] = {dgx[u].x, dgx[u].y, dgx[u].z, dgx[u].w, dgy[u].x, dgy[u].y, dgy[u].z, dgy[u].w};
+        float xn[8], vg[8];
+        float acc = 0.f;
+#pragma unroll
+        for (int j = 0; j < 8; ++j) {
+          xn[j] = add_rn(xo[j], add_rn(add_rn(0.f, s0[j]), s1[j]));
+          const float q = mul_rn(xn[j], xn[j]);
+          acc = j == 0 ? q : add_rn(acc, q);
+          vg[j] = mul_rn(xn[j], gn[j]);
+        }
+        hs[row * (4 * KT) + kt * 4 + kq] = acc;
+        if (p.wo_xnew != nullptr && kt * 2 + (kq >> 1) == (int)blockIdx.x && row < p.M) {
+          float4* o = reinterpret_cast<float4*>(p.wo_xnew + (long)row * p.wo_ldx + kt * 32 + kq * 8);
+          o[0] = float4{xn[0], xn[1], xn[2], xn[3]}; o[1] = float4{xn[4], xn[5], xn[6], xn[7]};
+        }
+        bf16x8 h, mi, lo;
+        split3x8(float4{vg[0], vg[1], vg[2], vg[3]}, float4{vg[4], vg[5], vg[6], vg[7]}, h, mi, lo);
+        As[c] = h; As[nentries + c] = mi; As[2 * nentries + c] = lo;
+      }
+    lds_barrier();
+    if (tid < 128) {
+      const float* h = hs + min(s_row, RS - 1) * (4 * KT);
+#pragma unroll
+      for (int i = 0; i < 16; ++i) sq[i] = h[2 * (s_part + 8 * i)] + h[2 * (s_part + 8 * i) + 1];
+    }
+  } else if constexpr (AF32) {
 #pragma unroll
     for (int u = 0; u < CE; ++u)
       if (tid + u * NT < nentries) {
@@ -211,8 +263,8 @@
   {
     float s0 = 0.f;
 #pragma unroll
-    for (int i = 0; i < 16; ++i) s0 += (s_part + 8 * i < p.ssq_in_n && s_row < p.M) ? sq[i] : 0.f;
-    if (s_thread && s_row < p.M)
+    for (int i = 0; i < 16; ++i) s0 += ((DF == 2 || s_part + 8 * i < p.ssq_in_n) && s_row < p.M) ? sq[i] : 0.f;
+    if (DF != 2 && s_thread && s_row < p.M)
       for (int idx = s_part + 128; idx < p.ssq_in_n; idx += 8) s0 += p.ssq_in[(long)idx * p.ssq_ld + s_row];
     s0 += __builtin_bit_cast(float, __builtin_amdgcn_update_dpp(0, __builtin_bit_cast(int, s0), 0xB1, 0xF, 0xF, true));
     s0 += __builtin_bit_cast(float, __builtin_amdgcn_update_dpp(0, __builtin_bit_cast(int, s0), 0x4E, 0xF, 0xF, true));
@@ -242,7 +294,7 @@
     }
     STAMP(3);
     float v = 0.f;
-    if (MULTI || gridDim.y == 1) {
+    if (MULTI || DF == 1 || gridDim.y == 1) {
       f32x4* rb = red16 + sbuf * (NW * 16);
       sbuf ^= 1;
       if (lane < 16) rb[w * 16 + lane] = acc[0];
@@ -259,6 +311,11 @@
       STAMP(4);
       if (!splitk_combine(p, tile, strip, tid, &sk_flag)) return;
       if (r_thread) v = tile[(tid >> 4) * 17 + (tid & 15)];
+    }
+    if constexpr (DF == 1) {
+      const int m = tid >> 4, n = strip * 16 + (tid & 15);
+      if (r_thread && m < p.M) p.wo_slices[(long)blockIdx.y * p.wo_slice_stride + plane_frag_off(m, n & ~7, p.p_ktiles) + (n & 7)] = v;
+      return;
     }
     if (r_thread) {
       run_epilogue_rows<RS, PF32>(p, v, inv_s, tid, strip, xpre1, gpre1);
@@ -1782,6 +1839,38 @@
   return dia_check_launch("k_gemm16");
 }
 
+template <int RS>
+int launch_wo_deferred(const GemmK& k, int role, hipStream_t st) {
+  if (role == 1) {
+    launch_small_kernel<k_gemv_small<16, 8, RS, false, true, true, false, 1>>(dim3(k.nstrips, 2), dim3(1024), small_smem(16, 128, RS), st, k);
+    return dia_check_launch("k_gemv_small");
+  }
+  const size_t smem = small_smem(8, 64, RS) + sizeof(float) * RS * 256;
+  const int spw = pick_spw(k, 512, 1, 1);
+  const int grid = (k.nstrips + spw - 1) / spw;
+  if (k.wo_xnew && grid < 128) return dia_fail(DIA_E_ARG, "dia_gemm: deferred wo merge: fewer workgroups than strips of x to write back");
+  if (spw > 1) launch_small_kernel<k_gemv_small<8, 8, RS, true, true, true, false, 2>>(dim3(grid), dim3(512), smem, st, k);
+  else launch_small_kernel<k_gemv_small<8, 8, RS, false, true, true, false, 2>>(dim3(grid), dim3(512), smem, st, k);
+  return dia_check_launch("k_gemv_small");
+}
+
+int gemm_wo_deferred(const dia_gemm_args* a, const dia_wo_defer_args* w, GemmK& k, hipStream_t st) {
+  const int role = w->defer ? 1 : 2;
+  const bool emits = a->epi == DIA_EPI_RESID_EMIT;
+  const auto al16 = [](const void* q) { return (reinterpret_cast<uintptr_t>(q) & 15) == 0; };
+  bool ok = a->M <= 4 && a->w_format == DIA_W_DENSE && a->w_planes <= 1 && a->w_layout == 0 && !a->cmap && !a->sp_blocks && !a->sp_toff &&
+            w->nslices == 2 && w->slices && al16(w->slices) && w->slice_stride % 4 == 0 && a->gnext && dia_tune(DIA_TUNE_GEMM_SPW) <= 0;
+  if (role == 1) ok = ok && emits && (a->act_f32 & 3) == 3 && a->sk == 2 && a->KT == 256 && (a->nw == 0 || a->nw == 16) && !w->xold && !w->xnew &&
+                      w->slice_stride >= (int64_t)a->p_ktiles * 512 && (int64_t)a->nstrips * 16 <= (int64_t)a->p_ktiles * 32 && a->P && a->out;
+  else ok = ok && a->epi == DIA_EPI_SCALE_STORE && (a->act_f32 & 1) && a->sk <= 1 && a->KT == 64 && (a->nw == 0 || a->nw == 8) && w->xold &&
+            w->xold != w->xnew && al16(w->xold) && al16(w->xnew) && al16(a->gnext) && w->ldx >= 2048 && w->ldx % 4 == 0 &&
+            w->slice_stride >= 64 * 512;
+  if (!ok) return dia_fail(DIA_E_ARG, "dia_gemm_wo_deferred: serves M <= 4, dense one-plane weights, fp32 tiles, no cmap, two slices: wo as K 8192 "
+                                      "RESID_EMIT with gnext, its consumer as K 2048 SCALE_STORE with xold and gnext (16-byte aligned)");
+  k.wo_slices = w->slices; k.wo_slice_stride = w->slice_stride; k.wo_xold = w->xold; k.wo_xnew = w->xnew; k.wo_ldx = w->ldx;
+  return a->M <= 2 ? launch_wo_deferred<2>(k, role, st) : launch_wo_deferred<4>(k, role, st);
+}
+
 }
 
 #ifdef DIA_DBG_STAMPS
@@ -1824,9 +1913,11 @@
 }
 }
 
-extern "C" int dia_gemm(const dia_gemm_args* a, void* stream) {
+static int gemm_impl(const dia_gemm_args* a, const dia_wo_defer_args* wd, void* stream) {
   if (!a || !a->A || (!a->W && !a->sp_blocks)) return dia_fail(DIA_E_ARG, "dia_gemm: null argument");
   if (a->M <= 0 || a->KT <= 0 || a->nstrips <= 0) return dia_fail(DIA_E_ARG, "dia_gemm: empty problem");
+  if (wd && (a->w_format != DIA_W_DENSE || a->w_layout != 0 || a->w_planes > 1 || a->sp_blocks || a->sp_toff))
+    return dia_fail(DIA_E_ARG, "dia_gemm_wo_deferred: dense one-plane weight tiles only");
   if (a->w_format != DIA_W_DENSE && a->w_format != DIA_W_SPARSE24 && a->w_format != DIA_W_MXFP8) return dia_fail(DIA_E_ARG, "dia_gemm: unknown w_format");
   if (a->w_format == DIA_W_SPARSE24) {
     const int rc = dia_gemm_sparse24_check(a);
@@ -1884,6 +1975,7 @@
   }
   GemmK k;
   fill_gemmk(a, k);
+  if (wd) return gemm_wo_deferred(a, wd, k, (hipStream_t)stream);
   if (a->w_planes == 2) return gemm_w2(a, k, (hipStream_t)stream);
   if (a->w_planes > 1) {
     if (a->w_planes != 3) return dia_fail(DIA_E_ARG, "dia_gemm: w_planes must be 0, 1, 2 or 3");
@@ -2001,6 +2093,21 @@
   return launch_generic(k, nw, st);
 }
 
+extern "C" int dia_gemm(const dia_gemm_args* a, void* stream) { return gemm_impl(a, nullptr, stream); }
+
+extern "C" int dia_gemm_wo_deferred(const dia_gemm_args* a, const dia_wo_defer_args* w, void* stream, float* ms_out) {
+  if (!w) return dia_fail(DIA_E_ARG, "dia_gemm_wo_deferred: null argument");
+  if (!ms_out) return gemm_impl(a, w, stream);
+  dia_recorder_arm();
+  int rc = gemm_impl(a, w, stream);
+  float ms[4] = {0.f, 0.f, 0.f, 0.f};
+  const int n = dia_recorder_collect(ms, 4);
+  if (rc != DIA_OK) return rc;
+  if (n < 1) return n < 0 ? n : dia_fail(DIA_E_STATE, "dia_gemm_wo_deferred: nothing was launched");
+  *ms_out = ms[0];
+  return DIA_OK;
+}
+
 extern "C" int dia_gemm_timed(const dia_gemm_args* a, void* stream, float* ms_out) {
   if (!ms_out) return dia_fail(DIA_E_ARG, "dia_gemm_timed: null output");
   dia_recorder_arm();
diff --git a/dia-tts-prune_amd/csrc/gemm_common.hpp b/dia-tts-prune_amd/csrc/gemm_common.hpp
--- a/dia-tts-prune_amd/csrc/gemm_common.hpp
+++ b/dia-tts-prune_amd/csrc/gemm_common.hpp
@@ -57,6 +57,8 @@
   long kv_layer_stride; int kv_layer_strips;
   int sk2_quads;
   int w_planes; long w_plane_stride;
+  float* wo_slices; long wo_slice_stride;
+  const float* wo_xold; float* wo_xnew; int wo_ldx;
 };
 
 __device__ __forceinline__ void load_afrag3(const GemmK& p, long off, bf16x8& a0, bf16x8& a1, bf16x8& a2) {
@@ -355,6 +357,7 @@
   k.kv_layer_strips = a->kv_layer_strips; k.kv_layer_stride = a->kv_layer_stride;
   k.sk2_quads = dia_tune(DIA_TUNE_GEMM_2T) != 7;
   k.w_planes = a->w_planes > 1 ? a->w_planes : 1; k.w_plane_stride = (long)a->KT * a->nstrips * 512;
+  k.wo_slices = nullptr; k.wo_slice_stride = 0; k.wo_xold = nullptr; k.wo_xnew = nullptr; k.wo_ldx = 0;
   return DIA_OK;
 }
 
diff --git a/dia-tts-prune_amd/csrc/tuning.cpp b/dia-tts-prune_amd/csrc/tuning.cpp
--- a/dia-tts-prune_amd/csrc/tuning.cpp
+++ b/dia-tts-prune_amd/csrc/tuning.cpp
@@ -7,9 +7,9 @@
 #include <string>
 
 static const char* const k_names[DIA_TUNE_COUNT] = {
-    "attn_nz", "attn_gpw", "attn_gpw_cross", "gemm_spw", "gemm_mz_max", "tile_min_blocks", "wo_sk", "wo_pair", "wo_nw", "wo_spw", "act_f32", "wo_diag", "gemm_2t", "gemm_zr", "seg", "seg_nb", "seg_dbg", "seg_sleep", "g2t_wgs", "ckv_merge", "mxfp8",
+    "attn_nz", "attn_gpw", "attn_gpw_cross", "gemm_spw", "gemm_mz_max", "tile_min_blocks", "wo_sk", "wo_pair", "wo_nw", "wo_spw", "act_f32", "wo_diag", "gemm_2t", "gemm_zr", "seg", "seg_nb", "seg_dbg", "seg_sleep", "g2t_wgs", "ckv_merge", "mxfp8", "wo_defer",
     "mlp_fuse", "tile_v", "blk32_kr", "blk32_ws", "no_g32", "g32_all", "g32m"};
-static int g_tune[DIA_TUNE_COUNT] = {-1, -1, -1, -1, -1, -1, -1, -1, -1, -1, -1, -1, -1, -1, -1, -1, -1, -1, -1, -1, -1, -1, -1, -1, -1, -1, -1};
+static int g_tune[DIA_TUNE_COUNT] = {-1, -1, -1, -1, -1, -1, -1, -1, -1, -1, -1, -1, -1, -1, -1, -1, -1, -1, -1, -1, -1, -1, -1, -1, -1, -1, -1, -1};
 
 int dia_tune(int id) {
   dia_tuning_init_from_env();
diff --git a/dia-tts-prune_amd/csrc/tuning.hpp b/dia-tts-prune_amd/csrc/tuning.hpp
--- a/dia-tts-prune_amd/csrc/tuning.hpp
+++ b/dia-tts-prune_amd/csrc/tuning.hpp
@@ -22,6 +22,7 @@
   DIA_TUNE_G2T_WGS,
   DIA_TUNE_CKV_MERGE,
   DIA_TUNE_MXFP8,
+  DIA_TUNE_WO_DEFER,
   DIA_TUNE_MLP_FUSE,
   DIA_TUNE_TILE_V,
   DIA_TUNE_BLK32_KR,
diff --git a/dia-tts-prune_amd/dia_hip/binding.py b/dia-tts-prune_amd/dia_hip/binding.py
--- a/dia-tts-prune_amd/dia_hip/binding.py
+++ b/dia-tts-prune_amd/dia_hip/binding.py
@@ -15,9 +15,9 @@
 ATTN_SELF, ATTN_CROSS, ATTN_ENC = 0, 1, 2
 
 EXPORTS = (
-    "dia_last_error", "dia_abi_version", "dia_device_count", "dia_set_tuning", "dia_get_tuning", "dia_has_experiments", "dia_gemm", "dia_gemm_timed", "dia_mlp_fused", "dia_mlp_fused_timed", "dia_engine_mlp_fused", "dia_attn", "dia_attn_scratch_floats", "dia_enc_kv_prep", "dia_enc_attn", "dia_dec_prefill_embed", "dia_dec_prefill_kv", "dia_dec_prefill_attn",
+    "dia_last_error", "dia_abi_version", "dia_device_count", "dia_set_tuning", "dia_get_tuning", "dia_has_experiments", "dia_gemm", "dia_gemm_timed", "dia_gemm_wo_deferred", "dia_mlp_fused", "dia_mlp_fused_timed", "dia_engine_mlp_fused", "dia_attn", "dia_attn_scratch_floats", "dia_enc_kv_prep", "dia_enc_attn", "dia_dec_prefill_embed", "dia_dec_prefill_kv", "dia_dec_prefill_attn",
     "dia_embed_text", "dia_embed_tokens", "dia_sample", "dia_slot_admit", "dia_slot_retire", "dia_prefetch", "dia_engine_create", "dia_engine_destroy",
-    "dia_engine_decode", "dia_engine_set_prefetch", "dia_engine_step_logits_only", "dia_engine_profile_step", "dia_engine_time_step", "dia_timed_kernel_name", "dia_engine_launches_per_step", "dia_mxfp8_classes",
+    "dia_engine_decode", "dia_engine_set_prefetch", "dia_engine_set_x_alt", "dia_engine_step_logits_only", "dia_engine_profile_step", "dia_engine_time_step", "dia_timed_kernel_name", "dia_engine_launches_per_step", "dia_mxfp8_classes",
     "dia_seg_mlp", "dia_seg_workspace_bytes", "dia_seg_workspace_control_bytes", "dia_seg_slots", "dia_seg_supported", "dia_seg_error",
 )
 
@@ -43,6 +43,13 @@
         ("act_f32", C.c_int32), ("w_planes", C.c_int32), ("kv_plane_stride", C.c_int64),
         ("w_layout", C.c_int32), ("kv_layer_strips", C.c_int32), ("kv_layer_stride", C.c_int64),
         ("w_format", C.c_int32), ("_pad2", C.c_int32),
+    ]
+
+
+class WoDeferArgs(C.Structure):
+    _fields_ = [
+        ("slices", C.c_void_p), ("slice_stride", C.c_int64), ("nslices", C.c_int32), ("defer", C.c_int32),
+        ("xold", C.c_void_p), ("xnew", C.c_void_p), ("ldx", C.c_int32), ("_pad0", C.c_int32),
     ]
 
 
@@ -207,6 +214,8 @@
     L.dia_has_experiments.restype = C.c_int
     L.dia_gemm.argtypes = [C.POINTER(GemmArgs), C.c_void_p]
     L.dia_gemm_timed.argtypes = [C.POINTER(GemmArgs), C.c_void_p, C.POINTER(C.c_float)]
+    L.dia_gemm_wo_deferred.argtypes = [C.POINTER(GemmArgs), C.POINTER(WoDeferArgs), C.c_void_p, C.POINTER(C.c_float)]
+    L.dia_engine_set_x_alt.argtypes = [C.c_void_p, C.c_void_p]
     L.dia_mlp_fused.argtypes = [C.POINTER(GemmArgs), C.POINTER(GemmArgs), C.c_void_p, C.c_void_p]
     L.dia_mlp_fused_timed.argtypes = [C.POINTER(GemmArgs), C.POINTER(GemmArgs), C.c_void_p, C.c_void_p, C.POINTER(C.c_float)]
     L.dia_engine_mlp_fused.argtypes = [C.c_void_p]
diff --git a/dia-tts-prune_amd/dia_hip/engine.py b/dia-tts-prune_amd/dia_hip/engine.py
--- a/dia-tts-prune_amd/dia_hip/engine.py
+++ b/dia-tts-prune_amd/dia_hip/engine.py
@@ -449,6 +449,7 @@
         mt = self.rows_pad // 16
         self.xkt, self.akt, self.hkt = self.D // 32, max(d.gqa_query_heads, d.cross_query_heads) * HEAD_DIM // 32, self.F // 32
         self.x = z(self.rows_pad, self.D)
+        self.x_alt = z(self.rows_pad, self.D) if self.R <= 4 else None
         t_ = hb.get_tuning("act_f32")
         self.act_f32 = int(t_ != 0)
         self.seg = bool(self.R <= 4 and w.seg_layers and self.act_f32 and hb.get_tuning("seg") == 1)
@@ -485,6 +486,8 @@
         if 16 < self.R <= 32:
             n_scr = max([n_scr, w.logits.ns * -(-w.logits.kt // 8) * 512] +
                         [DL[k].ns * -(-DL[k].kt // 8) * 512 for DL in w.dec_layers for k in DEC_MATS])
+        if self.R <= 4:
+            n_scr = max(n_scr, 2 * self.rows_pad * self.D)
         self.sk_scratch = z(n_scr)
         self.sk_tickets = z(max(ns_max, 8 * (self.D // 16)), dt=torch.int32)
         self.mlp_barrier = z(2, dt=torch.int32)
@@ -636,6 +639,8 @@
         self._desc = ed
         hb.check(hb.lib().dia_engine_create(C.byref(ed), C.c_void_p(self.stream.cuda_stream), C.byref(self._engine)),
                  "dia_engine_create")
+        if self.x_alt is not None:
+            hb.check(hb.lib().dia_engine_set_x_alt(self._engine, hb.ptr(self.x_alt)), "dia_engine_set_x_alt")
 
     def close(self):
         if self._engine:
diff --git a/include/dia_hip.h b/include/dia_hip.h
--- a/include/dia_hip.h
+++ b/include/dia_hip.h
@@ -92,6 +92,17 @@
   int32_t _pad2;
 } dia_gemm_args;
 int dia_gemm(const dia_gemm_args* a, void* stream);
+typedef struct {
+  float* slices;
+  int64_t slice_stride;
+  int32_t nslices;
+  int32_t defer;
+  const float* xold;
+  float* xnew;
+  int32_t ldx;
+  int32_t _pad0;
+} dia_wo_defer_args;
+int dia_gemm_wo_deferred(const dia_gemm_args* a, const dia_wo_defer_args* w, void* stream, float* ms_out);
 int dia_mlp_fused(const dia_gemm_args* wi, const dia_gemm_args* wo, int32_t* barrier, void* stream);
 int dia_mlp_fused_timed(const dia_gemm_args* wi, const dia_gemm_args* wo, int32_t* barrier, void* stream, float* ms_out);
 
@@ -364,6 +375,7 @@
 int dia_engine_mlp_fused(const dia_engine* e);
 int dia_engine_decode(dia_engine* e, int n_steps, int use_graph);
 int dia_engine_set_prefetch(dia_engine* e, int lookahead);
+int dia_engine_set_x_alt(dia_engine* e, float* x_alt);
 int dia_engine_step_logits_only(dia_engine* e);
 int dia_engine_profile_step(dia_engine* e, float* ms_per_launch, int cap);
 int dia_engine_time_step(dia_engine* e, float* ms_per_kernel, float* interval_ms, int cap);
```

Result: faster. 1041 frames/s (median of 6 runs) (+1.3%).
